# isunLt/U2MKD

Hardware: AMD Instinct MI355X
Metric: LiDAR points/sec/node fwd+bwd (teacher+student+KD), 1/2/4/8 MI355X (higher is better)
Workload: dtype f32 (fp32 products emulated on the 16-bit matrix pipe: f16x2 forward / input gradient, bf16x3 weight gradient; fp32 accumulate)

## Files before the change

### include/u2mkd_hip.h

```cpp
#ifndef U2MKD_HIP_H
#define U2MKD_HIP_H

#include <stddef.h>
#include <stdint.h>

#ifdef __cplusplus
extern "C" {
#endif

typedef void *u2mkd_stream_t;

int u2mkd_version(void);
const char *u2mkd_last_error(void);
int u2mkd_stream_wait_stream(u2mkd_stream_t waiter, u2mkd_stream_t signaler);
void *u2mkd_mailbox_alloc(size_t bytes);
int u2mkd_mailbox_free(void *p);
int u2mkd_mailbox_post(const void *const *srcs, uint32_t is64, int32_t n, int64_t *slot, int64_t seq, u2mkd_stream_t s);

int u2mkd_hash(const int32_t *coords , int64_t n, int64_t *out , u2mkd_stream_t s);
int u2mkd_kernel_hash(const int32_t *coords , const int32_t *offsets , int64_t n,
                      int32_t k, int64_t *out , u2mkd_stream_t s);

size_t u2mkd_hash_table_bytes(int64_t n_refs);
int u2mkd_hash_table_build(const int64_t *refs, int64_t n_refs, void *table, u2mkd_stream_t s);
// ... 7 lines not shown
                           int32_t *nbr , u2mkd_stream_t s);
int u2mkd_kmap_invert(const int32_t *nbr , int64_t n_out, int32_t k, int64_t n_in,
                      int32_t *nbr_inv , u2mkd_stream_t s);
int u2mkd_kmap_sizes(const int32_t *nbr, int64_t n_out, int32_t k, int32_t *nbsizes ,
                     int32_t *block_counts , u2mkd_stream_t s);
int u2mkd_kmap_compact(const int32_t *nbr, int64_t n_out, int32_t k, const int32_t *nbsizes ,
                       int32_t *block_counts ,
                       int32_t *nbmaps , u2mkd_stream_t s);

int64_t u2mkd_pairs_capacity(int64_t n_in, int64_t n_out, int32_t k);
int u2mkd_pairs_build(const int32_t *nbr , int64_t n_out, int64_t n_in, int32_t k,
                      const int32_t *nbsizes, int32_t *block_counts, int32_t *pair_in, int32_t *pair_out,
                      int32_t *pos_out, int32_t *pos_in, int32_t *tile_k, int32_t *meta, u2mkd_stream_t s);
int u2mkd_downsample_keys(const int32_t *coords , int64_t n, int32_t sx, int32_t sy, int32_t sz,
                          int64_t *keys , u2mkd_stream_t s);
int u2mkd_downsample_keys_checked(const int32_t *coords , int64_t n, int32_t sx, int32_t sy, int32_t sz,
                                  int64_t *keys , int32_t *range_flag, u2mkd_stream_t s);
int u2mkd_unpack_keys(const int64_t *keys, int64_t n, int32_t *coords , u2mkd_stream_t s);
int u2mkd_downsample_keys_general(const int32_t *coords , int64_t n, int32_t tsx, int32_t tsy, int32_t tsz, int32_t kx,
                                  int32_t ky, int32_t kz, int32_t sx, int32_t sy, int32_t sz, const int32_t *cmin ,
                                  int32_t m, int64_t *keys , int32_t *range_flag, u2mkd_stream_t s);
int u2mkd_floor_coords(const float *pc , int64_t n, int32_t stride, int32_t *out , u2mkd_stream_t s);

int u2mkd_transpose_weights(const float *w , int32_t k, int32_t cin, int32_t cout,
                            float *wt , u2mkd_stream_t s);
int u2mkd_conv_forward(const float *in , int64_t n_in, int32_t cin, const float *wt ,
                       int32_t cout, const int32_t *nbr , int64_t n_out, int32_t k, int32_t kflip,
                       float *out , u2mkd_stream_t s);
int u2mkd_conv_forward_sorted(const float *in, int64_t n_in, int32_t cin, const float *wt, int32_t cout,
                              const int32_t *nbr_sorted , const int32_t *order ,
                              const int32_t *tile_order , int64_t n_out, int32_t k,
                              int32_t kflip, float *out , u2mkd_stream_t s);
int32_t u2mkd_conv_tiles_supported(int32_t cin, int32_t cout, int32_t k);
int32_t u2mkd_conv_tiles_arith(int32_t cin, int32_t cout, int32_t k);
size_t u2mkd_weight_fragments_bytes(int32_t k, int32_t rows, int32_t cols, int32_t arith);
int u2mkd_weight_fragments(const float *w, int32_t k, int32_t rows, int32_t cols, int32_t transpose, int32_t arith,
                           void *wf, u2mkd_stream_t s);
int u2mkd_weight_fragments_batch(const int64_t *jobs, int32_t n_jobs, int64_t total_units, u2mkd_stream_t s);
int u2mkd_conv_forward_tiles(const float *in, int64_t n_in, int32_t cin, const void *wf, int32_t cout,
                             const int32_t *nbr_sorted , const int32_t *order ,
                             const int32_t *items ,
                             const int32_t *n_items , int64_t n_out, int32_t k,
                             int32_t kflip, int32_t arith, float *out , u2mkd_stream_t s);
int u2mkd_conv_forward_tiles_ep(const float *in, int64_t n_in, int32_t cin, const void *wf, int32_t cout,
                                const int32_t *nbr_sorted, const int32_t *order, const int32_t *items,
                                const int32_t *n_items, int64_t n_out, int32_t k, int32_t kflip, int32_t arith,
                                const float *scale , const float *shift , const float *res ,
                                int32_t relu, float *out, u2mkd_stream_t s);
int32_t u2mkd_pairs_gather_sum_stats_slab_rows(void);
int32_t u2mkd_pairs_gather_sum_stats_supported(int32_t cout);
int u2mkd_pairs_gather_sum_stats(const float *y, const int32_t *pos, int64_t n_rows, int32_t k, int32_t cout, float *out,
                                 float *partial, u2mkd_stream_t s);
int u2mkd_pairs_gather_sum_ep(const float *y, const int32_t *pos, int64_t n_rows, int32_t k, int32_t cout, const float *scale,
                              const float *shift, const float *res, int32_t relu, float *out, u2mkd_stream_t s);
int u2mkd_debug_conv_forward_sorted(const float *in, int64_t n_in, int32_t cin, const float *wt, int32_t cout,
                                    const int32_t *nbr_sorted, const int32_t *order, const int32_t *tile_order,
                                    int64_t n_out, int32_t k, int32_t kflip, int32_t variant, float *out,
                                    u2mkd_stream_t s);
int u2mkd_debug_conv_tile_pairs_stamps(const float *in, int64_t n_in, const void *wf ,
                                       const int32_t *nbr_sorted, const int32_t *order, const int32_t *items,
                                       const int32_t *n_items, int64_t n_out, int32_t k, int32_t arith, float *out,
                                       uint64_t *stamps, u2mkd_stream_t s);
int u2mkd_debug_wgrad_stamps(const float *a, const float *b, const int32_t *pairs, const int32_t *plan, int64_t n_rows,
                             int32_t k, void *workspace, uint64_t *stamps, u2mkd_stream_t s);
int u2mkd_conv_forward_pairs(const float *in, int64_t n_in, int32_t cin, const float *wt, int32_t cout,
                             const int32_t *pair_idx, const int32_t *tile_k, const int32_t *meta, int64_t capacity,
                             int32_t k, int32_t kc, float *y , u2mkd_stream_t s);
int32_t u2mkd_conv_pairs_x3_supported(int32_t cin, int32_t cout);
int u2mkd_conv_forward_pairs_x3(const float *in, int64_t n_in, int32_t cin, const void *wf, int32_t cout,
                                const int32_t *pair_idx, const int32_t *tile_k, const int32_t *meta, int64_t capacity,
                                int32_t k, float *y , u2mkd_stream_t s);
int u2mkd_linear_forward(const float *x , int64_t n, int32_t cin, const float *w , int32_t cout,
                         const float *bias , int32_t kc, float *y, u2mkd_stream_t s);
int u2mkd_linear_forward_x3(const float *x , int64_t n, int32_t cin, const void *wf, int32_t cout,
                            const float *bias , float *y , u2mkd_stream_t s);
int32_t u2mkd_conv_pairs_f16x2_supported(int32_t cin, int32_t cout);
int u2mkd_conv_forward_pairs_f16x2(const float *in, int64_t n_in, int32_t cin, const void *wf, int32_t cout,
                                    const int32_t *pair_idx, const int32_t *tile_k, const int32_t *meta, int64_t capacity,
                                    int32_t k, float *y, u2mkd_stream_t s);
int u2mkd_linear_forward_f16x2(const float *x, int64_t n, int32_t cin, const void *wf, int32_t cout, const float *bias,
                               float *y, u2mkd_stream_t s);
int u2mkd_pairs_gather_sum(const float *y, const int32_t *pos , int64_t n_rows, int32_t k, int32_t cout,
                           float *out , u2mkd_stream_t s);
int u2mkd_kmap_rowmask(const int32_t *nbr , int64_t n_out, int32_t k, int32_t *mask ,
                       u2mkd_stream_t s);
int u2mkd_conv_forward_tiles_bf16(const void *in , int64_t n_in, int32_t cin, const void *wf, int32_t cout,
                                  const int32_t *nbr_sorted, const int32_t *order, const int32_t *items,
                                  const int32_t *n_items, int64_t n_out, int32_t k, int32_t kflip,
                                  void *out , u2mkd_stream_t s);
int u2mkd_conv_wgrad_pairs_bf16(const void *a , int32_t ca, const void *b , int32_t cb,
                                const int32_t *pairs, const int32_t *plan, int64_t n_rows, int32_t k, int32_t swap,
                                void *workspace, size_t workspace_bytes, float *dw , u2mkd_stream_t s);
int u2mkd_conv_forward_tiles_f16(const void *in , int64_t n_in, int32_t cin, const void *wf, int32_t cout,
                                 const int32_t *nbr_sorted, const int32_t *order, const int32_t *items,
                                 const int32_t *n_items, int64_t n_out, int32_t k, int32_t kflip,
                                 void *out , u2mkd_stream_t s);
int u2mkd_conv_wgrad_pairs_f16(const void *a , int32_t ca, const void *b , int32_t cb,
                               const int32_t *pairs, const int32_t *plan, int64_t n_rows, int32_t k, int32_t swap,
                               void *workspace, size_t workspace_bytes, float *dw , u2mkd_stream_t s);
int u2mkd_conv_forward_pairs_f16(const void *in , int64_t n_in, int32_t cin, const void *wf, int32_t cout,
                                  const int32_t *pair_idx, const int32_t *tile_k, const int32_t *meta, int64_t capacity,
                                  int32_t k, void *y , u2mkd_stream_t s);
int u2mkd_linear_forward_f16(const void *x , int64_t n, int32_t cin, const void *wf, int32_t cout,
                             const float *bias , void *y , u2mkd_stream_t s);
int u2mkd_pairs_gather_sum_f16(const void *y , const int32_t *pos , int64_t n_rows, int32_t k,
                               int32_t cout, void *out , u2mkd_stream_t s);
int u2mkd_conv_forward_pairs_bf16(const void *in , int64_t n_in, int32_t cin, const void *wf, int32_t cout,
                                   const int32_t *pair_idx, const int32_t *tile_k, const int32_t *meta, int64_t capacity,
                                   int32_t k, void *y , u2mkd_stream_t s);
int u2mkd_linear_forward_bf16(const void *x , int64_t n, int32_t cin, const void *wf, int32_t cout,
                              const float *bias , void *y , u2mkd_stream_t s);
int u2mkd_pairs_gather_sum_bf16(const void *y , const int32_t *pos , int64_t n_rows, int32_t k,
                                int32_t cout, void *out , u2mkd_stream_t s);
size_t u2mkd_tile_schedule_workspace_bytes(int64_t n_rows);
int u2mkd_tile_schedule(const int32_t *mask , const int32_t *order , int64_t n_rows,
                        int32_t k, int32_t split0, int32_t split1, void *workspace, int32_t *tile_order,
                        int32_t *items, int32_t *n_items, u2mkd_stream_t s);
int32_t u2mkd_wgrad_plan_ints(int32_t k);
int u2mkd_wgrad_plan(const int32_t *nbsizes , int32_t k, int64_t n_rows, int32_t *plan, u2mkd_stream_t s);
size_t u2mkd_conv_wgrad_pairs_workspace_bytes(int64_t n_rows, int32_t ca, int32_t cb, int32_t k);
int u2mkd_conv_wgrad_pairs(const float *a, int32_t ca, const float *b, int32_t cb, const int32_t *pairs ,
                           const int32_t *plan, int64_t n_rows, int32_t k, int32_t swap, void *workspace,
                           size_t workspace_bytes, float *dw , u2mkd_stream_t s);

size_t u2mkd_convolution_workspace_bytes(int64_t n_in_rows, int64_t n_out_rows, int32_t cin, int32_t cout,
                                         const int32_t *nbsizes_host , int32_t k);
int u2mkd_convolution_forward(const float *in_feat , int64_t n_in_rows, int32_t cin,
                              float *out_feat , int64_t n_out_rows, int32_t cout,
                              const float *kernel , const int32_t *nbmaps ,
                              const int32_t *nbsizes_host , int32_t k, int32_t transpose, void *workspace,
                              size_t workspace_bytes, u2mkd_stream_t s);
int u2mkd_convolution_backward(const float *in_feat , int64_t n_in_rows, int32_t cin,
                               float *grad_in_feat , const float *grad_out_feat ,
                               int64_t n_out_rows, int32_t cout, const float *kernel ,
                               float *grad_kernel , const int32_t *nbmaps, const int32_t *nbsizes_host,
                               int32_t k, int32_t transpose, void *workspace, size_t workspace_bytes, u2mkd_stream_t s);

int u2mkd_count(const int32_t *idx , int64_t n, int32_t *counts , int64_t num,
                u2mkd_stream_t s);
int u2mkd_voxelize_forward(const float *feats , const int32_t *idx , const int32_t *counts ,
                           int64_t n, int64_t nv, int32_t c, float *out , u2mkd_stream_t s);
int u2mkd_voxelize_backward(const float *grad_out , const int32_t *idx, const int32_t *counts, int64_t n,
                            int64_t nv, int32_t c, float *grad_feats , u2mkd_stream_t s);
int u2mkd_devoxelize_forward(const float *feats , const int32_t *idx , const float *w ,
                             int64_t n, int32_t c, float *out , u2mkd_stream_t s);
int u2mkd_devoxelize_backward(const float *grad_out , const int32_t *idx , const float *w ,
                              int64_t n, int64_t nv, int32_t c, float *grad_feats ,
                              u2mkd_stream_t s);
int u2mkd_segment_sum(const float *src , int32_t c, const int32_t *entry_row ,
                      const float *entry_w , const int32_t *seg_offsets , int64_t nv,
                      int32_t mean, float *out , u2mkd_stream_t s);
int u2mkd_voxelize_backward_bf16(const void *grad_out , const int32_t *idx, const int32_t *counts, int64_t n,
                                 int64_t nv, int32_t c, void *grad_feats , u2mkd_stream_t s);
int u2mkd_devoxelize_forward_bf16(const void *feats , const int32_t *idx , const float *w ,
                                  int64_t n, int32_t c, void *out , u2mkd_stream_t s);
int u2mkd_segment_sum_bf16(const void *src , int32_t c, const int32_t *entry_row ,
                           const float *entry_w , const int32_t *seg_offsets , int64_t nv,
                           int32_t mean, void *out , u2mkd_stream_t s);
int u2mkd_voxelize_backward_f16(const void *grad_out , const int32_t *idx, const int32_t *counts, int64_t n,
                                int64_t nv, int32_t c, void *grad_feats , u2mkd_stream_t s);
int u2mkd_devoxelize_forward_f16(const void *feats , const int32_t *idx , const float *w ,
                                 int64_t n, int32_t c, void *out , u2mkd_stream_t s);
int u2mkd_segment_sum_f16(const void *src , int32_t c, const int32_t *entry_row ,
                          const float *entry_w , const int32_t *seg_offsets , int64_t nv,
                          int32_t mean, void *out , u2mkd_stream_t s);
size_t u2mkd_csr_workspace_bytes(int64_t n_entries, int64_t nv);
// ... 254 lines not shown
```

### u2mkd_amd/_lib.py

```python
from __future__ import annotations

import ctypes as C
import os

import torch

_HERE = os.path.dirname(os.path.abspath(__file__))
LIB_PATH = os.path.join(_HERE, 'lib', 'libu2mkd_hip%s.so' % os.environ.get('U2MKD_LIB_SUFFIX', ''))

_i32, _i64, _sz, _f32, _p = C.c_int32, C.c_int64, C.c_size_t, C.c_float, C.c_void_p

SIGNATURES = {
    'u2mkd_version': (C.c_int, []),
    'u2mkd_last_error': (C.c_char_p, []),
    'u2mkd_hash': (C.c_int, [_p, _i64, _p, _p]),
    'u2mkd_kernel_hash': (C.c_int, [_p, _p, _i64, _i32, _p, _p]),
    'u2mkd_hash_table_bytes': (_sz, [_i64]),
    'u2mkd_hash_table_build': (C.c_int, [_p, _i64, _p, _p]),
    'u2mkd_hash_table_query': (C.c_int, [_p, _i64, _p, _i64, _p, _p]),
    'u2mkd_hash_table_query2': (C.c_int, [_p, _i64, _p, _i64, _p, _p, _p]),
    'u2mkd_kmap_build_table': (C.c_int, [_p, _i64, _p, _i64, _p, _i32, _p, _p]),
    'u2mkd_kmap_invert': (C.c_int, [_p, _i64, _i32, _i64, _p, _p]),
    'u2mkd_kmap_sizes': (C.c_int, [_p, _i64, _i32, _p, _p, _p]),
    'u2mkd_kmap_compact': (C.c_int, [_p, _i64, _i32, _p, _p, _p, _p]),
    'u2mkd_downsample_keys': (C.c_int, [_p, _i64, _i32, _i32, _i32, _p, _p]),
    'u2mkd_downsample_keys_checked': (C.c_int, [_p, _i64, _i32, _i32, _i32, _p, _p, _p]),
    'u2mkd_downsample_keys_general': (C.c_int, [_p, _i64] + [_i32] * 9 + [_p, _i32, _p, _p, _p]),
    'u2mkd_floor_coords': (C.c_int, [_p, _i64, _i32, _p, _p]),
    'u2mkd_unpack_keys': (C.c_int, [_p, _i64, _p, _p]),
    'u2mkd_transpose_weights': (C.c_int, [_p, _i32, _i32, _i32, _p, _p]),
    'u2mkd_conv_forward': (C.c_int, [_p, _i64, _i32, _p, _i32, _p, _i64, _i32, _i32, _p, _p]),
    'u2mkd_conv_forward_sorted': (C.c_int, [_p, _i64, _i32, _p, _i32, _p, _p, _p, _i64, _i32, _i32, _p, _p]),
    'u2mkd_debug_conv_forward_sorted': (C.c_int, [_p, _i64, _i32, _p, _i32, _p, _p, _p, _i64, _i32, _i32, _i32, _p, _p]),
    'u2mkd_stream_wait_stream': (C.c_int, [_p, _p]),
    'u2mkd_sgd_chunk_elements': (_i32, []),
    'u2mkd_sgd_batch': (C.c_int, [_p, _i32, _i64, _f32, _f32, _f32, _i32, _i32, _p]),
    'u2mkd_grads_unscale_check': (C.c_int, [_p, _i32, _i64, _p, _p, _p]),
    'u2mkd_sgd_batch_amp': (C.c_int, [_p, _i32, _i64, _f32, _f32, _f32, _i32, _i32, _p, _p, _p]),
    'u2mkd_adam_batch': (C.c_int, [_p, _i32, _i64, _p, _f32, _f32, _i32, _f32, _f32, _f32, _f32, _i32, _p]),
    'u2mkd_adam_batch_amp': (C.c_int, [_p, _i32, _i64, _p, _i32, _f32, _f32, _i32, _f32, _f32, _f32, _f32, _i32, _p, _p, _i32, _p, _p, _p]),
    'u2mkd_debug_adam_stage': (C.c_int, [_i32, _i32, _p, _p, _p, _f32, _p, _i64, _p]),
    'u2mkd_mailbox_alloc': (_p, [_sz]),
    'u2mkd_mailbox_free': (C.c_int, [_p]),
    'u2mkd_mailbox_post': (C.c_int, [_p, C.c_uint32, _i32, _p, _i64, _p]),
    'u2mkd_conv_tiles_supported': (_i32, [_i32, _i32, _i32]),
    'u2mkd_conv_tiles_arith': (_i32, [_i32, _i32, _i32]),
    'u2mkd_weight_fragments_bytes': (_sz, [_i32, _i32, _i32, _i32]),
    'u2mkd_weight_fragments': (C.c_int, [_p, _i32, _i32, _i32, _i32, _i32, _p, _p]),
    'u2mkd_weight_fragments_batch': (C.c_int, [_p, _i32, _i64, _p]),
    'u2mkd_conv_forward_tiles': (C.c_int, [_p, _i64, _i32, _p, _i32, _p, _p, _p, _p, _i64, _i32, _i32, _i32, _p, _p]),
    'u2mkd_conv_forward_tiles_ep': (C.c_int, [_p, _i64, _i32, _p, _i32, _p, _p, _p, _p, _i64, _i32, _i32, _i32, _p, _p, _p, _i32, _p, _p]),
    'u2mkd_pairs_gather_sum_ep': (C.c_int, [_p, _p, _i64, _i32, _i32, _p, _p, _p, _i32, _p, _p]),
    'u2mkd_pairs_gather_sum_stats_slab_rows': (_i32, []),
    'u2mkd_pairs_gather_sum_stats_supported': (_i32, [_i32]),
    'u2mkd_pairs_gather_sum_stats': (C.c_int, [_p, _p, _i64, _i32, _i32, _p, _p, _p]),
    'u2mkd_debug_conv_tile_pairs_stamps': (C.c_int, [_p, _i64, _p, _p, _p, _p, _p, _i64, _i32, _i32, _p, _p, _p]),
    'u2mkd_debug_wgrad_stamps': (C.c_int, [_p, _p, _p, _p, _i64, _i32, _p, _p, _p]),
    'u2mkd_conv_forward_pairs': (C.c_int, [_p, _i64, _i32, _p, _i32, _p, _p, _p, _i64, _i32, _i32, _p, _p]),
    'u2mkd_conv_pairs_x3_supported': (_i32, [_i32, _i32]),
    'u2mkd_conv_forward_pairs_x3': (C.c_int, [_p, _i64, _i32, _p, _i32, _p, _p, _p, _i64, _i32, _p, _p]),
    'u2mkd_linear_forward': (C.c_int, [_p, _i64, _i32, _p, _i32, _p, _i32, _p, _p]),
    'u2mkd_bn2d_workspace_bytes': (C.c_size_t, [_i64, _i32, _i64]),
    'u2mkd_bn2d_train_forward': (C.c_int, [_p, _p, _i64, _i32, _i64, _p, _p, C.c_float, C.c_float, _i32, _p, _p, _p, _p, _p, _p, _p, _p]),
    'u2mkd_bn2d_eval_forward': (C.c_int, [_p, _p, _i64, _i32, _i64, _p, _p, C.c_float, _i32, _p, _p, _p, _p]),
    'u2mkd_bn2d_backward': (C.c_int, [_p, _p, _p, _i64, _i32, _i64, _p, _p, _p, _p, _i32, _i32, _p, _p, _p, _p, _p, _p]),
    'u2mkd_bn2d_local_stats': (C.c_int, [_p, _i64, _i32, _i64, _p, _p, _p]),
    'u2mkd_bn2d_apply': (C.c_int, [_p, _p, _i64, _i32, _i64, _p, _p, _p, _p, _i32, _p, _p]),
    'u2mkd_bn2d_backward_local': (C.c_int, [_p, _p, _p, _i64, _i32, _i64, _p, _p, _p, _p, _i32, _p, _p, _p, _p]),
    'u2mkd_bn2d_backward_apply': (C.c_int, [_p, _p, _p, _i64, _i32, _i64, _p, _p, _p, _p, _p, _i32, _p, _p, _p, _p]),
    'u2mkd_linear_forward_x3': (C.c_int, [_p, _i64, _i32, _p, _i32, _p, _p, _p]),
    'u2mkd_conv_pairs_f16x2_supported': (_i32, [_i32, _i32]),
    'u2mkd_conv_forward_pairs_f16x2': (C.c_int, [_p, _i64, _i32, _p, _i32, _p, _p, _p, _i64, _i32, _p, _p]),
    'u2mkd_linear_forward_f16x2': (C.c_int, [_p, _i64, _i32, _p, _i32, _p, _p, _p]),
    'u2mkd_pairs_capacity': (_i64, [_i64, _i64, _i32]),
    'u2mkd_pairs_build': (C.c_int, [_p, _i64, _i64, _i32, _p, _p, _p, _p, _p, _p, _p, _p, _p]),
    'u2mkd_pairs_gather_sum': (C.c_int, [_p, _p, _i64, _i32, _i32, _p, _p]),
    'u2mkd_kmap_rowmask': (C.c_int, [_p, _i64, _i32, _p, _p]),
    'u2mkd_tile_schedule_workspace_bytes': (_sz, [_i64]),
    'u2mkd_tile_schedule': (C.c_int, [_p, _p, _i64, _i32, _i32, _i32, _p, _p, _p, _p, _p]),
    'u2mkd_wgrad_plan_ints': (_i32, [_i32]),
    'u2mkd_wgrad_plan': (C.c_int, [_p, _i32, _i64, _p, _p]),
    'u2mkd_conv_wgrad_pairs_workspace_bytes': (_sz, [_i64, _i32, _i32, _i32]),
    'u2mkd_conv_wgrad_pairs': (C.c_int, [_p, _i32, _p, _i32, _p, _p, _i64, _i32, _i32, _p, _sz, _p, _p]),
    'u2mkd_conv_forward_tiles_bf16': (C.c_int, [_p, _i64, _i32, _p, _i32, _p, _p, _p, _p, _i64, _i32, _i32, _p, _p]),
    'u2mkd_conv_forward_tiles_f16': (C.c_int, [_p, _i64, _i32, _p, _i32, _p, _p, _p, _p, _i64, _i32, _i32, _p, _p]),
    'u2mkd_conv_wgrad_pairs_bf16': (C.c_int, [_p, _i32, _p, _i32, _p, _p, _i64, _i32, _i32, _p, _sz, _p, _p]),
    'u2mkd_conv_wgrad_pairs_f16': (C.c_int, [_p, _i32, _p, _i32, _p, _p, _i64, _i32, _i32, _p, _sz, _p, _p]),
    'u2mkd_conv_forward_pairs_bf16': (C.c_int, [_p, _i64, _i32, _p, _i32, _p, _p, _p, _i64, _i32, _p, _p]),
    'u2mkd_conv_forward_pairs_f16': (C.c_int, [_p, _i64, _i32, _p, _i32, _p, _p, _p, _i64, _i32, _p, _p]),
    'u2mkd_linear_forward_bf16': (C.c_int, [_p, _i64, _i32, _p, _i32, _p, _p, _p]),
    'u2mkd_linear_forward_f16': (C.c_int, [_p, _i64, _i32, _p, _i32, _p, _p, _p]),
    'u2mkd_pairs_gather_sum_bf16': (C.c_int, [_p, _p, _i64, _i32, _i32, _p, _p]),
    'u2mkd_pairs_gather_sum_f16': (C.c_int, [_p, _p, _i64, _i32, _i32, _p, _p]),
    'u2mkd_convolution_workspace_bytes': (_sz, [_i64, _i64, _i32, _i32, _p, _i32]),
    'u2mkd_convolution_forward': (C.c_int, [_p, _i64, _i32, _p, _i64, _i32, _p, _p, _p, _i32, _i32, _p, _sz, _p]),
    'u2mkd_convolution_backward': (C.c_int, [_p, _i64, _i32, _p, _p, _i64, _i32, _p, _p, _p, _p, _i32, _i32, _p, _sz, _p]),
    'u2mkd_bn_num_slabs': (_i64, [_i64]),
    'u2mkd_bn_train_forward': (C.c_int, [_p, _p, _i32, _i64, _i32, _p, _p, _f32, _f32, _p, _p, _p, _i32, _p, _p, _p, _p, _p]),
    'u2mkd_bn_train_forward_from_partial': (C.c_int, [_p, _p, _i64, _i32, _p, _p, _f32, _f32, _p, _p, _p, _i32, _p, _i32, _p, _p, _p, _p]),
    'u2mkd_bn_eval_forward': (C.c_int, [_p, _p, _i32, _i64, _i32, _p, _p, _f32, _p, _p, _i32, _p, _p, _p]),
    'u2mkd_bn_backward': (C.c_int, [_p, _p, _p, _i32, _i64, _i32, _p, _p, _p, _p, _i32, _i32, _p, _p, _p, _p, _p, _p]),
    'u2mkd_bn_local_stats': (C.c_int, [_p, _i32, _i64, _i32, _p, _p, _p]),
    'u2mkd_bn_merge_stats': (C.c_int, [_p, _i32, _i32, _f32, _f32, _p, _p, _p, _p, _p, _p, _p]),
    'u2mkd_bn_apply': (C.c_int, [_p, _p, _i32, _i64, _i32, _p, _p, _p, _p, _i32, _p, _p]),
    'u2mkd_bn_backward_local': (C.c_int, [_p, _p, _p, _i32, _i64, _i32, _p, _p, _p, _p, _i32, _p, _p, _p, _p]),
    'u2mkd_bn_backward_apply': (C.c_int, [_p, _p, _p, _i32, _i64, _i32, _p, _p, _p, _p, _p, _i32, _p, _p, _p, _p]),
    'u2mkd_ln_num_slabs': (_i64, [_i64, _i32]),
    'u2mkd_ln_forward': (C.c_int, [_p, _i32, _i64, _i32, _p, _p, _f32, _p, _p, _p, _p]),
    'u2mkd_ln_add_forward': (C.c_int, [_p, _p, _p, _i32, _i64, _i32, _p, _p, _f32, _p, _p, _p, _p, _p]),
    'u2mkd_ln_backward': (C.c_int, [_p, _p, _p, _p, _i32, _i64, _i32, _p, _p, _p, _p, _p, _p, _p, _p, _p]),
    'u2mkd_sptr_window_keys': (C.c_int, [_p, _p, _i64, _p, _p, _f32, _f32, _f32, _p, _p]),
    'u2mkd_select_mse_partials': (_i32, []),
    'u2mkd_select_mse_forward': (C.c_int, [_p, _p, _p, _i64, _i32, _p, _p, _p, _p]),
    'u2mkd_select_mse_backward': (C.c_int, [_p, _p, _p, _p, _p, _p, _i64, _i32, _p, _p, _p]),
    'u2mkd_sptr_plan_prepare_workspace_bytes': (_sz, []),
    'u2mkd_sptr_plan_prepare': (C.c_int, [_p, _p, _i64, _f32, _f32, _f32, _f32, _f32, _f32, _p, _p, _p, _p, _p, _p]),
    'u2mkd_sptr_window_ranges': (C.c_int, [_p, _i64, _p, _p, _p]),
    'u2mkd_sptr_quant_coords': (C.c_int, [_p, _p, _i64, _p, _f32, _f32, _f32, _f32, _f32, _f32, _p, _p, _p]),
    'u2mkd_sptr_attention_forward': (C.c_int, [_p, _p, _p, _p, _p, _p, _p, _p, _p, _p, _p, _i32, _i32, _f32, _i64, _i32, _i32, _p, _p, _p]),
    'u2mkd_sptr_backward_workspace_bytes': (_sz, [_i64, _i32, _i32]),
    'u2mkd_sptr_attention_backward': (C.c_int, [_p] * 14 + [_i32, _i32, _f32, _i32, _i64, _i32, _i32] + [_p, _p, _sz] + [_p] * 7),
    'u2mkd_sptr_tiles_workspace_bytes': (_sz, [_i64, _i32]),
    'u2mkd_sptr_attention_forward_tiles': (C.c_int, [_p, _p, _p, _i64, _f32] + [_p] * 8 + [_i32, _i32, _f32, _i64, _i32, _i32, _p, _i64, _p, _p, _sz, _p]),
    'u2mkd_sptr_attention_forward_strided': (C.c_int, [_p, _p, _p, _i64, _f32] + [_p] * 8 + [_i32, _i32, _f32, _i64, _i32, _i32, _p, _i64, _p, _p]),
    'u2mkd_sptr_attention_backward_strided': (C.c_int, [_p, _p, _p, _i64, _f32, _p, _p, _i64] + [_p] * 9 + [_i32, _i32, _f32, _i32, _i64, _i32, _i32]
                                              + [_p, _p, _sz] + [_p, _p, _p, _i64, _p, _p, _p, _p]),
    'u2mkd_sptr_table_reduce': (C.c_int, [_p, _i64, _i32, _i32, _f32, _p, _p, _p, _p]),
    'u2mkd_sptr_precompute_all': (C.c_int, [_i32, _i32, C.c_uint32] + [_p] * 8),
    'u2mkd_sptr_attention_step1_forward': (C.c_int, [_i32, _i32, _i32, _i32, _i32, C.c_uint32] + [_p] * 6),
    'u2mkd_sptr_attention_step1_backward': (C.c_int, [_i32, _i32, _i32, _i32, C.c_uint32] + [_p] * 10),
    'u2mkd_sptr_attention_step2_forward': (C.c_int, [_i32] * 5 + [_p] * 6),
    'u2mkd_sptr_attention_step2_backward': (C.c_int, [_i32] * 5 + [_p] * 10),
    'u2mkd_sptr_dot_prod_with_idx_forward': (C.c_int, [_i32] * 6 + [_p] * 10),
    'u2mkd_sptr_dot_prod_with_idx_all_forward': (C.c_int, [_i32] * 6 + [_p] * 10),
    'u2mkd_sptr_dot_prod_with_idx_backward': (C.c_int, [_i32] * 6 + [_p] * 14),
    'u2mkd_sptr_attention_step2_with_rel_pos_value_forward': (C.c_int, [_i32] * 5 + [_p] * 8),
    'u2mkd_sptr_attention_step2_with_rel_pos_value_backward': (C.c_int, [_i32] * 6 + [_p] * 13),
    'u2mkd_count': (C.c_int, [_p, _i64, _p, _i64, _p]),
    'u2mkd_voxelize_forward': (C.c_int, [_p, _p, _p, _i64, _i64, _i32, _p, _p]),
    'u2mkd_voxelize_backward': (C.c_int, [_p, _p, _p, _i64, _i64, _i32, _p, _p]),
    'u2mkd_devoxelize_forward': (C.c_int, [_p, _p, _p, _i64, _i32, _p, _p]),
    'u2mkd_devoxelize_backward': (C.c_int, [_p, _p, _p, _i64, _i64, _i32, _p, _p]),
    'u2mkd_segment_sum': (C.c_int, [_p, _i32, _p, _p, _p, _i64, _i32, _p, _p]),
    'u2mkd_voxelize_backward_bf16': (C.c_int, [_p, _p, _p, _i64, _i64, _i32, _p, _p]),
    'u2mkd_voxelize_backward_f16': (C.c_int, [_p, _p, _p, _i64, _i64, _i32, _p, _p]),
    'u2mkd_devoxelize_forward_bf16': (C.c_int, [_p, _p, _p, _i64, _i32, _p, _p]),
    'u2mkd_devoxelize_forward_f16': (C.c_int, [_p, _p, _p, _i64, _i32, _p, _p]),
    'u2mkd_segment_sum_bf16': (C.c_int, [_p, _i32, _p, _p, _p, _i64, _i32, _p, _p]),
    'u2mkd_segment_sum_f16': (C.c_int, [_p, _i32, _p, _p, _p, _i64, _i32, _p, _p]),
    'u2mkd_c2l_plan': (C.c_int, [_p, _p, _i32, _i64, _i32, _i32, _i32, _p, _p, _p]),
    'u2mkd_l2c_keys': (C.c_int, [_p, _p, _i32, _i64, _i32, _i64, _i64, _i32, _i32, _p, _p, _p, _p, _p]),
    'u2mkd_l2c_finish': (C.c_int, [_p, _p, _p, _p, _p, _i64, _p, _p, _p, _p, _p]),
    'u2mkd_up_bilinear_forward': (C.c_int, [_p, _p, _i64, _i32, _i32, _i32, _i32, _f32, _f32, _p, _p]),
    'u2mkd_up_bilinear_backward': (C.c_int, [_p, _i64, _i32, _i32, _i32, _i32, _p, _p, _p, _p, _i32, _p, _p]),
    'u2mkd_maxpool3s2_forward': (C.c_int, [_p, _i64, _i32, _i32, _p, _p, _p]),
    'u2mkd_maxpool3s2_backward': (C.c_int, [_p, _p, _i64, _i32, _i32, _p, _p]),
    'u2mkd_transpose_batched': (C.c_int, [_p, _p, _i32, _i32, _i32, _p]),
    'u2mkd_transpose_batched_scaled': (C.c_int, [_p, _p, _i32, _i32, _i32, C.c_float, _p]),
    'u2mkd_l2c_combine_forward': (C.c_int, [_p, _p, _p, _p] + [_i32] * 11 + [_p, _p]),
# ... 76 lines not shown
```

### u2mkd_amd/csrc/conv.hip

```cpp
#include <stdlib.h>

#include "conv_internal.h"

namespace u2mkd {

__global__ void transpose_weights_kernel(const float *__restrict__ w, int cin, int cout, float *__restrict__ wt,
                                         int64_t total) {
    int64_t t = (int64_t)blockIdx.x * blockDim.x + threadIdx.x;
    if (t >= total) return;
    int ci = (int)(t % cin);
    int64_t r = t / cin;
    int co = (int)(r % cout);
    int64_t k = r / cout;
    wt[t] = w[(k * cin + ci) * cout + co];
}

template <int WAVES, int NB, int KC>
__global__ void __launch_bounds__(64 * WAVES)
conv_os2_kernel(const float *__restrict__ in, int cin, const float *__restrict__ wt, int cout,
                const int32_t *__restrict__ nbr, const int32_t *__restrict__ order, RowRange rr_, int K, int kflip,
                float *__restrict__ out) {
    constexpr int NT = 64 * WAVES;
    constexpr int TM = 16 * WAVES, TN = 16 * NB;
    constexpr int BS = KC + 8;
// ... 654 lines not shown
    __syncthreads();
    int buf = 0, c = 0;
    while (true) {
        const bool last_chunk = c + 1 == nchunk;
        const bool have_next = !last_chunk || tile_n < tile_end;
        const bool new_b = have_next && (nchunk > 1 || k_n != k);
        if (have_next) {
            if (!last_chunk) load_stage(k, c + 1, idx, a_nxt, new_b);
            else load_stage(k_n, 0, idx_n, a_nxt, new_b);
        }
        if (__ballot(idx >= 0) != 0ULL) {
            const float *bb = Bs + (size_t)buf * TN * BS + r * BS + 4 * q;
#pragma unroll
            for (int j = 0; j < NJ; ++j) {
                float4 b[NB];
#pragma unroll
                for (int n = 0; n < NB; ++n) b[n] = *reinterpret_cast<const float4 *>(bb + 16 * n * BS + 16 * j);
#pragma unroll
                for (int n = 0; n < NB; ++n) acc[n] = __builtin_amdgcn_mfma_f32_16x16x4f32(a_cur[j].x, b[n].x, acc[n], 0, 0, 0);
#pragma unroll
                for (int n = 0; n < NB; ++n) acc[n] = __builtin_amdgcn_mfma_f32_16x16x4f32(a_cur[j].y, b[n].y, acc[n], 0, 0, 0);
#pragma unroll
                for (int n = 0; n < NB; ++n) acc[n] = __builtin_amdgcn_mfma_f32_16x16x4f32(a_cur[j].z, b[n].z, acc[n], 0, 0, 0);
#pragma unroll
                for (int n = 0; n < NB; ++n) acc[n] = __builtin_amdgcn_mfma_f32_16x16x4f32(a_cur[j].w, b[n].w, acc[n], 0, 0, 0);
            }
        }
        if (last_chunk) {
            float *yr = y + ((size_t)tile * 64 + 16 * wave + 4 * q) * cout + col0 + r;
#pragma unroll
            for (int reg = 0; reg < 4; ++reg)
#pragma unroll
                for (int n = 0; n < NB; ++n) {
                    if (col0 + 16 * n + r < cout) yr[(size_t)reg * cout + 16 * n] = acc[n][reg];
                    acc[n][reg] = bv[n];
                }
        }
        if (!have_next) break;
        if (new_b) {
            store_B(buf ^ 1);
            __syncthreads();
            buf ^= 1;
        }
        if (last_chunk) {
            tile = tile_n;
            idx = idx_n;
            k = k_n;
            c = 0;
            ++tile_n;
            idx_n = -1;
            if (tile_n < tile_end) {
                idx_n = entry(tile_n);
                k_n = tile_k ? tile_k[tile_n] : 0;
            }
        } else {
            ++c;
        }
#pragma unroll
        for (int j = 0; j < NJ; ++j) a_cur[j] = a_nxt[j];
    }
}

template <int KC>
static int launch_conv_pairs(int nb, dim3 grid, hipStream_t st, const float *in, int cin, const float *wt, int cout,
                             const int32_t *pair_idx, const int32_t *tile_k, const int32_t *n_tiles, int64_t n_dense,
                             const float *bias, float *y) {
    size_t lds = (size_t)2 * 16 * nb * (KC + 8) * 4;
#define U2_CASE(N)                                                                                                 \
    case N:                                                                                                        \
        if (lds > 65536)                                                                                           \
            (void)hipFuncSetAttribute(reinterpret_cast<const void *>(&conv_pairs_kernel<N, KC>),                   \
                                      hipFuncAttributeMaxDynamicSharedMemorySize, (int)lds);                       \
        hipLaunchKernelGGL((conv_pairs_kernel<N, KC>), grid, dim3(256), lds, st, in, cin, wt, cout, pair_idx,      \
                           tile_k, n_tiles, n_dense, bias, y);                                                     \
        break;
    switch (nb) {
        U2_CASE(1) U2_CASE(2) U2_CASE(3) U2_CASE(4) U2_CASE(5) U2_CASE(6) U2_CASE(7) U2_CASE(8)
        default: set_error("conv pairs: unsupported column block count %d", nb); return 2;
    }
#undef U2_CASE
    return 0;
}

__global__ void __launch_bounds__(256)
pairs_gather_sum_kernel(const float *__restrict__ y, const int32_t *__restrict__ pos, int64_t n_rows, int K, int c4,
                        float *__restrict__ out, const float *__restrict__ ep_scale = nullptr,
                        const float *__restrict__ ep_shift = nullptr, const float *__restrict__ ep_res = nullptr, int ep_relu = 0) {
    int64_t t = (int64_t)blockIdx.x * 256 + threadIdx.x;
    if (t >= n_rows * c4) return;
    int64_t r = t / c4;
    int c = (int)(t - r * c4);
    const int32_t *pr = pos + r * K;
    float4 acc = make_float4(0.f, 0.f, 0.f, 0.f);
    for (int k0 = 0; k0 < K; k0 += 8) {
        int p[8];
        float4 v[8];
#pragma unroll
        for (int i = 0; i < 8; ++i) p[i] = k0 + i < K ? pr[k0 + i] : -1;
#pragma unroll
        for (int i = 0; i < 8; ++i)
            v[i] = p[i] >= 0 ? reinterpret_cast<const float4 *>(y)[(int64_t)p[i] * c4 + c] : make_float4(0.f, 0.f, 0.f, 0.f);
#pragma unroll
        for (int i = 0; i < 8; ++i) { acc.x += v[i].x; acc.y += v[i].y; acc.z += v[i].z; acc.w += v[i].w; }
    }
    if (ep_scale) {
        const float4 sc = reinterpret_cast<const float4 *>(ep_scale)[c], sh = reinterpret_cast<const float4 *>(ep_shift)[c];
        acc.x = fmaf(acc.x, sc.x, sh.x); acc.y = fmaf(acc.y, sc.y, sh.y); acc.z = fmaf(acc.z, sc.z, sh.z); acc.w = fmaf(acc.w, sc.w, sh.w);
        if (ep_res) {
            const float4 rs = reinterpret_cast<const float4 *>(ep_res)[r * c4 + c];
            acc.x += rs.x; acc.y += rs.y; acc.z += rs.z; acc.w += rs.w;
        }
        if (ep_relu) { acc.x = fmaxf(acc.x, 0.f); acc.y = fmaxf(acc.y, 0.f); acc.z = fmaxf(acc.z, 0.f); acc.w = fmaxf(acc.w, 0.f); }
    }
    reinterpret_cast<float4 *>(out)[r * c4 + c] = acc;
}

constexpr int kGsSlabRows = 32, kGsMaxIt = 16;

__global__ void __launch_bounds__(256)
pairs_gather_sum_stats_kernel(const float *__restrict__ y, const int32_t *__restrict__ pos, int64_t n_rows, int K, int c4,
                              float *__restrict__ out, float *__restrict__ partial) {
    __shared__ float4 red[256];
    const int rl = 256 / c4;
    const int ry = threadIdx.x / c4, j = threadIdx.x - ry * c4;
    const bool lane_on = ry < rl;
    const int64_t r0 = (int64_t)blockIdx.x * kGsSlabRows;
    const int rows = (int)min((int64_t)kGsSlabRows, n_rows - r0);
    float4 vals[kGsMaxIt];
    float4 sum = make_float4(0.f, 0.f, 0.f, 0.f);
#pragma unroll
    for (int it = 0; it < kGsMaxIt; ++it) {
        const int rr = it * rl + ry;
        vals[it] = make_float4(0.f, 0.f, 0.f, 0.f);
        if (lane_on && rr < rows) {
            const int64_t r = r0 + rr;
            const int32_t *pr = pos + r * K;
            float4 acc = make_float4(0.f, 0.f, 0.f, 0.f);
            for (int k0 = 0; k0 < K; k0 += 8) {
                int p[8];
                float4 v[8];
#pragma unroll
                for (int i = 0; i < 8; ++i) p[i] = k0 + i < K ? pr[k0 + i] : -1;
#pragma unroll
                for (int i = 0; i < 8; ++i)
                    v[i] = p[i] >= 0 ? reinterpret_cast<const float4 *>(y)[(int64_t)p[i] * c4 + j] : make_float4(0.f, 0.f, 0.f, 0.f);
#pragma unroll
                for (int i = 0; i < 8; ++i) { acc.x += v[i].x; acc.y += v[i].y; acc.z += v[i].z; acc.w += v[i].w; }
            }
            reinterpret_cast<float4 *>(out)[r * c4 + j] = acc;
            vals[it] = acc;
            sum.x += acc.x; sum.y += acc.y; sum.z += acc.z; sum.w += acc.w;
        }
    }
    if (lane_on) red[ry * c4 + j] = sum;
    __syncthreads();
    float4 mean = make_float4(0.f, 0.f, 0.f, 0.f);
    if (lane_on) {
        for (int g = 0; g < rl; ++g) {
            const float4 v = red[g * c4 + j];
            mean.x += v.x; mean.y += v.y; mean.z += v.z; mean.w += v.w;
        }
        const float inv = 1.f / (float)rows;
        mean.x *= inv; mean.y *= inv; mean.z *= inv; mean.w *= inv;
    }
    __syncthreads();
    float4 m2 = make_float4(0.f, 0.f, 0.f, 0.f);
#pragma unroll
    for (int it = 0; it < kGsMaxIt; ++it) {
        if (lane_on && it * rl + ry < rows) {
            const float dx = vals[it].x - mean.x, dy = vals[it].y - mean.y, dz = vals[it].z - mean.z, dw = vals[it].w - mean.w;
            m2.x += dx * dx; m2.y += dy * dy; m2.z += dz * dz; m2.w += dw * dw;
        }
    }
    if (lane_on) red[ry * c4 + j] = m2;
    __syncthreads();
    if (lane_on && ry == 0) {
        float4 t = make_float4(0.f, 0.f, 0.f, 0.f);
        for (int g = 0; g < rl; ++g) {
            const float4 v = red[g * c4 + j];
            t.x += v.x; t.y += v.y; t.z += v.z; t.w += v.w;
        }
        float *p = partial + (size_t)blockIdx.x * 2 * (4 * c4);
        *reinterpret_cast<float4 *>(p + 4 * j) = mean;
        *reinterpret_cast<float4 *>(p + 4 * c4 + 4 * j) = t;
    }
}

template <bool H16>
__global__ void __launch_bounds__(256)
pairs_gather_sum_rows16_kernel(const uint4 *__restrict__ y, const int32_t *__restrict__ pos, int64_t n_rows, int K, int c8,
                               uint4 *__restrict__ out) {
    int64_t t = (int64_t)blockIdx.x * 256 + threadIdx.x;
    if (t >= n_rows * c8) return;
    int64_t r = t / c8;
    int c = (int)(t - r * c8);
// ... 263 lines not shown
}

int u2mkd_conv_forward_pairs_x3(const float *in, int64_t n_in, int32_t cin, const void *wf, int32_t cout,
                                 const int32_t *pair_idx, const int32_t *tile_k, const int32_t *meta, int64_t capacity,
                                 int32_t k, float *y, u2mkd_stream_t s) {
    if (capacity == 0) return 0;
    U2_REQUIRE(in && wf && pair_idx && tile_k && meta && y, "u2mkd_conv_forward_pairs_x3: null pointer");
    U2_REQUIRE(k > 0 && n_in > 0 && capacity % 64 == 0, "u2mkd_conv_forward_pairs_x3: the capacity must be a multiple of 64");
    int rc = launch_conv_px3("u2mkd_conv_forward_pairs_x3", in, cin, reinterpret_cast<const float *>(wf), cout, pair_idx,
                             tile_k, meta + 1, capacity, y, as_stream(s));
    U2_REQUIRE(rc >= 0, "u2mkd_conv_forward_pairs_x3: cin=%d and cout=%d must be multiples of 32 "
               "(ask u2mkd_conv_pairs_x3_supported first)", cin, cout);
    return rc;
}

int32_t u2mkd_conv_pairs_f16x2_supported(int32_t cin, int32_t cout) {
    static const int pref = [] {
        const char *e = getenv("U2MKD_CONV_ARITH");
        return (e && (e[0] == 'b' || (e[0] == 'f' && e[1] == '3'))) ? 0 : 1;
    }();
    return (pref && conv_px3_supported(cin, cout)) ? 1 : 0;
}

int u2mkd_conv_forward_pairs_f16x2(const float *in, int64_t n_in, int32_t cin, const void *wf, int32_t cout,
                                    const int32_t *pair_idx, const int32_t *tile_k, const int32_t *meta, int64_t capacity,
                                    int32_t k, float *y, u2mkd_stream_t s) {
    if (capacity == 0) return 0;
    U2_REQUIRE(in && wf && pair_idx && tile_k && meta && y, "u2mkd_conv_forward_pairs_f16x2: null pointer");
    U2_REQUIRE(k > 0 && n_in > 0 && capacity % 64 == 0, "u2mkd_conv_forward_pairs_f16x2: the capacity must be a multiple of 64");
    int rc = launch_conv_px3("u2mkd_conv_forward_pairs_f16x2", in, cin, reinterpret_cast<const float *>(wf), cout, pair_idx,
                             tile_k, meta + 1, capacity, y, as_stream(s), false, k);
    U2_REQUIRE(rc >= 0, "u2mkd_conv_forward_pairs_f16x2: cin=%d and cout=%d must be multiples of 32", cin, cout);
    return rc;
}

int u2mkd_linear_forward_f16x2(const float *x, int64_t n, int32_t cin, const void *wf, int32_t cout, const float *bias,
                               float *y, u2mkd_stream_t s) {
    if (n == 0) return 0;
    U2_REQUIRE(x && wf && y, "u2mkd_linear_forward_f16x2: null pointer");
    U2_REQUIRE(n > 0 && n < ((int64_t)1 << 31) - 64, "u2mkd_linear_forward_f16x2: %lld rows out of range", (long long)n);
    int rc = launch_linear_px3("u2mkd_linear_forward_f16x2", x, n, cin, reinterpret_cast<const float *>(wf), cout, bias, y,
                               as_stream(s), false, true);
    U2_REQUIRE(rc >= 0, "u2mkd_linear_forward_f16x2: cin=%d and cout=%d must be multiples of 32", cin, cout);
    return rc;
}

int u2mkd_linear_forward(const float *x, int64_t n, int32_t cin, const float *w, int32_t cout, const float *bias,
                         int32_t variant, float *y, u2mkd_stream_t s) {
    if (n == 0) return 0;
    U2_REQUIRE(x && w && y, "u2mkd_linear_forward: null pointer");
    U2_REQUIRE(cin > 0 && cin % 4 == 0 && cout > 0, "u2mkd_linear_forward: cin=%d must be a positive multiple of 4", cin);
    if (variant == 0) variant = ((int64_t)cin * cout >= 16384 && cin % 64 == 0) ? 64 : 32;
    U2_REQUIRE(variant == 32 || variant == 64, "u2mkd_linear_forward: bad variant %d", variant);
    const int c16 = (cout + 15) / 16;
    const int nb = pick_nb(c16);
    int64_t gx = ceil_div(n, 64);
    if (gx > 2048) gx = 2048;
    dim3 grid((unsigned)gx, (unsigned)ceil_div(c16, nb));
    int rc = variant == 32 ? launch_conv_pairs<32>(nb, grid, as_stream(s), x, cin, w, cout, nullptr, nullptr, nullptr, n, bias, y)
                           : launch_conv_pairs<64>(nb, grid, as_stream(s), x, cin, w, cout, nullptr, nullptr, nullptr, n, bias, y);
    if (rc) return rc;
    return check_launch("u2mkd_linear_forward");
}

int u2mkd_linear_forward_x3(const float *x, int64_t n, int32_t cin, const void *wf, int32_t cout, const float *bias,
                            float *y, u2mkd_stream_t s) {
    if (n == 0) return 0;
    U2_REQUIRE(x && wf && y, "u2mkd_linear_forward_x3: null pointer");
    U2_REQUIRE(n > 0 && n < ((int64_t)1 << 31) - 64, "u2mkd_linear_forward_x3: %lld rows out of range", (long long)n);
    int rc = launch_linear_px3("u2mkd_linear_forward_x3", x, n, cin, reinterpret_cast<const float *>(wf), cout, bias, y,
                               as_stream(s));
    U2_REQUIRE(rc >= 0, "u2mkd_linear_forward_x3: cin=%d and cout=%d must be multiples of 32 "
               "(ask u2mkd_conv_pairs_x3_supported first)", cin, cout);
    return rc;
}

int u2mkd_pairs_gather_sum(const float *y, const int32_t *pos, int64_t n_rows, int32_t k, int32_t cout, float *out,
                            u2mkd_stream_t s) {
    if (n_rows == 0) return 0;
    U2_REQUIRE(y && pos && out, "u2mkd_pairs_gather_sum: null pointer");
    U2_REQUIRE(cout > 0 && cout % 4 == 0 && k > 0, "u2mkd_pairs_gather_sum: cout=%d must be a positive multiple of 4", cout);
    const int c4 = cout / 4;
    const int64_t total = n_rows * c4;
    hipLaunchKernelGGL(pairs_gather_sum_kernel, dim3((unsigned)ceil_div(total, 256)), dim3(256), 0, as_stream(s), y, pos,
                       n_rows, k, c4, out, (const float *)nullptr, (const float *)nullptr, (const float *)nullptr, 0);
    return check_launch("u2mkd_pairs_gather_sum");
}

int32_t u2mkd_pairs_gather_sum_stats_slab_rows(void) { return kGsSlabRows; }

int32_t u2mkd_pairs_gather_sum_stats_supported(int32_t cout) { return cout >= 8 && cout % 4 == 0 && cout <= 512; }

int u2mkd_pairs_gather_sum_stats(const float *y, const int32_t *pos, int64_t n_rows, int32_t k, int32_t cout, float *out,
                                 float *partial, u2mkd_stream_t s) {
    if (n_rows == 0) return 0;
    U2_REQUIRE(y && pos && out && partial, "u2mkd_pairs_gather_sum_stats: null pointer");
    U2_REQUIRE(k > 0 && u2mkd_pairs_gather_sum_stats_supported(cout), "u2mkd_pairs_gather_sum_stats: cout=%d must be a multiple of 4 in 8..512", cout);
    const int64_t slabs = ceil_div(n_rows, (int64_t)kGsSlabRows);
    U2_REQUIRE(slabs < ((int64_t)1 << 31), "u2mkd_pairs_gather_sum_stats: too many rows");
    hipLaunchKernelGGL(pairs_gather_sum_stats_kernel, dim3((unsigned)slabs), dim3(256), 0, as_stream(s), y, pos, n_rows, k, cout / 4,
                       out, partial);
    return check_launch("u2mkd_pairs_gather_sum_stats");
}

int u2mkd_pairs_gather_sum_ep(const float *y, const int32_t *pos, int64_t n_rows, int32_t k, int32_t cout, const float *scale,
                              const float *shift, const float *res, int32_t relu, float *out, u2mkd_stream_t s) {
    if (n_rows == 0) return 0;
    U2_REQUIRE(y && pos && out && scale && shift, "u2mkd_pairs_gather_sum_ep: null pointer");
    U2_REQUIRE(cout > 0 && cout % 4 == 0 && k > 0, "u2mkd_pairs_gather_sum_ep: cout=%d must be a positive multiple of 4", cout);
    const int c4 = cout / 4;
    const int64_t total = n_rows * c4;
    hipLaunchKernelGGL(pairs_gather_sum_kernel, dim3((unsigned)ceil_div(total, 256)), dim3(256), 0, as_stream(s), y, pos,
                       n_rows, k, c4, out, scale, shift, res, (int)relu);
    return check_launch("u2mkd_pairs_gather_sum_ep");
}

static int conv_forward_pairs_rows16(const char *who, int rows16, const void *in, int64_t n_in, int32_t cin, const void *wf,
                                     int32_t cout, const int32_t *pair_idx, const int32_t *tile_k, const int32_t *meta,
                                     int64_t capacity, int32_t k, void *y, u2mkd_stream_t s) {
    if (capacity == 0) return 0;
    U2_REQUIRE(in && wf && pair_idx && tile_k && meta && y, "%s: null pointer", who);
    U2_REQUIRE(k > 0 && n_in > 0 && capacity % 64 == 0, "%s: the capacity must be a multiple of 64", who);
    int rc = launch_conv_px3(who, reinterpret_cast<const float *>(in), cin, reinterpret_cast<const float *>(wf), cout, pair_idx,
                             tile_k, meta + 1, capacity, reinterpret_cast<float *>(y), as_stream(s), rows16);
    U2_REQUIRE(rc >= 0, "%s: cin=%d and cout=%d must be multiples of 32", who, cin, cout);
    return rc;
}

static int linear_forward_rows16(const char *who, int rows16, const void *x, int64_t n, int32_t cin, const void *wf,
                                 int32_t cout, const float *bias, void *y, u2mkd_stream_t s) {
    if (n == 0) return 0;
    U2_REQUIRE(x && wf && y, "%s: null pointer", who);
    U2_REQUIRE(n > 0 && n < ((int64_t)1 << 31) - 64, "%s: %lld rows out of range", who, (long long)n);
    int rc = launch_linear_px3(who, reinterpret_cast<const float *>(x), n, cin, reinterpret_cast<const float *>(wf), cout, bias,
                               reinterpret_cast<float *>(y), as_stream(s), rows16);
    U2_REQUIRE(rc >= 0, "%s: cin=%d and cout=%d must be multiples of 32", who, cin, cout);
    return rc;
}

static int pairs_gather_sum_rows16(const char *who, int rows16, const void *y, const int32_t *pos, int64_t n_rows, int32_t k,
                                   int32_t cout, void *out, u2mkd_stream_t s) {
    if (n_rows == 0) return 0;
    U2_REQUIRE(y && pos && out, "%s: null pointer", who);
    U2_REQUIRE(cout > 0 && cout % 8 == 0 && k > 0, "%s: cout=%d must be a positive multiple of 8", who, cout);
    const int c8 = cout / 8;
    const int64_t total = n_rows * c8;
    if (rows16 == kRowsF16)
        hipLaunchKernelGGL(pairs_gather_sum_rows16_kernel<true>, dim3((unsigned)ceil_div(total, 256)), dim3(256), 0, as_stream(s),
                           reinterpret_cast<const uint4 *>(y), pos, n_rows, k, c8, reinterpret_cast<uint4 *>(out));
    else
        hipLaunchKernelGGL(pairs_gather_sum_rows16_kernel<false>, dim3((unsigned)ceil_div(total, 256)), dim3(256), 0, as_stream(s),
                           reinterpret_cast<const uint4 *>(y), pos, n_rows, k, c8, reinterpret_cast<uint4 *>(out));
    return check_launch(who);
}

int u2mkd_conv_forward_pairs_bf16(const void *in, int64_t n_in, int32_t cin, const void *wf, int32_t cout,
                                   const int32_t *pair_idx, const int32_t *tile_k, const int32_t *meta, int64_t capacity,
                                   int32_t k, void *y, u2mkd_stream_t s) {
    return conv_forward_pairs_rows16("u2mkd_conv_forward_pairs_bf16", kRowsBf16, in, n_in, cin, wf, cout, pair_idx, tile_k, meta,
                                     capacity, k, y, s);
}

int u2mkd_conv_forward_pairs_f16(const void *in, int64_t n_in, int32_t cin, const void *wf, int32_t cout,
                                  const int32_t *pair_idx, const int32_t *tile_k, const int32_t *meta, int64_t capacity,
                                  int32_t k, void *y, u2mkd_stream_t s) {
    return conv_forward_pairs_rows16("u2mkd_conv_forward_pairs_f16", kRowsF16, in, n_in, cin, wf, cout, pair_idx, tile_k, meta,
                                     capacity, k, y, s);
}

int u2mkd_linear_forward_bf16(const void *x, int64_t n, int32_t cin, const void *wf, int32_t cout, const float *bias,
                              void *y, u2mkd_stream_t s) {
    return linear_forward_rows16("u2mkd_linear_forward_bf16", kRowsBf16, x, n, cin, wf, cout, bias, y, s);
}

int u2mkd_linear_forward_f16(const void *x, int64_t n, int32_t cin, const void *wf, int32_t cout, const float *bias,
                             void *y, u2mkd_stream_t s) {
    return linear_forward_rows16("u2mkd_linear_forward_f16", kRowsF16, x, n, cin, wf, cout, bias, y, s);
}

int u2mkd_pairs_gather_sum_bf16(const void *y, const int32_t *pos, int64_t n_rows, int32_t k, int32_t cout, void *out,
                                u2mkd_stream_t s) {
    return pairs_gather_sum_rows16("u2mkd_pairs_gather_sum_bf16", kRowsBf16, y, pos, n_rows, k, cout, out, s);
}

int u2mkd_pairs_gather_sum_f16(const void *y, const int32_t *pos, int64_t n_rows, int32_t k, int32_t cout, void *out,
                               u2mkd_stream_t s) {
    return pairs_gather_sum_rows16("u2mkd_pairs_gather_sum_f16", kRowsF16, y, pos, n_rows, k, cout, out, s);
}

int u2mkd_debug_wgrad_stamps(const float *a, const float *b, const int32_t *pairs, const int32_t *plan, int64_t n_rows,
                             int32_t k, void *workspace, uint64_t *stamps, u2mkd_stream_t s) {
    constexpr int SA_ = 80;
    size_t lds = (size_t)2 * 32 * (SA_ + SA_) * 4;
    dim3 grid(wgrad_g_target(n_rows, k) + k, 1);
    hipLaunchKernelGGL((conv_wgrad_pairs_kernel<2, 2, 32, true>), grid, dim3(256), lds, as_stream(s), a, 64, b, 64, pairs, plan,
// ... 156 lines not shown
```

### u2mkd_amd/csrc/conv_internal.h

```cpp
#pragma once
#include "common.h"

namespace u2mkd {

typedef float f32x4 __attribute__((ext_vector_type(4)));

#ifndef U2MKD_MFMA_GFX950_K32
#define U2MKD_MFMA_GFX950_K32 0
#endif
typedef short u2_s16x8 __attribute__((ext_vector_type(8)));
typedef short u2_s16x4 __attribute__((ext_vector_type(4)));
template <int H, class V8>
__device__ __forceinline__ f32x4 mfma_bf16_k32_half(const V8 &a, const V8 &b, f32x4 c) {
    static_assert(sizeof(V8) == 16, "mfma_bf16_k32_half: 8 bf16 per lane");
    const u2_s16x8 a8 = __builtin_bit_cast(u2_s16x8, a), b8 = __builtin_bit_cast(u2_s16x8, b);
    return H == 0 ? __builtin_amdgcn_mfma_f32_16x16x16bf16_1k(a8.lo, b8.lo, c, 0, 0, 0)
                  : __builtin_amdgcn_mfma_f32_16x16x16bf16_1k(a8.hi, b8.hi, c, 0, 0, 0);
}

template <class V8>
__device__ __forceinline__ f32x4 mfma_bf16_k32(const V8 &a, const V8 &b, f32x4 c, int = 0, int = 0, int = 0) {
    static_assert(sizeof(V8) == 16, "mfma_bf16_k32: 8 bf16 per lane");
#if U2MKD_MFMA_GFX950_K32
    typedef __bf16 bf8_t __attribute__((ext_vector_type(8)));
// ... 6 lines not shown
}

typedef _Float16 u2_h16x8 __attribute__((ext_vector_type(8)));
typedef _Float16 u2_h16x4 __attribute__((ext_vector_type(4)));
typedef _Float16 u2_h16x2 __attribute__((ext_vector_type(2)));
template <int H, class V8>
__device__ __forceinline__ f32x4 mfma_f16_k32_half(const V8 &a, const V8 &b, f32x4 c) {
    static_assert(sizeof(V8) == 16, "mfma_f16_k32_half: 8 fp16 per lane");
    const u2_h16x8 a8 = __builtin_bit_cast(u2_h16x8, a), b8 = __builtin_bit_cast(u2_h16x8, b);
    return H == 0 ? __builtin_amdgcn_mfma_f32_16x16x16f16(a8.lo, b8.lo, c, 0, 0, 0)
                  : __builtin_amdgcn_mfma_f32_16x16x16f16(a8.hi, b8.hi, c, 0, 0, 0);
}
enum Row16 : int { kRowsF32 = 0, kRowsBf16 = 1, kRowsF16 = 2 };
template <class V8>
__device__ __forceinline__ f32x4 mfma_f16_k32(const V8 &a, const V8 &b, f32x4 c) {
    static_assert(sizeof(V8) == 16, "mfma_f16_k32: 8 fp16 per lane");
    const u2_h16x8 a8 = __builtin_bit_cast(u2_h16x8, a), b8 = __builtin_bit_cast(u2_h16x8, b);
    c = __builtin_amdgcn_mfma_f32_16x16x16f16(a8.lo, b8.lo, c, 0, 0, 0);
    return __builtin_amdgcn_mfma_f32_16x16x16f16(a8.hi, b8.hi, c, 0, 0, 0);
}
template <bool H16, class V8>
__device__ __forceinline__ f32x4 mfma_rows16_k32(const V8 &a, const V8 &b, f32x4 c) {
    if constexpr (H16) return mfma_f16_k32(a, b, c);
    else return mfma_bf16_k32(a, b, c);
}
template <bool H16>
__device__ __forceinline__ uint32_t pack_rows16(float lo, float hi) {
    if constexpr (H16) {
        const u2_h16x2 h = {(_Float16)lo, (_Float16)hi};
        return __builtin_bit_cast(uint32_t, h);
    } else {
        const __bf16 a = (__bf16)lo, b = (__bf16)hi;
        return (uint32_t)__builtin_bit_cast(unsigned short, a) | ((uint32_t)__builtin_bit_cast(unsigned short, b) << 16);
    }
}
template <bool H16>
__device__ __forceinline__ void unpack_rows16(uint32_t w, float &lo, float &hi) {
    if constexpr (H16) {
        const u2_h16x2 h = __builtin_bit_cast(u2_h16x2, w);
        lo = (float)h[0];
        hi = (float)h[1];
    } else {
        lo = __uint_as_float(w << 16);
        hi = __uint_as_float(w & 0xffff0000u);
    }
}

__device__ __forceinline__ void f16x2_scale(float m, float &s, float &inv) {
    unsigned e = __float_as_uint(m) >> 23;
    e = e < 15u ? 15u : (e > 253u ? 253u : e);
    s = __uint_as_float((268u - e) << 23);
    inv = __uint_as_float((e - 14u) << 23);
}
__device__ __forceinline__ void f16x2_split2(float a, float b, uint32_t &h, uint32_t &l) {
    const u2_h16x2 hv = {(_Float16)a, (_Float16)b};
    const u2_h16x2 lv = {(_Float16)(a - (float)hv[0]), (_Float16)(b - (float)hv[1])};
    h = __builtin_bit_cast(uint32_t, hv);
    l = __builtin_bit_cast(uint32_t, lv);
}

struct RowRange {
    int64_t ld, begin, end;
    const int32_t *tile_order;
    const float *ep_scale = nullptr, *ep_shift = nullptr, *ep_res = nullptr;
    int ep_relu = 0;
};

int launch_conv_tp(const char *who, const float *in, int cin, const float *wf, int cout, const int32_t *nbr,
                   const int32_t *order, RowRange rr, const int32_t *items, const int32_t *n_items, int k, int kflip,
                   int arith, float *out, hipStream_t st, unsigned long long *stamps = nullptr);
bool conv_tp_supported(int cin, int cout, int k);
bool conv_tp_f16x2_supported(int cin);
int conv_tp_arith(int arith);
size_t weight_fragments_bytes(int k, int rows, int cols, int arith);
int launch_weight_fragments(const float *w, int k, int rows, int cols, int transpose, int arith, float *wf, hipStream_t st);
int launch_weight_fragments_batch(const int64_t *jobs, int n_jobs, int64_t total_units, hipStream_t st);

bool conv_px3_supported(int cin, int cout);
int launch_conv_px3(const char *who, const float *in, int cin, const float *wf, int cout, const int32_t *pair_idx,
                    const int32_t *tile_k, const int32_t *n_tiles, int64_t capacity, float *y, hipStream_t st,
                    int rows16 = kRowsF32 ,
                    int f16x2_k = 0 );
int launch_linear_px3(const char *who, const float *in, int64_t n_rows, int cin, const float *wf, int cout,
                      const float *bias, float *y, hipStream_t st, int rows16 = kRowsF32, bool f16x2 = false);

bool conv_wgrad_x3_supported(int ca, int cb, int k);
int launch_conv_wgrad_x3(const float *a, int ca, const float *b, int cb, const int32_t *pairs, const int32_t *plan,
                         int k, int swap, int g, int merge, float *slabs, hipStream_t st, int rows16);
int conv_wgrad_x3_merge(int ca, int cb);

}
```

### u2mkd_amd/csrc/conv_px3.hip

```cpp
#include <stdlib.h>

#include <type_traits>

#include "conv_internal.h"

namespace u2mkd {

typedef __bf16 px_bf16x8 __attribute__((ext_vector_type(8)));
typedef __bf16 px_bf16x4 __attribute__((ext_vector_type(4)));

__device__ __forceinline__ void px_split3(float x, __bf16 &h, __bf16 &m, __bf16 &l) {
    h = (__bf16)x;
    float r1 = x - (float)h;
    m = (__bf16)r1;
    float r2 = r1 - (float)m;
    l = (__bf16)r2;
}

__device__ __forceinline__ px_bf16x8 px_bf8(const float4 &x) {
    f32x4 v = (f32x4){x.x, x.y, x.z, x.w};
    return __builtin_bit_cast(px_bf16x8, v);
}

template <int CTRL>
__device__ __forceinline__ float px_dpp(float v) {
    return __int_as_float(__builtin_amdgcn_update_dpp(0, __float_as_int(v), CTRL, 0xf, 0xf, true));
}

template <int NW, int NBW, bool DENSE = false, bool B16 = false, int SC = 32, int TL = 1, bool F2 = false, bool H16 = false>
__global__ void __launch_bounds__(64 * NW)
conv_px3_kernel(const float *__restrict__ in, int cin, const float *__restrict__ wf, int cout,
                const int32_t *__restrict__ pair_idx, const int32_t *__restrict__ tile_k,
                const int32_t *__restrict__ n_tiles, float *__restrict__ y, const float *__restrict__ bias = nullptr,
                int n_rows = 0, int k_total = 1) {
    static_assert(B16 ? (SC == 32 || SC == 64) : SC == 32, "step width");
    static_assert(!(F2 && B16), "f16x2 is an arithmetic of fp32 rows");
    static_assert(!H16 || B16, "fp16 storage is a form of the 2-byte-row pipeline");
    constexpr int NT = 64 * NW, TN = 16 * NW * NBW;
    constexpr int RS = 192;
    constexpr int CH = B16 ? SC / 8 : 8;
    constexpr int RU = 64 * TL, RB = 4 * TL;
    constexpr int NCH = RU * CH;
    constexpr int LPT = (NCH + NT - 1) / NT;
    constexpr int NWF = B16 ? SC / 32 : F2 ? 2 : 3;
    const float wsc = F2 ? reinterpret_cast<const float *>(reinterpret_cast<const char *>(wf) + (size_t)k_total * cin * cout * 4)[1] : 1.f;
    const int esz = B16 ? 2 : 4;
    extern __shared__ __attribute__((aligned(16))) char smem[];
    const int tid = threadIdx.x, lane = tid & 63, wave = tid >> 6;
    const int r = lane & 15, q = lane >> 4;
    const int ntile64 = DENSE ? (n_rows + 63) / 64 : *n_tiles;
    const int ntile = (ntile64 + TL - 1) / TL;
    const int gy = (cout + TN - 1) / TN;
    const int lin = (int)blockIdx.x, wpx = (int)gridDim.x >> 3;
    int upb = wpx;
    while ((upb & 1) == 0 && ((ntile + upb - 1) / upb) * gy < 24 * (wpx / upb)) upb >>= 1;
    const int teams = 8 * (wpx / upb);
    const int team = (lin & 7) + 8 * ((lin >> 3) / upb), slot = (lin >> 3) % upb;
    if (slot >= ntile) return;
    const int gmax = (ntile - 1 - slot) / upb;
    const int bmax = gmax * gy + gy - 1;
    if (bmax < team) return;
    const int t0 = 0, t1 = (bmax - team) / teams + 1;
    const int ns = cin / SC;
    const int nsteps = (t1 - t0) * ns;
    const int ncb = cout / 16;
    auto block_of = [&](int t) __attribute__((always_inline)) { return team + teams * min(t, t1 - 1); };
    auto unit_of = [&](int t) __attribute__((always_inline)) { return (block_of(t) / gy) * upb + slot; };
    auto cbw_of = [&](int t) __attribute__((always_inline)) { return (block_of(t) % gy) * (TN / 16) + NBW * wave; };

    int crow[LPT], cch[LPT];
#pragma unroll
    for (int l = 0; l < LPT; ++l) {
        const int e = min(tid + l * NT, NCH - 1);
        crow[l] = e / CH;
        cch[l] = e % CH;
    }

    f32x4 acc[RB][NBW];
#pragma unroll
    for (int b = 0; b < RB; ++b)
#pragma unroll
        for (int n = 0; n < NBW; ++n) acc[b][n] = (f32x4){0.f, 0.f, 0.f, 0.f};
    float4 bw[2][NWF * NBW];
    f32x4 g[2][LPT];
    int gix[LPT];
    int kw, cw;

    auto load_idx = [&](int t, int (&ix)[LPT]) __attribute__((always_inline)) {
        const int tt = unit_of(t);
#pragma unroll
        for (int l = 0; l < LPT; ++l) {
            if (DENSE) {
                const int row = tt * RU + crow[l];
                ix[l] = row < n_rows ? row : 0;
            } else {
                ix[l] = pair_idx[(size_t)tt * RU + crow[l]];
            }
        }
    };
    auto issue_G = [&](const int (&ix)[LPT], int s, f32x4 (&gg)[LPT]) __attribute__((always_inline)) {
#pragma unroll
        for (int l = 0; l < LPT; ++l) {
            const int row = ix[l] >= 0 ? ix[l] : 0;
            gg[l] = *reinterpret_cast<const f32x4 *>(reinterpret_cast<const char *>(in) +
                                                     ((size_t)row * cin + SC * s) * esz + 16 * cch[l]);
        }
    };
    auto issue_B = [&](int k, int cbw, int s, float4 (&bb)[NWF * NBW]) __attribute__((always_inline)) {
#pragma unroll
        for (int n = 0; n < NBW; ++n) {
            const int cb = min(cbw + n, ncb - 1);
            const float *pb = wf + ((((size_t)k * ncb + cb) * ns + s) * NWF * 64 + lane) * 4;
#pragma unroll
            for (int p = 0; p < NWF; ++p) bb[NWF * n + p] = *reinterpret_cast<const float4 *>(pb + p * 256);
        }
    };
    auto store_G = [&](const f32x4 (&gg)[LPT], int slot) __attribute__((always_inline)) {
#pragma unroll
        for (int l = 0; l < LPT; ++l) {
            if (B16) {
// ... 60 lines not shown
        load_idx(tg, gix);
        kw = tile_offset(tw);
        cw = cbw_of(tw);
        store_G(g[0], 0);
        lds_barrier();
    }

    auto step = [&](auto U, int i) __attribute__((always_inline)) {
        constexpr int u = decltype(U)::value;
        const int kcur = __builtin_amdgcn_readfirstlane(kw);
        issue_B(kcur, __builtin_amdgcn_readfirstlane(cw), sw, bw[u ^ 1]);
        issue_G(gix, sg, g[u]);
        adv(tw, sw);
        adv(tg, sg);
        kw = tile_offset(tw);
        cw = cbw_of(tw);
        load_idx(tg, gix);
        float4 a[2][NWF];
        read_frag(u, 0, a[0]);
#pragma unroll
        for (int rb = 0; rb < RB; ++rb) {
            if (rb < RB - 1) read_frag(u, rb + 1, a[(rb + 1) & 1]);
            if (B16) {
#pragma unroll
                for (int n = 0; n < NBW; ++n) {
                    f32x4 c = acc[rb][n];
#pragma unroll
                    for (int p = 0; p < NWF; ++p)
                        c = mfma_rows16_k32<H16>(px_bf8(bw[u][NWF * n + p]), px_bf8(a[rb & 1][p]), c);
                    acc[rb][n] = c;
                }
                continue;
            }
            if (F2) {
                const float osc = *reinterpret_cast<const float *>(smem + (u * RU + 16 * rb + r) * RS + 128);
                const float4 xh = a[rb & 1][0], xl = a[rb & 1][NWF - 1];
                f32x4 c[NBW];
#pragma unroll
                for (int n = 0; n < NBW; ++n) c[n] = mfma_f16_k32_half<0>(bw[u][NWF * n + NWF - 1], xh, (f32x4){0.f, 0.f, 0.f, 0.f});
#pragma unroll
                for (int n = 0; n < NBW; ++n) c[n] = mfma_f16_k32_half<1>(bw[u][NWF * n + NWF - 1], xh, c[n]);
#pragma unroll
                for (int n = 0; n < NBW; ++n) c[n] = mfma_f16_k32_half<0>(bw[u][NWF * n], xl, c[n]);
#pragma unroll
                for (int n = 0; n < NBW; ++n) c[n] = mfma_f16_k32_half<1>(bw[u][NWF * n], xl, c[n]);
#pragma unroll
                for (int n = 0; n < NBW; ++n) c[n] = mfma_f16_k32_half<0>(bw[u][NWF * n], xh, c[n]);
#pragma unroll
                for (int n = 0; n < NBW; ++n) c[n] = mfma_f16_k32_half<1>(bw[u][NWF * n], xh, c[n]);
#pragma unroll
                for (int n = 0; n < NBW; ++n) {
                    acc[rb][n][0] = fmaf(c[n][0], osc, acc[rb][n][0]);
                    acc[rb][n][1] = fmaf(c[n][1], osc, acc[rb][n][1]);
                    acc[rb][n][2] = fmaf(c[n][2], osc, acc[rb][n][2]);
                    acc[rb][n][3] = fmaf(c[n][3], osc, acc[rb][n][3]);
                }
                continue;
            }
            const px_bf16x8 xh = px_bf8(a[rb & 1][0]), xm = px_bf8(a[rb & 1][NWF / 2]), xl = px_bf8(a[rb & 1][NWF - 1]);
#pragma unroll
            for (int n = 0; n < NBW; ++n) {
                const px_bf16x8 wh = px_bf8(bw[u][NWF * n]), wm = px_bf8(bw[u][NWF * n + NWF / 2]), wl = px_bf8(bw[u][NWF * n + NWF - 1]);
                f32x4 c = acc[rb][n];
                c = mfma_bf16_k32(wl, xh, c, 0, 0, 0);
                c = mfma_bf16_k32(wh, xl, c, 0, 0, 0);
                c = mfma_bf16_k32(wm, xm, c, 0, 0, 0);
                c = mfma_bf16_k32(wm, xh, c, 0, 0, 0);
                c = mfma_bf16_k32(wh, xm, c, 0, 0, 0);
                c = mfma_bf16_k32(wh, xh, c, 0, 0, 0);
                acc[rb][n] = c;
            }
        }
        if (sc + 1 == ns) {
            const int cbw = cbw_of(tc);
#pragma unroll
            for (int rb = 0; rb < RB; ++rb)
#pragma unroll
                for (int n = 0; n < NBW; ++n) {
                    const int col = 16 * (cbw + n) + 4 * q;
                    const int row = unit_of(tc) * RU + 16 * rb + r;
                    if (cbw + n < ncb && (!DENSE || row < n_rows)) {
                        f32x4 o = acc[rb][n];
                        if (DENSE && bias) o += *reinterpret_cast<const f32x4 *>(bias + col);
                        if (H16) {
                            *reinterpret_cast<uint2 *>(reinterpret_cast<char *>(y) + ((size_t)row * cout + col) * 2) =
                                make_uint2(pack_rows16<true>(o[0], o[1]), pack_rows16<true>(o[2], o[3]));
                        } else if (B16) {
                            px_bf16x4 ob;
                            ob[0] = (__bf16)o[0]; ob[1] = (__bf16)o[1]; ob[2] = (__bf16)o[2]; ob[3] = (__bf16)o[3];
                            *reinterpret_cast<px_bf16x4 *>(reinterpret_cast<char *>(y) + ((size_t)row * cout + col) * 2) = ob;
                        } else {
                            *reinterpret_cast<f32x4 *>(y + (size_t)row * cout + col) = o;
                        }
                    }
                    acc[rb][n] = (f32x4){0.f, 0.f, 0.f, 0.f};
                }
        }
        adv(tc, sc);
        store_G(g[u ^ 1], u ^ 1);
        (void)i;
        lds_barrier();
    };
    for (int i = 0; i < nsteps; i += 2) {
        step(std::integral_constant<int, 0>{}, i);
        if (i + 1 >= nsteps) break;
        step(std::integral_constant<int, 1>{}, i + 1);
    }
}

bool conv_px3_supported(int cin, int cout) { return cin >= 32 && cin % 32 == 0 && cout >= 32 && cout % 32 == 0; }

static bool px3_wide(int cout) { return cout % 256 == 0; }

static bool px3_wide3(int cout) { return cout % 192 == 0; }

struct Px3Shape { bool w3; int nbw, tl, tn; };
static Px3Shape px3_shape(int cin, int cout) {
    Px3Shape p;
    p.w3 = cout % 96 == 0 && cout % 128 != 0;
    p.tl = (cin >= 512 || cout >= 384) ? 2 : 1;
    if (p.tl == 2) p.nbw = 2;
    else p.nbw = (!p.w3 && px3_wide(cout)) || (p.w3 && px3_wide3(cout)) ? 4 : 2;
    p.tn = 16 * (p.w3 ? 3 : 4) * p.nbw;
    return p;
}

template <bool DENSE, bool B16, int SC, bool F2 = false, bool H16 = false>
static void px3_launch(const Px3Shape &p, dim3 grid, hipStream_t st, const float *in, int cin, const float *wf, int cout,
                       const int32_t *pair_idx, const int32_t *tile_k, const int32_t *n_tiles, float *y, const float *bias,
                       int n_rows, int k_total = 1) {
    const size_t lds = (size_t)2 * 64 * p.tl * 192;
#define U2_PX3(NW_, NBW_, TL_)                                                                                                  \
    hipLaunchKernelGGL((conv_px3_kernel<NW_, NBW_, DENSE, B16, SC, TL_, F2, H16>), grid, dim3(64 * NW_), lds, st, in, cin, wf, cout, pair_idx, \
                       tile_k, n_tiles, y, bias, n_rows, k_total)
    if (p.tl == 2) {
        if (p.w3) U2_PX3(3, 2, 2); else U2_PX3(4, 2, 2);
    } else if (p.nbw == 4) {
        if (p.w3) U2_PX3(3, 4, 1); else U2_PX3(4, 4, 1);
    } else {
        if (p.w3) U2_PX3(3, 2, 1); else U2_PX3(4, 2, 1);
    }
#undef U2_PX3
}

int launch_conv_px3(const char *who, const float *in, int cin, const float *wf, int cout, const int32_t *pair_idx,
                    const int32_t *tile_k, const int32_t *n_tiles, int64_t capacity, float *y, hipStream_t st, int rows16,
                    int f16x2_k) {
    if (!conv_px3_supported(cin, cout)) return -1;
    const Px3Shape p = px3_shape(cin, cout);
    const int64_t cap_x = (p.tl == 1 && p.nbw == 2 ? 3 : 2) * 256;
    const int gy = (int)ceil_div(cout, p.tn);
    int64_t gx = std::min<int64_t>(cap_x, ceil_div(capacity / (64 * p.tl) * gy, 8) * 8);
    if (gx < 8) gx = 8;
    dim3 grid((unsigned)gx);
    if (f16x2_k > 0) px3_launch<false, false, 32, true>(p, grid, st, in, cin, wf, cout, pair_idx, tile_k, n_tiles, y, nullptr, 0, f16x2_k);
    else if (rows16 == kRowsF32) px3_launch<false, false, 32>(p, grid, st, in, cin, wf, cout, pair_idx, tile_k, n_tiles, y, nullptr, 0);
    else if (rows16 == kRowsF16 && cin % 64 == 0) px3_launch<false, true, 64, false, true>(p, grid, st, in, cin, wf, cout, pair_idx, tile_k, n_tiles, y, nullptr, 0);
    else if (rows16 == kRowsF16) px3_launch<false, true, 32, false, true>(p, grid, st, in, cin, wf, cout, pair_idx, tile_k, n_tiles, y, nullptr, 0);
    else if (cin % 64 == 0) px3_launch<false, true, 64>(p, grid, st, in, cin, wf, cout, pair_idx, tile_k, n_tiles, y, nullptr, 0);
    else px3_launch<false, true, 32>(p, grid, st, in, cin, wf, cout, pair_idx, tile_k, n_tiles, y, nullptr, 0);
    return check_launch(who);
}

int launch_linear_px3(const char *who, const float *in, int64_t n_rows, int cin, const float *wf, int cout,
                      const float *bias, float *y, hipStream_t st, int rows16, bool f16x2) {
    if (!conv_px3_supported(cin, cout)) return -1;
    const Px3Shape p = px3_shape(cin, cout);
    const int gy = (int)ceil_div(cout, p.tn);
    const int64_t cap_x = (p.tl == 1 && p.nbw == 2 ? 3 : 2) * 256;
    int64_t gx = std::min<int64_t>(cap_x, ceil_div(ceil_div(n_rows, 64 * p.tl) * gy, 8) * 8);
    if (gx < 8) gx = 8;
    dim3 grid((unsigned)gx);
    if (f16x2) px3_launch<true, false, 32, true>(p, grid, st, in, cin, wf, cout, nullptr, nullptr, nullptr, y, bias, (int)n_rows, 1);
    else if (rows16 == kRowsF32) px3_launch<true, false, 32>(p, grid, st, in, cin, wf, cout, nullptr, nullptr, nullptr, y, bias, (int)n_rows);
    else if (rows16 == kRowsF16 && cin % 64 == 0) px3_launch<true, true, 64, false, true>(p, grid, st, in, cin, wf, cout, nullptr, nullptr, nullptr, y, bias, (int)n_rows);
    else if (rows16 == kRowsF16) px3_launch<true, true, 32, false, true>(p, grid, st, in, cin, wf, cout, nullptr, nullptr, nullptr, y, bias, (int)n_rows);
    else if (cin % 64 == 0) px3_launch<true, true, 64>(p, grid, st, in, cin, wf, cout, nullptr, nullptr, nullptr, y, bias, (int)n_rows);
    else px3_launch<true, true, 32>(p, grid, st, in, cin, wf, cout, nullptr, nullptr, nullptr, y, bias, (int)n_rows);
    return check_launch(who);
}

}
```

### u2mkd_amd/csrc/conv_tp.hip

```cpp
#include <stdlib.h>

#include <type_traits>

#include "conv_internal.h"

namespace u2mkd {

#ifndef U2MKD_TP_EXTRA_LDS
#define U2MKD_TP_EXTRA_LDS 0
#endif
constexpr int kTpPad = 8;
constexpr int kTpRowShift = 25;

__global__ void weight_fragments_kernel(const float *__restrict__ w, int rows, int cols, int transpose,
                                        float *__restrict__ wf, int64_t total) {
    int64_t t = (int64_t)blockIdx.x * blockDim.x + threadIdx.x;
    if (t >= total) return;
    if (transpose == 2) {
        transpose = 1 - (int)blockIdx.y;
        wf += (size_t)blockIdx.y * total;
    }
    const int ncol = transpose ? cols : rows, nred = transpose ? rows : cols;
    const int c = (int)(t & 3);
    const int lane = (int)((t >> 2) & 63);
// ... 503 lines not shown
                        const float4 wh = bw[SB ? 0 : (u & 1)][2 * sk][n], wl = bw[SB ? 0 : (u & 1)][2 * sk + 1][n];
                        const float4 xh = a[2 * sk], xl = a[2 * sk + 1];
                        acc0 = mfma_f16_k32_half<0>(wl, xh, acc0);
                        acc1 = mfma_f16_k32_half<0>(wh, xl, acc1);
                        acc0 = mfma_f16_k32_half<1>(wl, xh, acc0);
                        acc1 = mfma_f16_k32_half<1>(wh, xl, acc1);
                        acc0 = mfma_f16_k32_half<0>(wh, xh, acc0);
                        acc1 = mfma_f16_k32_half<1>(wh, xh, acc1);
                    }
                } else if (B16) {
#pragma unroll
                    for (int sk = 0; sk < CIN / 32; ++sk) {
                        if (sk & 1) acc1 = mfma_rows16_k32<H16>(as_bf8(bw[SB ? 0 : (u & 1)][sk][n]), as_bf8(a[sk]), acc1);
                        else acc0 = mfma_rows16_k32<H16>(as_bf8(bw[SB ? 0 : (u & 1)][sk][n]), as_bf8(a[sk]), acc0);
                    }
                } else {
#pragma unroll
                    for (int j = 0; j < NJ; ++j) {
                        acc0 = __builtin_amdgcn_mfma_f32_16x16x4f32(bw[SB ? 0 : (u & 1)][j][n].x, a[j].x, acc0, 0, 0, 0);
                        acc1 = __builtin_amdgcn_mfma_f32_16x16x4f32(bw[SB ? 0 : (u & 1)][j][n].y, a[j].y, acc1, 0, 0, 0);
                        acc0 = __builtin_amdgcn_mfma_f32_16x16x4f32(bw[SB ? 0 : (u & 1)][j][n].z, a[j].z, acc0, 0, 0, 0);
                        acc1 = __builtin_amdgcn_mfma_f32_16x16x4f32(bw[SB ? 0 : (u & 1)][j][n].w, a[j].w, acc1, 0, 0, 0);
                    }
                }
                asm volatile("" : "+v"(o[n].x), "+v"(o[n].y), "+v"(o[n].z), "+v"(o[n].w));
                if (live) {
                    if (F2) {
                        o[n].x = fmaf(acc0[0] + acc1[0], osc, o[n].x);
                        o[n].y = fmaf(acc0[1] + acc1[1], osc, o[n].y);
                        o[n].z = fmaf(acc0[2] + acc1[2], osc, o[n].z);
                        o[n].w = fmaf(acc0[3] + acc1[3], osc, o[n].w);
                    } else {
                        o[n].x += acc0[0] + acc1[0];
                        o[n].y += acc0[1] + acc1[1];
                        o[n].z += acc0[2] + acc1[2];
                        o[n].w += acc0[3] + acc1[3];
                    }
                    *po[n] = o[n];
                }
            }
            if (SB && (d1 >> 8) != kcur) {
                issue_B(d1, bw[0]);
                kcur = d1 >> 8;
            }
            store_G(g[(u + 1) % 3], (u + 1) & 1);
            d1 = d2;
            d2 = desc(t + 3);
            d4 = d5;
            if (STAMP) ++n_blocks;
            asm volatile("s_waitcnt lgkmcnt(0)\n\ts_barrier" ::: "memory");
        };
        for (int t0 = 0; t0 < total; t0 += 6) {
            step(std::integral_constant<int, 0>{}, t0);
            if (t0 + 1 >= total) break;
            step(std::integral_constant<int, 1>{}, t0 + 1);
            if (t0 + 2 >= total) break;
            step(std::integral_constant<int, 2>{}, t0 + 2);
            if (t0 + 3 >= total) break;
            step(std::integral_constant<int, 3>{}, t0 + 3);
            if (t0 + 4 >= total) break;
            step(std::integral_constant<int, 4>{}, t0 + 4);
            if (t0 + 5 >= total) break;
            step(std::integral_constant<int, 5>{}, t0 + 5);
        }
    }
    if (STAMP) t_c2 = __builtin_amdgcn_s_memtime();
    __syncthreads();

    constexpr int F4 = TN / 4;
    for (int e = tid; e < T * F4; e += NT) {
        const int row = e / F4, c4 = e - row * F4;
        const int rid = s_rid[row];
        const int col = col0 + 4 * c4;
        if (rid >= 0 && col < cout) {
            float4 v = *reinterpret_cast<const float4 *>(s_out + row * OS + 4 * c4);
            if (!B16 && rr_.ep_scale) {
                const float4 sc = *reinterpret_cast<const float4 *>(rr_.ep_scale + col), sh = *reinterpret_cast<const float4 *>(rr_.ep_shift + col);
                v.x = fmaf(v.x, sc.x, sh.x); v.y = fmaf(v.y, sc.y, sh.y); v.z = fmaf(v.z, sc.z, sh.z); v.w = fmaf(v.w, sc.w, sh.w);
                if (rr_.ep_res) {
                    const float4 r = *reinterpret_cast<const float4 *>(rr_.ep_res + (size_t)rid * cout + col);
                    v.x += r.x; v.y += r.y; v.z += r.z; v.w += r.w;
                }
                if (rr_.ep_relu) { v.x = fmaxf(v.x, 0.f); v.y = fmaxf(v.y, 0.f); v.z = fmaxf(v.z, 0.f); v.w = fmaxf(v.w, 0.f); }
            }
            if (H16) {
                *reinterpret_cast<uint2 *>(reinterpret_cast<char *>(out) + ((size_t)rid * cout + col) * 2) =
                    make_uint2(pack_rows16<true>(v.x, v.y), pack_rows16<true>(v.z, v.w));
            } else if (B16) {
                bf16x4 b;
                b[0] = (__bf16)v.x; b[1] = (__bf16)v.y; b[2] = (__bf16)v.z; b[3] = (__bf16)v.w;
                *reinterpret_cast<bf16x4 *>(reinterpret_cast<char *>(out) + ((size_t)rid * cout + col) * 2) = b;
            } else {
                *reinterpret_cast<float4 *>(out + (size_t)rid * cout + col) = v;
            }
        }
    }
    if (STAMP && tid == 0) {
        unsigned long long *o = stamps + (size_t)it * 8;
        o[0] = t_rt0; o[1] = t_c0; o[2] = t_c1; o[3] = t_c2; o[4] = __builtin_amdgcn_s_memtime();
        o[5] = __builtin_amdgcn_s_memrealtime(); o[6] = (unsigned long long)n_blocks; o[7] = (unsigned long long)code;
    }
    __syncthreads();
    if (it_n < 0) break;
    rq = rq_n; it = it_n; code = code_n;
    if (PF) {
#pragma unroll
        for (int i = 0; i < KPW; ++i) v[i] = vn[PF ? i : 0];
    }
    }
}

static int device_cus() {
    static const int cus = [] {
        int dev = 0, n = 0;
        if (hipGetDevice(&dev) != hipSuccess || hipDeviceGetAttribute(&n, hipDeviceAttributeMultiprocessorCount, dev) != hipSuccess || n <= 0)
            n = 256;
        return n;
    }();
    return cus;
}

template <int NW, int NBW, int CIN, bool STAMP = false, int AR = 1, bool SB = true>
static void launch_tp(dim3 grid, int K, hipStream_t st, const float *in, const float *wt, int cout, const int32_t *nbr,
                      const int32_t *order, RowRange rr, const int32_t *items, const int32_t *n_items, int kflip,
                      float *out, unsigned long long *stamps = nullptr) {
    constexpr int TN = 16 * NW * NBW;
    const size_t lds = (size_t)64 * (TN + 4) * 4 + (size_t)2 * 16 * ((AR == 2 ? 6 * CIN : (AR == 3 || AR == 5) ? 2 * CIN : 4 * CIN) + 4 * kTpPad) + (size_t)(K + 1) * 64 * 4 + 32 * 4 + 64 * 4 +
                       (size_t)(4 * K + 8) * 4 + (AR == 4 ? 2 * 16 * 4 : 0) + U2MKD_TP_EXTRA_LDS;
    const int n_tiles = (int)ceil_div(rr.end - rr.begin, 64);
    static int occ_by_k[33];
    if (occ_by_k[K] == 0) {
        int n = 0;
        if (hipOccupancyMaxActiveBlocksPerMultiprocessor(&n, conv_tp_kernel<NW, NBW, CIN, STAMP, AR, SB>, 64 * NW, lds) != hipSuccess || n <= 0) n = 1;
        occ_by_k[K] = n;
    }
    const int per_cu = occ_by_k[K];
    const unsigned slots = (unsigned)(per_cu * device_cus());
    if (grid.x > slots) grid.x = slots;
    hipLaunchKernelGGL((conv_tp_kernel<NW, NBW, CIN, STAMP, AR, SB>), grid, dim3(64 * NW), lds, st, in, wt, cout, nbr, order, rr,
                       items, n_items, n_tiles, K, kflip, out, stamps);
}

static bool tp_split(int cout, int &nw, int &nbw) {
    if (cout % 16 != 0) return false;
    switch (cout) {
        case 32: nw = 2; nbw = 1; return true;
        case 64: nw = 4; nbw = 1; return true;
        case 96: nw = 3; nbw = 2; return true;
        case 128: nw = 4; nbw = 2; return true;
        default: return false;
    }
}

bool conv_tp_supported(int cin, int cout, int k) {
    int nw, nbw;
    if (k < 1 || k > 32 || !tp_split(cout, nw, nbw)) return false;
    if (!(cin == 32 || cin == 64 || cin == 96 || cin == 128)) return false;
    return cin * nbw <= 128;
}

bool conv_tp_f16x2_supported(int cin) { return cin == 32 || cin == 64 || cin == 128; }

int conv_tp_arith(int arith) {
    if (arith >= 1 && arith <= 5) return arith;
    static const int dflt = [] {
        const char *e = getenv("U2MKD_CONV_ARITH");
// ... 88 lines not shown
```

### u2mkd_amd/fusion.py

```python
import os

import torch
import torch.nn.functional as F
from torch import nn

from .camera import BatchNorm2d, bn_act

__all__ = ['IA_Layer', 'Atten_Fusion_Conv', 'L2CAILayer', 'L2CFusion', 'feature_gather', 'c2l_gather',
           'l2c_scatter', 'feature_fetch', 'l2c_scatter_torch', 'c2l_gather_torch']


def _rows_linear(x, weight, bias, before=None):
    w = weight.squeeze(-1) if weight.dim() == 3 else weight
    if x.is_cuda and w.shape[1] % 4 == 0:
        from .torchsparse.nn import functional as spf
        return spf.linear(x, w, bias, bias_feeds_batchnorm=before is not None and before.training)
    return F.linear(x, w, bias)


def _rows_bn(bn, x, relu=False):
    if x.is_cuda and x.shape[1] % 4 == 0:
        from .torchsparse.nn import functional as spf
        return spf.batch_norm(x, bn, relu)
    y = bn(x)
    return F.relu(y) if relu else y


class IA_Layer(nn.Module):

    def __init__(self, channels):
        super().__init__()
        self.ic, self.pc = channels
        rc = self.pc // 4
        self.conv1 = nn.Sequential(nn.Conv1d(self.ic, self.pc, 1), nn.BatchNorm1d(self.pc), nn.ReLU(True))
        self.fc1 = nn.Sequential(nn.BatchNorm1d(self.ic), nn.ReLU(True), nn.Linear(self.ic, rc))
        self.fc2 = nn.Linear(self.pc, rc)
        self.fc3 = nn.Linear(rc, 1)

    def forward(self, img_feats, point_feats):
        img_feats = img_feats.contiguous()
        ri = _rows_linear(_rows_bn(self.fc1[0], img_feats, relu=True), self.fc1[2].weight, self.fc1[2].bias)
        rp = _rows_linear(point_feats.contiguous(), self.fc2.weight, self.fc2.bias)
        att = torch.sigmoid(_rows_linear(torch.tanh(ri + rp), self.fc3.weight, self.fc3.bias))
        img = _rows_bn(self.conv1[1], _rows_linear(img_feats, self.conv1[0].weight, self.conv1[0].bias, before=self.conv1[1]), relu=True)
        return img * att


class Atten_Fusion_Conv(nn.Module):
    def __init__(self, inplanes_I, inplanes_P, outplanes):
        super().__init__()
        self.ai_layer = IA_Layer(channels=[inplanes_I, inplanes_P])
        self.conv1 = nn.Conv1d(inplanes_P + inplanes_P, outplanes, 1)
        self.bn1 = nn.BatchNorm1d(outplanes)

    def forward(self, point_features, img_features):
        img = self.ai_layer(img_features, point_features)
        fused = torch.cat([point_features, img], dim=1)
        return _rows_bn(self.bn1, _rows_linear(fused, self.conv1.weight, self.conv1.bias, before=self.bn1), relu=True)


class L2CAILayer(nn.Module):
    def __init__(self, channels):
        super().__init__()
        self.ic, self.pc = channels
        rc = self.ic // 4
        self.conv1 = nn.Sequential(nn.Conv2d(self.pc, self.ic, 1), BatchNorm2d(self.ic), nn.ReLU(True))
        self.fc1 = nn.Conv2d(self.ic, rc, kernel_size=1)
        self.fc2 = nn.Conv2d(self.pc, rc, kernel_size=1)
        self.fc3 = nn.Conv2d(rc, 1, kernel_size=1)

    def forward(self, img_feats, point_feats):
        att = torch.sigmoid(self.fc3(torch.tanh(self.fc1(img_feats.contiguous()) + self.fc2(point_feats.contiguous()))))
        return bn_act(self.conv1[1], self.conv1[0](point_feats), relu=True) * att


class L2CFusion(nn.Module):
    def __init__(self, inplanes_I, inplanes_P, outplanes):
        super().__init__()
        self.conv1 = nn.Conv2d(inplanes_I + inplanes_I, outplanes, kernel_size=1)
        self.bn1 = BatchNorm2d(outplanes)
        self.l2c_ai_layer = L2CAILayer(channels=[inplanes_I, inplanes_P])

    def forward(self, point_features, img_features):
        l2c = self.l2c_ai_layer(img_features, point_features)
        fused = self.bn1(self.conv1(torch.cat([img_features, l2c], dim=1)))
        return F.relu(fused), fused


def feature_gather(feature_map, xy, mode='bilinear'):
    return F.grid_sample(feature_map, xy.unsqueeze(1), padding_mode='zeros', align_corners=True, mode=mode).squeeze(2)


def _last_camera(mask):
    ncam = mask.shape[0]
    rank = torch.arange(1, ncam + 1, device=mask.device).view(-1, 1) * mask.to(torch.int64)
    best = rank.max(0)[0]
    return (best - 1).clamp(min=0), best > 0


class _NchwToRows(torch.autograd.Function):

    @staticmethod
    def forward(ctx, fm):
        ctx.shape = fm.shape
        B, ncam, C, h, w = fm.shape
        if fm.is_cuda and fm.dtype == torch.float32 and fm.is_contiguous() and B * ncam <= 65535 and fm.numel():
            from . import _lib as L
            out = torch.empty(B * ncam * h * w, C, dtype=torch.float32, device=fm.device)
            L.call('u2mkd_transpose_batched', L.ptr(fm), L.ptr(out), B * ncam, C, h * w, L.stream())
            return out
        return fm.permute(0, 1, 3, 4, 2).contiguous().view(B * ncam * h * w, C)

    @staticmethod
    def backward(ctx, g):
        B, ncam, C, h, w = ctx.shape
        if g.is_cuda and g.dtype == torch.float32 and B * ncam <= 65535 and g.numel():
            from . import _lib as L
            g = g.contiguous()
            out = torch.empty(B, ncam, C, h, w, dtype=torch.float32, device=g.device)
            L.call('u2mkd_transpose_batched', L.ptr(g), L.ptr(out), B * ncam, h * w, C, L.stream())
            return out
        return g.view(B, ncam, h, w, C).permute(0, 1, 4, 2, 3).contiguous()


def _c2l_plan_torch(pixel_coordinates, masks, h, w):
    ncam = masks[0].shape[0]
    idx, wts = [], []
    for b, (coord, mask) in enumerate(zip(pixel_coordinates, masks)):
        cam, seen = _last_camera(mask)
        xy = coord.gather(0, cam.view(1, -1, 1).expand(1, -1, 2)).squeeze(0).float()
        x = (xy[:, 0] + 1.0) * 0.5 * (w - 1)
        y = (xy[:, 1] + 1.0) * 0.5 * (h - 1)
        x0, y0 = torch.floor(x), torch.floor(y)
        fx, fy = x - x0, y - y0
        base = (b * ncam + cam) * (h * w)
        ii, ww = [], []
        for dy, wy in ((0, 1.0 - fy), (1, fy)):
            for dx, wx in ((0, 1.0 - fx), (1, fx)):
                xi, yi = x0.long() + dx, y0.long() + dy
# ... 271 lines not shown
```

### u2mkd_amd/kd.py

```python
from copy import deepcopy

import os

import torch
import torch.nn.functional as F
from torch import nn

from . import torchsparse
from .camera import BNReluConv, SwiftNetRes18
from .graphs import PieceCache, StaticPiece
from .fusion import Atten_Fusion_Conv, L2CFusion, c2l_gather, feature_fetch, l2c_scatter
from .pixel_head import sampled_head_applies, sampled_pixel_logits
from .lidar.blocks import (BasicConvolutionBlock, BasicDeconvolutionBlock, FusedSequential, PointBatchNorm1d, PointLinear,
                           ResidualBlock)
from .lidar.point_voxel import (initial_voxelize, point_to_voxel, prepare_geometry, prepare_geometry_many, prepare_geometry_staged,
                                voxel_to_point)
from .torchsparse.nn import functional as spf
from .lidar.sphereformer import SphereFormer
from .lidar.spvcnn_spformer import SPVCNN_SPFORMER
from .losses import MixLovaszCrossEntropy, kl_div_logits
from .torchsparse import PointTensor
from .torchsparse import nn as spnn

__all__ = ['StudentMSP2IFM', 'TSDFull', 'teacher_to_student', 'kd_losses', 'KDCriterion']
# ... 88 lines not shown
            elif name.startswith('l2c'):
                blk = self.l2c_fusion_blocks[int(name[3:])]
                fn, mods = (lambda fmap, skip: blk(fmap, skip)), [blk]
            elif name == 'decoder_low':
                fn, mods = (lambda *feats: pb.forward_up(list(feats), im_size=None)), [pb.upsample]
            else:
                assert name.startswith('decoder_'), name
                im_size = tuple(int(v) for v in name[8:].split('x'))
                fn = lambda *feats: self.classifier_pix(pb.forward_up(list(feats), im_size=im_size))
                mods = [pb.upsample, self.classifier_pix]
            pieces[name] = StaticPiece(name, fn, mods)
        return pieces[name]

    def _camera_stage(self, x_in, idx):
        return self._piece('head')(x_in) if idx == 0 else self._piece('stage%d' % idx)(x_in)

    def camera_head(self, in_mod):
        im = in_mod['images']
        im = im.reshape(-1, *im.shape[2:])
        return _Fork(im, 'camera', _CAMERA_STREAM and _overlap_ok()).on_side(
            lambda: self._camera_stage(im, 0), im)

    @staticmethod
    def _tokens(coords, stride, zz):
        from .lidar.point_voxel import p2v_maps
        idx_query, counts = p2v_maps(coords, stride, zz)
        return spf.spvoxelize(zz.F, idx_query, counts)[:, :3].contiguous(), coords[:, 3]

    @torch.no_grad()
    def prefetch_plans(self, in_mod):
        from .fusion import prefetch_plans as fusion_plans
        from .lidar.point_voxel import p2v_maps, v2p_maps
        z, x0 = in_mod['_geometry']
        if x0.C.shape[0] == 0:
            return
        zz = PointTensor(x0.F, x0.C.float())
        n_stage = len(self.vox_downs)
        strides = [x0.s] + [tuple(v * 2 ** (i + 1) for v in x0.s) for i in range(n_stage)]
        if any(x0.cmaps.get(s3) is None for s3 in strides):
            return
        tokens = []
        parts = spf._PREFETCH_PARTS
        for i, s3 in enumerate(strides):
            coords = x0.cmaps[s3]
            if 'A' in parts:
                v2p_maps(coords, s3, z, plans=True)
                p2v_maps(coords, s3, z, plans=True)
            if i > 0 and 'C' in parts:
                p2v_maps(coords, s3, zz, plans=True)
                tok = self._tokens(coords, s3, zz)
                self.transformer_blocks[i - 1].attn.plans(tok[0].float(), tok[1], quantised=True)
                tokens.append(tok)
        if 'C' in parts:
            x0.__dict__['_u2mkd_kd_plans'] = {'zz': zz, 'tokens': tokens}
        im = in_mod['images']
        shapes = self._fusion_shapes.get((int(im.shape[-2]), int(im.shape[-1])))
        if shapes is not None and len(shapes) == n_stage and 'D' in parts:
            fusion_plans(in_mod['pixel_coordinates'], in_mod['masks'], [shapes[i] for i in range(n_stage)])

    def forward(self, in_mod):
        x = in_mod['lidar']
        im = in_mod['images']
        ib, ncam, ic, ih, iw = im.shape
        im = im.reshape(-1, ic, ih, iw)
        pixel_coordinates, masks, fov_mask = in_mod['pixel_coordinates'], in_mod['masks'], in_mod['fov_mask']
        fork = _Fork(im, 'camera', _CAMERA_STREAM and _overlap_ok())
        on_side, join = fork.on_side, fork.join
        n_stage = len(self.vox_downs)
        cam_stage = self._camera_stage
        cam = in_mod.get('_camera_head')
        if cam is None:
            cam = self.camera_head(in_mod)
        z, x0 = in_mod.get('_geometry') or prepare_geometry(x, self.pres, self.vres)
        ahead = x0.__dict__.get('_u2mkd_kd_plans')
        zz = ahead['zz'] if ahead is not None else PointTensor(x0.F, x0.C.float())
        x0 = self.stem(x0)
        z0 = voxel_to_point(x0, z, nearest=False)
        vox_feats = [point_to_voxel(x0, z0)]
        img_feats, mse_loss, pts_feats = [], [], []
        x_im_ready = None
        for idx in range(n_stage):
            if idx > 0:
                cam = on_side(lambda: cam_stage(x_im, idx), x_im, after=x_im_ready if _CAMERA_FORK_EARLY else None)
            vox_out = self.vox_downs[idx](vox_feats[idx])
            if ahead is not None:
                coord_xyz, batch = ahead['tokens'][idx]
            else:
                coord_xyz, batch = self._tokens(vox_out.C, vox_out.s, zz)
            vox_out.F = self.transformer_blocks[idx](vox_out.F, coord_xyz, batch)
            pts_feat = voxel_to_point(vox_out, z0)
            if idx == n_stage - 1:
                pts_feats.append(self.adapt_layer(pts_feat.F))

            x_im, skip = cam
            join(x_im, skip)
            _, ifc, ifh, ifw = skip.shape
            self._fusion_shapes.setdefault((ih, iw), {})[idx] = (ifh, ifw, n_stage - idx)

            l2c_feat_map = l2c_scatter(pts_feat.F, pixel_coordinates, masks, ifh, ifw, n_stage - idx)
            x_im, skip = self._piece('l2c%d' % idx)(l2c_feat_map, skip)
            x_im_ready = fork.mark()
            img_feats.append(skip)

            img_feat_tensor = c2l_gather(skip.view(ib, ncam, ifc, ifh, ifw), pixel_coordinates, masks)
            pseudo = self.learner[idx](pts_feat.F)
            img_feat_tensor, mse = _select_and_mse(img_feat_tensor, pseudo, fov_mask)
            mse_loss.append(mse)
            pts_feat.F = self.c2l_fusion_blocks[idx](pts_feat.F, img_feat_tensor)
            vox_feats.append(point_to_voxel(vox_out, pts_feat))

        fused = fork.mark()
        _, x1, x2, x3, x4 = vox_feats
        z1 = pts_feat
        z1.F = z1.F + self.point_transforms[0](z0.F)
        y1 = point_to_voxel(x4, z1)
        y1.F = self.dropout(y1.F)
        y1 = self.vox_ups[0][0](y1)
        y1 = self.vox_ups[0][1](torchsparse.cat([y1, x3]))
        y2 = self.vox_ups[1][0](y1)
        y2 = self.vox_ups[1][1](torchsparse.cat([y2, x2]))
        z2 = voxel_to_point(y2, z1)
        z2.F = z2.F + self.point_transforms[1](z1.F)
        y3 = point_to_voxel(y2, z2)
        y3.F = self.dropout(y3.F)
        y3 = self.vox_ups[2][0](y3)
        y3 = self.vox_ups[2][1](torchsparse.cat([y3, x1]))
        y4 = self.vox_ups[3][0](y3)
        y4 = self.vox_ups[3][1](torchsparse.cat([y4, x0]))
        z3 = voxel_to_point(y4, z2)
        z3.F = z3.F + self.point_transforms[2](z2.F)

        ret = {'x_vox': self.classifier_vox(z3.F), 'num_pts': [c.shape[1] for c in pixel_coordinates],
               'mse_loss': mse_loss, 'pts_feats': pts_feats}
        if self.run_pix_decoder:
            sampled = sampled_head_applies(img_feats[0], self.classifier_pix)

            def pix_decoder():
                if sampled:
                    fmap = self._piece('decoder_low')(*img_feats)
                    return sampled_pixel_logits(fmap, self.classifier_pix, pixel_coordinates, masks, (ih, iw), ib, ncam)
                if ib * ncam * self.pix_branch.num_features * ih * iw * 4 >= 2 ** 32:
                    raise RuntimeError('the dense pixel head would form a %.1f GB tensor, beyond what MIOpen computes '
                                       'correctly: use the sampled head (U2MKD_SAMPLED_PIXEL_HEAD=1, the default)'
                                       % (ib * ncam * self.pix_branch.num_features * ih * iw * 4 / 1e9))
                fmap = self._piece('decoder_%dx%d' % (ih, iw))(*img_feats)
                fmap = fmap.view(ib, ncam, fmap.shape[1], fmap.shape[2], fmap.shape[3])
                return feature_fetch(masks, pixel_coordinates, fmap)
            x_pix = on_side(pix_decoder, *img_feats, after=fused)
            join(x_pix)
            ret['x_pix'] = x_pix
        return ret


class _SelectMSE(torch.autograd.Function):

    @staticmethod
    def forward(ctx, gathered, pseudo, fov):
        from . import _lib as L
        n, c = pseudo.shape
        gathered, pseudo = gathered.contiguous(), pseudo.contiguous()
        fov8 = fov.contiguous().view(torch.uint8)
        out = torch.empty_like(pseudo)
        partial = torch.empty(2 * L.load().u2mkd_select_mse_partials(), dtype=torch.float32, device=pseudo.device)
        stats = torch.empty(2, dtype=torch.float32, device=pseudo.device)
        L.call('u2mkd_select_mse_forward', L.ptr(gathered), L.ptr(pseudo), L.ptr(fov8), n, c, L.ptr(out), L.ptr(partial),
               L.ptr(stats), L.stream())
        ctx.save_for_backward(gathered, pseudo, fov8, stats)
        return out, stats[0]

    @staticmethod
    def backward(ctx, g_out, g_loss):
        from . import _lib as L
        gathered, pseudo, fov8, stats = ctx.saved_tensors
        n, c = pseudo.shape
        g_out = g_out.contiguous() if g_out is not None else None
        g_loss = g_loss.contiguous().float() if g_loss is not None else None
        d_g = torch.empty_like(gathered) if ctx.needs_input_grad[0] else None
        d_p = torch.empty_like(pseudo)
        L.call('u2mkd_select_mse_backward', L.ptr(g_out), L.ptr(g_loss), L.ptr(stats), L.ptr(gathered), L.ptr(pseudo),
               L.ptr(fov8), n, c, L.ptr(d_g), L.ptr(d_p), L.stream())
        return d_g, d_p, None


def _select_and_mse(gathered, pseudo, fov):
    if (pseudo.is_cuda and pseudo.dtype == torch.float32 and gathered.dtype == torch.float32 and pseudo.shape[1] % 4 == 0
            and fov.dtype == torch.bool and not torch.is_autocast_enabled()):
        return _SelectMSE.apply(gathered, pseudo, fov)
    out = torch.where(fov.unsqueeze(1), gathered, pseudo)
    return out, _masked_mse(pseudo, out.detach(), fov)


# ... 207 lines not shown
```

### u2mkd_amd/lidar/blocks.py

```python
import torch
from torch import nn

from ..torchsparse import SparseTensor
from ..torchsparse import nn as spnn
from ..torchsparse.nn import functional as spf
from ..torchsparse.nn.utils import fapply

__all__ = ['BasicConvolutionBlock', 'BasicDeconvolutionBlock', 'ResidualBlock', 'FusedSequential',
           'PointBatchNorm1d', 'PointLinear', 'RowLayerNorm']


class PointLinear(nn.Linear):

    def forward(self, input):
        return spf.linear(input, self.weight, self.bias)


class RowLayerNorm(nn.LayerNorm):

    def forward(self, input, branch=None, row_scale=None):
        if branch is not None:
            return spf.add_layer_norm(input, branch, row_scale, self.normalized_shape, self.weight, self.bias, self.eps)
        return spf.layer_norm(input, self.normalized_shape, self.weight, self.bias, self.eps)

    def add_norm(self, shortcut, branch, row_scale=None):
        return self(shortcut, branch, row_scale)


class PointBatchNorm1d(nn.BatchNorm1d):

    def forward(self, input):
        return spf.batch_norm(input, self)


import os as _os
_FOLD_EVAL_BN = _os.environ.get('U2MKD_FOLD_EVAL_BN', '1') != '0'
_FOLDABLE_BN = ('BatchNorm', 'SparseSyncBatchNorm')

_FUSABLE_BN = ('BatchNorm', 'PointBatchNorm1d', 'SparseSyncBatchNorm', 'PointSyncBatchNorm1d')
_STATS_BN = ('BatchNorm',)


class FusedSequential(nn.Sequential):

    def forward(self, x, residual=None):
        mods = list(self)
        i = 0
        fold = _FOLD_EVAL_BN and isinstance(x, SparseTensor) and not torch.is_grad_enabled()
        stats = None
        while i < len(mods):
            m = mods[i]
            nxt = mods[i + 1] if i + 1 < len(mods) else None
            if fold and isinstance(m, spnn.Conv3d) and type(nxt).__name__ in _FOLDABLE_BN and not nxt.training \
                    and nxt.track_running_stats and nxt.running_mean is not None:
                after = mods[i + 2] if i + 2 < len(mods) else None
                last_bn = residual is not None and i + 1 == len(mods) - 1
                relu = last_bn or type(after) in (spnn.ReLU, nn.ReLU)
                scale, shift = spf.eval_bn_affine(nxt)
                y = spf.conv_eval_affine(x, m, scale, shift, relu, residual if last_bn else None)
                if y is not None:
                    x = y
                    i += 2 if last_bn or not relu else 3
                    continue
            if (isinstance(m, spnn.Conv3d) and m.bias is None and type(nxt).__name__ in _STATS_BN and nxt.training
                    and isinstance(x, SparseTensor) and torch.is_grad_enabled() and spf.conv_bn_stats_enabled()):
                stats = spf.BnStats()
                spf.BN_STATS_SINK[0] = stats
                try:
                    x = m(x)
                finally:
                    spf.BN_STATS_SINK[0] = None
                i += 1
                continue
            st, stats = (stats if stats is not None and stats.partial is not None else None), None
            fusable = (type(m).__name__ in _FUSABLE_BN and type(nxt) in (spnn.ReLU, nn.ReLU))
            if residual is not None and i == len(mods) - 1:
                assert type(m).__name__ in _FUSABLE_BN, type(m).__name__
                r = residual.F if isinstance(residual, SparseTensor) else residual
                kw = {'stats': st} if st is not None else {}
                if isinstance(x, SparseTensor):
                    x = fapply(x, spf.batch_norm, m, True, r, **kw)
                else:
                    x = spf.batch_norm(x, m, True, r, **kw)
                i += 1
            elif fusable:
                kw = {'stats': st} if st is not None else {}
                if isinstance(x, SparseTensor):
                    x = fapply(x, spf.batch_norm, m, True, **kw)
                else:
                    x = spf.batch_norm(x, m, True, **kw)
                i += 2
            elif st is not None and st.partial is not None and type(m).__name__ in _STATS_BN:
                x = fapply(x, spf.batch_norm, m, False, None, stats=st)
                i += 1
            elif isinstance(m, PointLinear) and type(nxt).__name__ in _FUSABLE_BN and nxt.training and not isinstance(x, SparseTensor):
                x = spf.linear(x, m.weight, m.bias, bias_feeds_batchnorm=True)
                i += 1
            else:
                x = m(x)
                i += 1
        return x


def _conv_bn(inc, outc, ks, stride=1, dilation=1, transposed=False, relu=True):
    layers = [spnn.Conv3d(inc, outc, kernel_size=ks, dilation=dilation, stride=stride, transposed=transposed),
              spnn.BatchNorm(outc)]
    if relu:
        layers.append(spnn.ReLU(True))
    return layers


class BasicConvolutionBlock(nn.Module):
    def __init__(self, inc, outc, ks=3, stride=1, dilation=1):
        super().__init__()
        self.net = FusedSequential(*_conv_bn(inc, outc, ks, stride, dilation))

    def forward(self, x):
        return self.net(x)


class BasicDeconvolutionBlock(nn.Module):
    def __init__(self, inc, outc, ks=3, stride=1):
        super().__init__()
        self.net = FusedSequential(*_conv_bn(inc, outc, ks, stride, transposed=True))

    def forward(self, x):
        return self.net(x)


class ResidualBlock(nn.Module):
    def __init__(self, inc, outc, ks=3, stride=1, dilation=1):
        super().__init__()
        self.net = FusedSequential(*_conv_bn(inc, outc, ks, stride, dilation),
                                   *_conv_bn(outc, outc, ks, 1, dilation, relu=False))
        if inc == outc and stride == 1:
            self.downsample = nn.Sequential()
        else:
            self.downsample = FusedSequential(*_conv_bn(inc, outc, 1, stride, 1, relu=False))
        self.relu = spnn.ReLU(True)

    def forward(self, x):
        return self.net(x, residual=self.downsample(x))
```

### u2mkd_amd/torchsparse/nn/functional.py

```python
from __future__ import annotations

import os
import threading

import weakref

import torch
from torch.autograd import Function

from ... import _host
from ... import _lib as L
from ..tensor import SparseTensor
from ..utils import make_ntuple
from .utils import get_kernel_offsets

_HOST = False


def host_ops():
    global _HOST
    if _HOST is False:
        _HOST = _host.ops()
    return _HOST

# ... 470 lines not shown

class deferred_range_check:

    def __enter__(self):
        st = _deferred()
        self._outer = st[0]
        st[0] = True
        self._start = len(st)
        return self

    def __exit__(self, exc_type, exc, tb):
        st = _deferred()
        flags = st[self._start:]
        del st[self._start:]
        st[0] = self._outer
        if exc_type is None and not self._outer:
            seen = set()
            for f in flags:
                if id(f) not in seen:
                    seen.add(id(f))
                    _check_range_flag(f)
        elif self._outer:
            st.extend(flags)
        return False


def _range_flag(device):
    key = (device.index, torch.cuda.current_stream(device).cuda_stream)
    f = _RANGE_FLAGS.get(key)
    if f is None:
        f = _RANGE_FLAGS[key] = torch.zeros(1, dtype=torch.int32, device=device)
    return f


def _pairs_mode(cin, cout, n_rows=0):
    env = os.environ.get('U2MKD_CONV_SCHEDULE')
    if env in ('tiles', 'pairs'):
        return env == 'pairs'
    if cout % 4:
        return False
    return cin * cout > 8192 or (cin * cout == 8192 and n_rows < 24000)


_PAIRS_X3 = os.environ.get('U2MKD_PAIRS_X3', '1') != '0'

_SCRATCH = {}


def _scratch(nbytes, device):
    key = (device.type, device.index, torch.cuda.current_stream(device).cuda_stream)
    buf = _SCRATCH.get(key)
    if buf is None or buf.numel() < nbytes:
        buf = torch.empty(int(nbytes * 1.25) + 4096, dtype=torch.uint8, device=device)
        _SCRATCH[key] = buf
    return buf


_TILE_SPLIT = tuple(int(v) for v in os.environ.get('U2MKD_TILE_SPLIT', '30,60').split(','))


class TileSchedule:

    def __init__(self, tbl):
        self.k, self.n = tbl.shape
        k, n = tbl.shape
        dev = tbl.device
        mask = torch.empty(n, dtype=torch.int32, device=dev)
        if n:
            L.call('u2mkd_kmap_rowmask', L.ptr(tbl), n, k, L.ptr(mask), L.stream())
        order = torch.argsort(mask, stable=True)
        self.nbr_s = tbl.index_select(1, order).contiguous()
        self.order = order.int()
        t = (n + 63) // 64
        self.tile_order = torch.empty(t, dtype=torch.int32, device=dev)
        self.items = torch.empty(7 * t, dtype=torch.int32, device=dev)
        self.n_items = torch.empty(1, dtype=torch.int32, device=dev)
        ws = torch.empty(max(t, 1) * 8, dtype=torch.int32, device=dev)
        L.call('u2mkd_tile_schedule', L.ptr(mask), L.ptr(self.order), n, k, _TILE_SPLIT[0], _TILE_SPLIT[1], L.ptr(ws),
               L.ptr(self.tile_order), L.ptr(self.items), L.ptr(self.n_items), L.stream())

    def tiles(self):
        return self.nbr_s, self.order

    def run(self, feats, weight, transpose, cout, kflip, out, epilogue=None):
        n_in, cin = feats.shape
        ar = 4 if feats.dtype == torch.float32 and _tiles_arith(cin, cout, self.k) == 4 else 0
        if epilogue is not None:
            sc, sh, res, relu = epilogue
            wf = _weight_layout(weight, transpose, True, arith=ar)
            L.call('u2mkd_conv_forward_tiles_ep', L.ptr(feats), n_in, cin, L.ptr(wf), cout, L.ptr(self.nbr_s),
                   L.ptr(self.order), L.ptr(self.items), L.ptr(self.n_items), self.n, self.k, int(kflip), ar, L.ptr(sc), L.ptr(sh),
                   L.ptr(res), int(relu), L.ptr(out), L.stream())
            return out
        if feats.dtype != torch.float32:
            wf = _weight_layout(weight, transpose, True, arith=_arith16(feats.dtype))
            L.call(_entry('u2mkd_conv_forward_tiles', feats.dtype), L.ptr(feats), n_in, cin, L.ptr(wf), cout, L.ptr(self.nbr_s),
                   L.ptr(self.order), L.ptr(self.items), L.ptr(self.n_items), self.n, self.k, int(kflip), L.ptr(out),
                   L.stream())
        elif L.load().u2mkd_conv_tiles_supported(cin, cout, self.k):
            wf = _weight_layout(weight, transpose, True, arith=ar)
            L.call('u2mkd_conv_forward_tiles', L.ptr(feats), n_in, cin, L.ptr(wf), cout, L.ptr(self.nbr_s),
                   L.ptr(self.order), L.ptr(self.items), L.ptr(self.n_items), self.n, self.k, int(kflip), ar, L.ptr(out),
                   L.stream())
        else:
            wt = _weight_layout(weight, transpose, False)
            L.call('u2mkd_conv_forward_sorted', L.ptr(feats), n_in, cin, L.ptr(wt), cout, L.ptr(self.nbr_s),
                   L.ptr(self.order), L.ptr(self.tile_order), self.n, self.k, int(kflip), L.ptr(out), L.stream())
        return out


class BnStats:
    __slots__ = ('partial', 'slab_rows', 'of')

    def __init__(self):
        self.partial = self.slab_rows = self.of = None

    def describes(self, x):
        return self.partial is not None and self.of == (x.data_ptr(), x.shape[0], x.shape[1]) and x.dtype == torch.float32


BN_STATS_SINK = [None]
_CONV_BN_STATS = os.environ.get('U2MKD_CONV_BN_STATS', '0') != '0'


def conv_bn_stats_enabled():
    return _CONV_BN_STATS


_STATS_MAX_ROWS, _STATS_MIN_COUT = (int(v) for v in os.environ.get('U2MKD_CONV_BN_STATS_SHAPES', '100000000,8').split(','))


def _stats_in_store(n_rows, cout):
    return n_rows <= _STATS_MAX_ROWS and cout >= _STATS_MIN_COUT and bool(L.load().u2mkd_pairs_gather_sum_stats_supported(cout))


class PairSchedule:

    def __init__(self, nbr, n_in):
        k, n_out = nbr.shape
        dev = nbr.device
        lib = L.load()
        self.k, self.n_in, self.n_out = k, n_in, n_out
        self.cap = int(lib.u2mkd_pairs_capacity(n_in, n_out, k))
        nblocks = max((n_out + 1023) // 1024, 1)
        zeros = torch.zeros(k + 2, dtype=torch.int32, device=dev)
        nbsizes = zeros[:k]
        block_counts = torch.empty(k, nblocks, dtype=torch.int32, device=dev)
        self.pair_in = torch.empty(self.cap, dtype=torch.int32, device=dev)
        self.pair_out = torch.empty(self.cap, dtype=torch.int32, device=dev)
        self.pos_out = torch.empty(n_out, k, dtype=torch.int32, device=dev)
        self.pos_in = torch.full((n_in, k), -1, dtype=torch.int32, device=dev)
        self.tile_k = torch.empty(self.cap // 64, dtype=torch.int32, device=dev)
        self.meta = zeros[k:]
        if n_out and n_in:
            st = L.stream()
            L.call('u2mkd_kmap_sizes', L.ptr(nbr), n_out, k, L.ptr(nbsizes), L.ptr(block_counts), st)
            L.call('u2mkd_pairs_build', L.ptr(nbr), n_out, n_in, k, L.ptr(nbsizes), L.ptr(block_counts),
                   L.ptr(self.pair_in), L.ptr(self.pair_out), L.ptr(self.pos_out), L.ptr(self.pos_in),
                   L.ptr(self.tile_k), L.ptr(self.meta), st)
        self.nbsizes = nbsizes

    def run(self, feats, wt, cout, swap, out, variant=0, fragments=False, epilogue=None):
        n, cin = feats.shape
        st = L.stream()
        idx, pos, n_rows = (self.pair_out, self.pos_in, self.n_in) if swap else (self.pair_in, self.pos_out, self.n_out)
        if n_rows == 0:
            return out
        y = _scratch(self.cap * cout * 4, feats.device)
        if feats.dtype != torch.float32:
            L.call(_entry('u2mkd_conv_forward_pairs', feats.dtype), L.ptr(feats), n, cin, L.ptr(wt), cout, L.ptr(idx), L.ptr(self.tile_k),
                   L.ptr(self.meta), self.cap, self.k, L.ptr(y), st)
            L.call(_entry('u2mkd_pairs_gather_sum', feats.dtype), L.ptr(y), L.ptr(pos), n_rows, self.k, cout, L.ptr(out), st)
            return out
        if fragments:
            L.call('u2mkd_conv_forward_pairs_f16x2' if fragments == 2 else 'u2mkd_conv_forward_pairs_x3', L.ptr(feats), n, cin, L.ptr(wt), cout, L.ptr(idx), L.ptr(self.tile_k),
                   L.ptr(self.meta), self.cap, self.k, L.ptr(y), st)
        else:
            L.call('u2mkd_conv_forward_pairs', L.ptr(feats), n, cin, L.ptr(wt), cout, L.ptr(idx), L.ptr(self.tile_k),
                   L.ptr(self.meta), self.cap, self.k, variant, L.ptr(y), st)
        if epilogue is not None:
            sc, sh, res, relu = epilogue
            L.call('u2mkd_pairs_gather_sum_ep', L.ptr(y), L.ptr(pos), n_rows, self.k, cout, L.ptr(sc), L.ptr(sh), L.ptr(res), int(relu),
                   L.ptr(out), st)
            return out
        sink = BN_STATS_SINK[0]
        if sink is not None and sink.partial is None and out.dtype == torch.float32 and _stats_in_store(n_rows, cout):
            rows = int(L.load().u2mkd_pairs_gather_sum_stats_slab_rows())
            partial = torch.empty((n_rows + rows - 1) // rows * 2 * cout, dtype=torch.float32, device=out.device)
            L.call('u2mkd_pairs_gather_sum_stats', L.ptr(y), L.ptr(pos), n_rows, self.k, cout, L.ptr(out), L.ptr(partial), st)
            sink.partial, sink.slab_rows, sink.of = partial, rows, (out.data_ptr(), n_rows, cout)
            return out
        L.call('u2mkd_pairs_gather_sum', L.ptr(y), L.ptr(pos), n_rows, self.k, cout, L.ptr(out), st)
        return out


KMAP_USES = {}


class KernelMap:

    def __init__(self, nbr, nbr_inv, n_in, n_out, symmetric, out_coords):
        self.nbr = nbr
        self.nbr_inv = nbr_inv
        self.n_in = int(n_in)
        self.n_out = int(n_out)
        self.k = int(nbr.shape[0])
        self.symmetric = bool(symmetric)
        self.out_coords = out_coords
        self._rulebook = None
        self._pairs = None
        self._sorted = {}
        self._pair_schedule = None
        self.tag = None

    def _note(self, use):
        if self.tag is not None:
            uses = KMAP_USES.get(self.tag)
            if uses is None:
                uses = KMAP_USES[self.tag] = set()
            uses.add(use)

    def prebuild(self, uses):
        for use in sorted(uses, key=repr):
            if use == 'pair_schedule':
                self.pair_schedule()
            elif use == 'pairs_plan':
                self.pairs_plan()
            elif use[0] == 'schedule' and (not use[1] or self.nbr_inv is not None):
                self.schedule(use[1])

    def sorted_table(self, inverse=False):
        return self.schedule(inverse).tiles()

    def schedule(self, inverse=False):
        hit = self._sorted.get(inverse)
        if hit is None:
            self._note(('schedule', bool(inverse)))
            hit = TileSchedule(self.nbr_inv if inverse else self.nbr)
            self._sorted[inverse] = hit
        return hit

    def pair_schedule(self):
        if self._pair_schedule is None:
            self._note('pair_schedule')
            self._pair_schedule = PairSchedule(self.nbr, self.n_in)
        return self._pair_schedule

    def pairs_plan(self):
        if self._pairs is None:
            self._note('pairs_plan')
            k, n_out = self.k, self.n_out
            dev = self.nbr.device
            nblocks = max((n_out + 1023) // 1024, 1)
            nbsizes = torch.zeros(k, dtype=torch.int32, device=dev)
            block_counts = torch.empty(k, nblocks, dtype=torch.int32, device=dev)
            cap = max(min(k * n_out, self.n_in * k), 1)
            pairs = torch.empty(cap, 2, dtype=torch.int32, device=dev)
            plan = torch.empty(L.load().u2mkd_wgrad_plan_ints(k), dtype=torch.int32, device=dev)
            if n_out:
                L.call('u2mkd_kmap_sizes', L.ptr(self.nbr), n_out, k, L.ptr(nbsizes), L.ptr(block_counts), L.stream())
                L.call('u2mkd_kmap_compact', L.ptr(self.nbr), n_out, k, L.ptr(nbsizes), L.ptr(block_counts),
                       L.ptr(pairs), L.stream())
            L.call('u2mkd_wgrad_plan', L.ptr(nbsizes), k, n_out, L.ptr(plan), L.stream())
            self._pairs = (pairs, nbsizes, plan)
        return self._pairs

    def rulebook(self):
        if self._rulebook is None:
            pairs, nbsizes, plan = self.pairs_plan()
            total = int(plan[0].item())
            self._rulebook = (pairs[:total], nbsizes)
        return self._rulebook

    def __len__(self):
        return 3

    def __getitem__(self, i):
        if i == 0:
            return self.rulebook()[0]
        if i == 1:
            return self.rulebook()[1]
        if i == 2:
            return (self.n_in, self.n_out)
        raise IndexError(i)

    def __iter__(self):
        return iter((self[0], self[1], self[2]))


def build_kmap(coords: torch.Tensor, tensor_stride, kernel_size, stride, out_coords=None) -> KernelMap:
    coords = _i32(coords).contiguous()
    L.require_cuda(coords)
    dev = coords.device
    n_in = coords.shape[0]
    offsets = get_kernel_offsets(kernel_size, stride=tensor_stride, device=dev)
    k = offsets.shape[0]
    table = coords_table(coords)
    strided = any(s > 1 for s in stride)
    if not strided:
        out_coords = coords
    elif out_coords is None:
        out_coords = spdownsample(coords, stride, kernel_size, tensor_stride)
    n_out = out_coords.shape[0]
    nbr = torch.empty(k, n_out, dtype=torch.int32, device=dev)
    L.call('u2mkd_kmap_build_table', L.ptr(table.buf), n_in, L.ptr(out_coords), n_out, L.ptr(offsets), k,
           L.ptr(nbr), L.stream())
    symmetric = (not strided) and (k % 2 == 1)
    nbr_inv = None
    if not symmetric:
        nbr_inv = torch.full((k, n_in), -1, dtype=torch.int32, device=dev)
        L.call('u2mkd_kmap_invert', L.ptr(nbr), n_out, k, n_in, L.ptr(nbr_inv), L.stream())
    return KernelMap(nbr, nbr_inv, n_in, n_out, symmetric, out_coords)


def prefetch_kmaps(x: SparseTensor, specs, level_coords=None, tag=None) -> None:
    coords, ts = x.coords, x.stride
    x.cmaps.setdefault(ts, coords)
    one = (1, 1, 1)
    for kernel_size, stride in specs:
        kernel_size, stride = make_ntuple(kernel_size, ndim=3), make_ntuple(stride, ndim=3)
        key = (ts, kernel_size, stride, one)
        kmap = x.kmaps.get(key)
        if kmap is None:
            nxt = None
            if level_coords is not None and stride != one:
                nxt = level_coords.get(tuple(ts[k] * stride[k] for k in range(3)))
            kmap = x.kmaps[key] = build_kmap(coords, ts, kernel_size, stride, out_coords=nxt)
            if tag is not None and _PREFETCH_PLANS and 'B' in _PREFETCH_PARTS:
                kmap.tag = (tag, key)
                kmap.prebuild(KMAP_USES.get(kmap.tag, ()))
        if stride != one:
            coords, ts = kmap.out_coords, tuple(ts[k] * stride[k] for k in range(3))
            x.cmaps.setdefault(ts, coords)


def _conv_os(feats, weight, transpose, cout, kmap, inverse, n_rows, kflip, epilogue=None):
    out = torch.empty(n_rows, cout, dtype=feats.dtype, device=feats.device)
    rows16 = feats.dtype != torch.float32
    if rows16 and not L.load().u2mkd_conv_tiles_supported(feats.shape[1], cout, kmap.k):
        wt = _weight_layout(weight, transpose, True, arith=_arith16(feats.dtype))
        return kmap.pair_schedule().run(feats, wt, cout, bool(inverse) or bool(kflip), out)
    if not rows16 and _pairs_mode(feats.shape[1], cout, n_rows):
        x3 = _PAIRS_X3 and bool(L.load().u2mkd_conv_pairs_x3_supported(feats.shape[1], cout))
        f2 = x3 and _pairs_f16x2(feats.shape[1], cout)
        wt = _weight_layout(weight, transpose, x3, arith=4 if f2 else 0)
        return kmap.pair_schedule().run(feats, wt, cout, bool(inverse) or bool(kflip), out, fragments=2 if f2 else x3, epilogue=epilogue)
    if inverse and kmap.nbr_inv is None:
        inverse, kflip = False, 1 - int(kflip)
    sch = kmap.schedule(inverse)
    assert sch.n == n_rows
    return sch.run(feats, weight, transpose, cout, kflip, out, epilogue=epilogue)


def conv_epilogue_supported(feats, cin, cout, k, n_rows):
    if feats.dtype != torch.float32 or row_dtype() is not None or cin % 4 or cout % 4:
        return False
    if _pairs_mode(cin, cout, n_rows):
        return True
    return bool(L.load().u2mkd_conv_tiles_supported(cin, cout, k)) and conv_arith_is_default()


_TILES_ARITH = {}
_PAIRS_F16X2 = {}


def _pairs_f16x2(cin, cout):
    key = (cin, cout)
    hit = _PAIRS_F16X2.get(key)
    if hit is None:
        hit = _PAIRS_F16X2[key] = bool(L.load().u2mkd_conv_pairs_f16x2_supported(cin, cout))
    return hit



def _tiles_arith(cin, cout, k):
    key = (cin, cout, k)
    hit = _TILES_ARITH.get(key)
    if hit is None:
        hit = _TILES_ARITH[key] = int(L.load().u2mkd_conv_tiles_arith(cin, cout, k))
    return hit


def conv_arith_is_default():
    return os.environ.get('U2MKD_CONV_SCHEDULE') in (None, 'tiles', 'pairs')


def conv_eval_affine(input: SparseTensor, conv, scale, shift, relu, residual=None):
    kernel_size, stride, dilation = make_ntuple(conv.kernel_size, ndim=3), make_ntuple(conv.stride, ndim=3), make_ntuple(conv.dilation, ndim=3)
    weight = conv.kernel
    if conv.bias is not None or weight.dim() != 3 or kernel_size == (1, 1, 1):
        return None
    feats = input.feats
    k, cin, cout = weight.shape
    if not conv.transposed:
        key = (input.stride, kernel_size, stride, dilation)
        kmap = input.kmaps.get(key)
        if kmap is None:
            kmap = build_kmap(input.coords, input.stride, kernel_size, stride)
            input.kmaps[key] = kmap
        inverse, n_rows = False, kmap.n_out
        out_coords, out_stride = kmap.out_coords, tuple(input.stride[i] * stride[i] for i in range(3))
    else:
        out_stride = tuple(input.stride[i] // stride[i] for i in range(3))
        kmap = input.kmaps[(out_stride, kernel_size, stride, dilation)]
        inverse, n_rows = True, kmap.n_in
        out_coords = input.cmaps[out_stride]
    if not conv_epilogue_supported(feats, cin, cout, k, n_rows) or feats.shape[1] != cin:
        return None
    res = None
    if residual is not None:
        res = (residual.F if isinstance(residual, SparseTensor) else residual).contiguous().float()
    with torch.no_grad():
        out = _conv_os(feats.contiguous(), weight.contiguous().float(), True, cout, kmap, inverse, n_rows, 0,
                       epilogue=(scale, shift, res, bool(relu)))
    output = SparseTensor(coords=out_coords, feats=out, stride=out_stride)
    output.cmaps = input.cmaps
    output.cmaps.setdefault(output.stride, output.coords)
    output.kmaps = input.kmaps
    return output


def eval_bn_affine(bn):
    key = (bn.running_mean._version, bn.running_var._version, None if bn.weight is None else bn.weight._version,
           None if bn.bias is None else bn.bias._version, bn.eps, bn.running_mean.data_ptr(), _WEIGHT_EPOCH[1])
    hit = bn.__dict__.get('_u2mkd_affine')
    if hit is not None and hit[0] == key:
        return hit[1], hit[2]
    with torch.no_grad():
        inv = torch.rsqrt(bn.running_var.float() + bn.eps)
        scale = inv * bn.weight.float() if bn.weight is not None else inv
        shift = (bn.bias.float() if bn.bias is not None else 0.0) - bn.running_mean.float() * scale
        scale, shift = scale.contiguous(), shift.contiguous()
    bn.__dict__['_u2mkd_affine'] = (key, scale, shift)
    return scale, shift
# ... 48 lines not shown
    L.call('u2mkd_weight_fragments_batch', L.ptr(_FRAG_TABLE[0]), len(live), _FRAG_TABLE[1], L.stream())
    epoch = tuple(_WEIGHT_EPOCH)
    for w, job in live:
        w.__dict__[job[1]] = ((w._version, job[7]) + epoch, job[2])


try:
    from torch.optim.optimizer import register_optimizer_step_post_hook as _reg_post
    _reg_post(refresh_weight_fragments)
except ImportError:
    pass


def _conv_rows16_ok(cin, cout):
    return cin >= 32 and cin % 32 == 0 and cout >= 32 and cout % 32 == 0


def _weight_layout(weight, transpose, fragments, arith=0):
    if not transpose and not fragments:
        return weight
    k, r, c = weight.shape if weight.dim() == 3 else (1,) + tuple(weight.shape)
    frozen = not weight.requires_grad
    stamp = (weight._version, weight.data_ptr(), _WEIGHT_EPOCH[0] if not frozen else -1, _WEIGHT_EPOCH[1])
    holder, tag = weight, ''
    base = weight._base
    if base is not None and base.numel() == weight.numel() and base.data_ptr() == weight.data_ptr() and base.is_contiguous() \
            and weight.is_contiguous() and base.requires_grad == weight.requires_grad:
        holder, tag = base, ':%dx%dx%d' % (k, r, c)
    if fragments:
        slot = {3: '_u2mkd_wfrag3', 4: '_u2mkd_wfrag4', 5: '_u2mkd_wfrag5'}.get(arith, '_u2mkd_wfrag') + tag
        hit = holder.__dict__.get(slot)
        if hit is None or hit[0] != stamp:
            nbytes = L.load().u2mkd_weight_fragments_bytes(k, r, c, arith)
            fresh = hit is None or hit[1].shape[1] != nbytes or hit[1].device != weight.device
            both = torch.empty(2, nbytes, dtype=torch.uint8, device=weight.device) if fresh else hit[1]
            L.call('u2mkd_weight_fragments', L.ptr(weight), k, r, c, 2, arith, L.ptr(both), L.stream())
            hit = (stamp, both)
            holder.__dict__[slot] = hit
            job = _FRAG_JOBS.get((id(holder), slot))
            if not frozen and holder.is_leaf and (fresh or job is None or job[0]() is not holder or job[7] != stamp[1] or job[2] is not both):
                _register_fragments(holder, slot, both, k, r, c, arith)
        return hit[1][0 if transpose else 1]
    key = '_u2mkd_wt' + tag
    if frozen:
        hit = holder.__dict__.get(key)
        if hit is not None and hit[0] == stamp:
            return hit[1]
    out = torch.empty(k, c, r, dtype=torch.float32, device=weight.device)
    L.call('u2mkd_transpose_weights', L.ptr(weight), k, r, c, L.ptr(out), L.stream())
    if frozen:
        holder.__dict__[key] = (stamp, out)
    return out


def _transpose_weights(weight):
    return _weight_layout(weight, True, False)


_IDENTITY_PAIRS = {}


def _identity_pairs(n, device):
    key = (n, device.index)
    hit = _IDENTITY_PAIRS.get(key)
    if hit is None:
        if len(_IDENTITY_PAIRS) > 64:
            _IDENTITY_PAIRS.clear()
        i = torch.arange(n, dtype=torch.int32, device=device)
        pairs = torch.stack([i, i], 1).contiguous()
        nbsizes = torch.full((1,), n, dtype=torch.int32, device=device)
        plan = torch.empty(L.load().u2mkd_wgrad_plan_ints(1), dtype=torch.int32, device=device)
        L.call('u2mkd_wgrad_plan', L.ptr(nbsizes), 1, n, L.ptr(plan), L.stream())
        hit = _IDENTITY_PAIRS[key] = (pairs, plan)
    return hit


_LINEAR_X3 = os.environ.get('U2MKD_LINEAR_X3', '1') != '0'


def _dense_x3_ok(cin, cout):
    return _PAIRS_X3 and _LINEAR_X3 and bool(L.load().u2mkd_conv_pairs_x3_supported(cin, cout))


def _dense_x3(x, weight, forward, bias=None, kernel_layout=False):
    n = x.shape[0]
    if kernel_layout:
        cout = weight.shape[-1] if forward else weight.shape[-2]
    else:
        cout = weight.shape[0] if forward else weight.shape[1]
    rows16 = x.dtype != torch.float32
    f2 = not rows16 and _pairs_f16x2(x.shape[1], cout)
    wf = _weight_layout(weight, forward if kernel_layout else not forward, True, arith=_arith16(x.dtype) if rows16 else (4 if f2 else 0))
    y = torch.empty(n, cout, dtype=x.dtype, device=x.device)
    L.call(_entry('u2mkd_linear_forward', x.dtype) if rows16 else ('u2mkd_linear_forward_f16x2' if f2 else 'u2mkd_linear_forward_x3'), L.ptr(x), n,
           x.shape[1], L.ptr(wf), cout, L.ptr(bias), L.ptr(y), L.stream())
    return y


def _dense(x, w_oc_ic, bias=None):
    n, cin = x.shape
    cout = w_oc_ic.shape[0]
    y = torch.empty((n + 63) // 64 * 64, cout, dtype=torch.float32, device=x.device)
    L.call('u2mkd_linear_forward', L.ptr(x), n, cin, L.ptr(w_oc_ic), cout, L.ptr(bias), 0, L.ptr(y), L.stream())
    return y[:n]


_VIEW_NODES = ('SqueezeBackward0', 'SqueezeBackward1', 'UnsqueezeBackward0', 'ViewBackward0', 'UnsafeViewBackward0', 'AliasBackward0')
_LEAF_VIEWS = os.environ.get('U2MKD_DEFER_VIEW_WGRAD', '1') != '0'


def _leaf_behind_view(w):
    base = w._base
    fn = w.grad_fn
    if (not _LEAF_VIEWS or base is None or fn is None or not base.is_leaf or not base.requires_grad or base.numel() != w.numel()
            or base.data_ptr() != w.data_ptr() or base.dtype != w.dtype or not base.is_contiguous() or not w.is_contiguous()
            or type(fn).__name__ not in _VIEW_NODES or len(fn.next_functions) != 1):
        return None
    acc = fn.next_functions[0][0]
    if acc is None or type(acc).__name__ != 'AccumulateGrad' or getattr(acc, 'variable', None) is not base:
        return None
    return base


class LinearFunction(Function):

    @staticmethod
    def forward(ctx, x, weight, bias, bias_grad_is_zero=False):
        L.require_cuda(x, weight)
        param = weight
        weight = weight.contiguous().float()
        owner = param if param.is_leaf else _leaf_behind_view(param)
        ctx.weight_owner = owner if (owner is not None and weight.data_ptr() == param.data_ptr() and weight.dtype == param.dtype) else None
        ctx.weight_is_param = ctx.weight_owner is not None
        ctx.bias_param = bias if (bias is not None and bias.is_leaf and bias.requires_grad and bias.dtype == torch.float32) else None
        ctx.overlap_ok = _deferred_overlap_ok()
        want16 = row_dtype()
        rows16 = want16 if _conv_rows16_ok(weight.shape[1], weight.shape[0]) else None
        ctx.in_dtype = x.dtype
        x = _rows(x, rows16)
        if x.dim() != 2 or x.shape[1] != weight.shape[1]:
            raise RuntimeError(f'linear: input {tuple(x.shape)} does not match weight {tuple(weight.shape)}')
        if weight.shape[1] % 4 != 0 or weight.shape[0] % 4 != 0:
            raise RuntimeError('linear: in/out features must be multiples of 4 on the HIP path')
        ctx.save_for_backward(x, weight)
        ctx.has_bias = bias is not None
        ctx.bias_grad_is_zero = bool(bias_grad_is_zero)
        if x.shape[0] == 0:
            return x.new_zeros(0, weight.shape[0])
        b = bias.contiguous().float() if bias is not None else None
        ctx.x3 = rows16 is not None or _dense_x3_ok(weight.shape[1], weight.shape[0])
        y = _dense_x3(x, weight, True, b) if ctx.x3 else _dense(x, weight, b)
        return y.to(want16) if (want16 is not None and rows16 is None) else y

    @staticmethod
    def backward(ctx, g):
        x, weight = ctx.saved_tensors
        g = _rows(g, x.dtype)
        n = x.shape[0]
        cout, cin = weight.shape
        gx = gw = gb = None
        if n == 0:
            return x.new_zeros(x.shape), torch.zeros_like(weight), (weight.new_zeros(cout) if ctx.has_bias else None), None
        side, deferred_join = None, False
        if ctx.needs_input_grad[1]:
            pairs, plan = _identity_pairs(n, g.device)
            lib = L.load()
            nbytes = lib.u2mkd_conv_wgrad_pairs_workspace_bytes(n, cout, cin, 1)
            ws = torch.empty(max(nbytes, 16), dtype=torch.uint8, device=g.device)
            gw = torch.empty_like(weight)
            side, deferred_join = _wgrad_side(ctx.weight_owner if ctx.weight_is_param else weight, ctx.weight_is_param, g.device,
                                               ctx.needs_input_grad[0], x, g, ws, gw, pairs, plan, allow=getattr(ctx, 'overlap_ok', True))
            L.call(_entry('u2mkd_conv_wgrad_pairs', x.dtype), L.ptr(g), cout, L.ptr(x), cin,
                   L.ptr(pairs), L.ptr(plan), n, 1, 0, L.ptr(ws), nbytes, L.ptr(gw), side.cuda_stream if side is not None else L.stream())
        if ctx.needs_input_grad[0] and ctx.x3:
            gx = _dense_x3(g, weight, False)
        elif ctx.needs_input_grad[0]:
            w_t = torch.empty(1, cin, cout, dtype=torch.float32, device=g.device)
            L.call('u2mkd_transpose_weights', L.ptr(weight), 1, cout, cin, L.ptr(w_t), L.stream())
            gx = _dense(g, w_t[0])
        if side is not None and not deferred_join:
            torch.cuda.current_stream(g.device).wait_stream(side)
        if ctx.has_bias and ctx.needs_input_grad[2]:
            if _DEFER_BIAS_GRAD and deferred_join and side is not None and ctx.bias_param is not None and ctx.bias_param.grad is None:
                gb = torch.empty(cout, dtype=torch.float32, device=g.device)
                gb.record_stream(side)
                with torch.cuda.stream(side):
                    if ctx.bias_grad_is_zero:
                        gb.zero_()
                    else:
                        torch.sum(g, 0, dtype=torch.float32, out=gb)
            else:
                gb = weight.new_zeros(cout) if ctx.bias_grad_is_zero else g.sum(0, dtype=torch.float32)
        if gx is not None and gx.dtype != ctx.in_dtype:
            gx = gx.to(ctx.in_dtype)
        return gx, gw, gb, None


class PointwiseConvFunction(Function):

    @staticmethod
    def forward(ctx, x, kernel, bias):
        L.require_cuda(x, kernel)
        ctx.weight_is_param = kernel.is_leaf
        ctx.overlap_ok = _deferred_overlap_ok()
        cin, cout = kernel.shape[-2], kernel.shape[-1]
        want16 = row_dtype()
        rows16 = want16 if _conv_rows16_ok(cin, cout) else None
        ctx.in_dtype = x.dtype
        x = _rows(x, rows16)
        if x.dim() != 2 or x.shape[1] != cin:
            raise RuntimeError(f'conv3d (1x1x1): input {tuple(x.shape)} does not match kernel {tuple(kernel.shape)}')
        ctx.save_for_backward(x, kernel)
        ctx.has_bias = bias is not None
        if x.shape[0] == 0:
            return x.new_zeros(0, cout)
        b = bias.contiguous().float() if bias is not None else None
        y = _dense_x3(x, kernel, True, b, kernel_layout=True)
        return y.to(want16) if (want16 is not None and rows16 is None) else y

    @staticmethod
    def backward(ctx, g):
        x, kernel = ctx.saved_tensors
        g = _rows(g, x.dtype)
        n = x.shape[0]
        cin, cout = kernel.shape[-2], kernel.shape[-1]
        gx = gw = gb = None
        if n == 0:
            return x.new_zeros(x.shape), torch.zeros_like(kernel), (kernel.new_zeros(cout) if ctx.has_bias else None)
        side, deferred_join = None, False
        if ctx.needs_input_grad[1]:
            pairs, plan = _identity_pairs(n, g.device)
            nbytes = L.load().u2mkd_conv_wgrad_pairs_workspace_bytes(n, cin, cout, 1)
            ws = torch.empty(max(nbytes, 16), dtype=torch.uint8, device=g.device)
            gw = torch.empty_like(kernel)
            side, deferred_join = _wgrad_side(kernel, ctx.weight_is_param, g.device, ctx.needs_input_grad[0], x, g, ws, gw, pairs, plan,
                                               allow=getattr(ctx, 'overlap_ok', True))
            L.call(_entry('u2mkd_conv_wgrad_pairs', x.dtype), L.ptr(x), cin, L.ptr(g), cout,
                   L.ptr(pairs), L.ptr(plan), n, 1, 0, L.ptr(ws), nbytes, L.ptr(gw), side.cuda_stream if side is not None else L.stream())
        if ctx.needs_input_grad[0]:
            gx = _dense_x3(g, kernel, False, kernel_layout=True)
        if side is not None and not deferred_join:
            torch.cuda.current_stream(g.device).wait_stream(side)
        if ctx.has_bias and ctx.needs_input_grad[2]:
            gb = g.sum(0, dtype=torch.float32)
        if gx is not None and gx.dtype != ctx.in_dtype:
            gx = gx.to(ctx.in_dtype)
        return gx, gw, gb


def linear(x, weight, bias=None, bias_feeds_batchnorm=False):
    cout, cin = weight.shape
    pin = (-cin) % 4
    pout = 0 if cout % 4 == 0 else ((-cout) % 32 if cin % 32 == 0 else (-cout) % 4)
    if pin == 0 and pout == 0:
        return LinearFunction.apply(x, weight, bias, bias_feeds_batchnorm)
    if pin:
        x = torch.nn.functional.pad(x, (0, pin))
    weight = torch.nn.functional.pad(weight, (0, pin, 0, pout))
    if bias is not None and pout:
        bias = torch.nn.functional.pad(bias, (0, pout))
    return LinearFunction.apply(x, weight, bias, bias_feeds_batchnorm)[:, :cout]


_OVERLAP_WGRAD = os.environ.get('U2MKD_OVERLAP_WGRAD', '1') != '0'
_DEFER_BIAS_GRAD = os.environ.get('U2MKD_DEFER_BIAS_GRAD', '1') != '0'


def _side_stream(device):
    from ... import deferred
    return deferred.stream(device.index if device.index is not None else torch.cuda.current_device(), 'sparse_wgrad')


def _deferred_overlap_ok():
    from ... import deferred
    return deferred.overlap_ok()


def _wgrad_side(weight, is_param, device, overlap_inline, *used, allow=True):
    from ... import deferred as _d
    if not _OVERLAP_WGRAD or not allow or not _d.overlap_ok():
        return None, False
    from ... import deferred
    if is_param and weight.grad is None and deferred.enabled():
        if deferred.owned(id(weight)):
            deferred.join()
        else:
            side = deferred.side_for('sparse_wgrad', device, owner=id(weight))
            for t in used:
                t.record_stream(side)
            return side, True
    if not overlap_inline:
        return None, False
    side = _side_stream(device)
    side.wait_stream(torch.cuda.current_stream(device))
    return side, False


class ConvolutionFunction(Function):

    @staticmethod
    def forward(ctx, input, weight, kmap, transposed=False):
        L.require_cuda(input, weight)
        param = weight
        weight = weight.contiguous().float()
        ctx.weight_is_param = param.is_leaf and weight.data_ptr() == param.data_ptr() and weight.dtype == param.dtype
        ctx.overlap_ok = _deferred_overlap_ok()
        k, cin, cout = weight.shape
        want16 = row_dtype()
        rows16 = want16 if _conv_rows16_ok(cin, cout) else None
        ctx.in_dtype = input.dtype
        input = _rows(input, rows16)
        if input.shape[1] != cin:
            raise RuntimeError(f'conv3d: input has {input.shape[1]} channels, kernel expects {cin}')
        if cin % 4 != 0:
            raise RuntimeError(f'conv3d: in_channels={cin} must be a multiple of 4 (16-byte row gathers)')
        if not transposed:
            inverse, n_rows = False, kmap.n_out
            expect = kmap.n_in
        else:
            inverse, n_rows = True, kmap.n_in
            expect = kmap.n_out
        if input.shape[0] != expect:
            raise RuntimeError(f'conv3d: {input.shape[0]} input rows, kernel map expects {expect}')
        out = _conv_os(input, weight, True, cout, kmap, inverse, n_rows, 0)
        ctx.save_for_backward(input, weight)
        ctx.kmap = kmap
        ctx.transposed = transposed
        return out.to(want16) if (want16 is not None and rows16 is None) else out

    @staticmethod
    def backward(ctx, grad_output):
        input, weight = ctx.saved_tensors
        kmap, transposed = ctx.kmap, ctx.transposed
        g = _rows(grad_output, input.dtype)
        k, cin, cout = weight.shape
        grad_input = grad_weight = None
        do_w = ctx.needs_input_grad[1]
        do_x = ctx.needs_input_grad[0]
        side, deferred_join = None, False
        if do_w:
            pairs, _, plan = kmap.pairs_plan()
            lib = L.load()
            nbytes = lib.u2mkd_conv_wgrad_pairs_workspace_bytes(kmap.n_out, cin, cout, k)
            ws = torch.empty(max(nbytes, 16), dtype=torch.uint8, device=g.device)
            grad_weight = torch.empty_like(weight)
            side, deferred_join = _wgrad_side(weight, ctx.weight_is_param, g.device, do_x, input, g, ws, grad_weight, pairs, plan,
                                               allow=getattr(ctx, 'overlap_ok', True))
            st = side.cuda_stream if side is not None else L.stream()
            L.call(_entry('u2mkd_conv_wgrad_pairs', input.dtype), L.ptr(input), cin, L.ptr(g), cout,
                   L.ptr(pairs), L.ptr(plan), kmap.n_out, k, 1 if transposed else 0, L.ptr(ws), nbytes, L.ptr(grad_weight), st)
        if do_x:
            if not transposed:
                inverse, kflip = (False, 1) if kmap.symmetric else (True, 0)
            else:
                inverse, kflip = False, 0
            if cout % 4 != 0:
                raise RuntimeError(f'conv3d backward: out_channels={cout} must be a multiple of 4')
            grad_input = _conv_os(g, weight, False, cin, kmap, inverse, input.shape[0], kflip)
        if side is not None and not deferred_join:
            torch.cuda.current_stream(g.device).wait_stream(side)
        if grad_input is not None and grad_input.dtype != ctx.in_dtype:
            grad_input = grad_input.to(ctx.in_dtype)
        return grad_input, grad_weight, None, None


def _conv_any_channels(feats, weight, kmap, transposed):
    cin, cout = weight.shape[1], weight.shape[2]
    pin, pout = (-cin) % 4, (-cout) % 4
    if feats.shape[1] != cin:
        raise RuntimeError(f'conv3d: input has {feats.shape[1]} channels, kernel expects {cin}')
    if pin == 0 and pout == 0:
        return ConvolutionFunction.apply(feats, weight, kmap, transposed)
    feats = torch.nn.functional.pad(feats, (0, pin))
    weight = torch.nn.functional.pad(weight, (0, pout, 0, pin))
    return ConvolutionFunction.apply(feats, weight, kmap, transposed)[:, :cout]


def conv3d(input: SparseTensor, weight: torch.Tensor, kernel_size, bias=None, stride=1, dilation=1,
           transposed: bool = False) -> SparseTensor:
    feats, coords = input.feats, input.coords
    kernel_size = make_ntuple(kernel_size, ndim=3)
    stride = make_ntuple(stride, ndim=3)
    dilation = make_ntuple(dilation, ndim=3)

    if kernel_size == (1, 1, 1) and stride == (1, 1, 1) and dilation == (1, 1, 1):
        w = weight[0] if weight.dim() == 3 else weight
        if (weight.dim() == 2 or weight.shape[0] == 1) and weight.is_contiguous() and weight.dtype == torch.float32 \
                and _dense_x3_ok(w.shape[0], w.shape[1]) and feats.is_cuda and feats.dim() == 2 and feats.shape[1] == w.shape[0]:
            feats = PointwiseConvFunction.apply(feats, weight, bias)
        elif w.shape[0] % 4 == 0 and w.shape[1] % 4 == 0:
            feats = linear(feats, w.t(), bias)
        else:
            feats = feats.matmul(w)
            if bias is not None:
                feats = feats + bias
        output = SparseTensor(coords=coords, feats=feats, stride=input.stride)
    elif not transposed:
        key = (input.stride, kernel_size, stride, dilation)
        kmap = input.kmaps.get(key)
        if kmap is None:
            kmap = build_kmap(coords, input.stride, kernel_size, stride)
            input.kmaps[key] = kmap
        feats = _conv_any_channels(feats, weight, kmap, transposed)
        if bias is not None:
            feats = feats + bias
        output = SparseTensor(coords=kmap.out_coords, feats=feats,
                              stride=tuple(input.stride[k] * stride[k] for k in range(3)))
    else:
        tensor_stride = tuple(input.stride[k] // stride[k] for k in range(3))
        kmap = input.kmaps[(tensor_stride, kernel_size, stride, dilation)]
        feats = _conv_any_channels(feats, weight, kmap, transposed)
        if bias is not None:
            feats = feats + bias
        output = SparseTensor(coords=input.cmaps[tensor_stride], feats=feats, stride=tensor_stride)

    output.cmaps = input.cmaps
    output.cmaps.setdefault(output.stride, output.coords)
    output.kmaps = input.kmaps
    return output


class BatchNormFunction(Function):

    @staticmethod
    def forward(ctx, x, gamma, beta, running_mean, running_var, training, momentum, eps, relu, counter=None, res=None, stats=None):
        L.require_cuda(x)
        rows16 = row_dtype() or _stored16(x.dtype)
        ctx.in_dtype, ctx.res_dtype = x.dtype, (res.dtype if res is not None else None)
        x = _rows(x, rows16)
        n, c = x.shape
        dev = x.device
        if res is not None:
            assert relu and res.shape == x.shape, (relu, res.shape, x.shape)
            res = _rows(res, rows16)
        y = torch.empty_like(x)
        invstd = torch.empty(c, dtype=torch.float32, device=dev)
        if training and stats is not None and rows16 is None:
            mean = torch.empty(c, dtype=torch.float32, device=dev)
            L.call('u2mkd_bn_train_forward_from_partial', L.ptr(x), L.ptr(res), n, c, L.ptr(gamma), L.ptr(beta), float(eps),
                   float(momentum), L.ptr(running_mean), L.ptr(running_var), L.ptr(counter), int(relu), L.ptr(stats.partial),
                   int(stats.slab_rows), L.ptr(mean), L.ptr(invstd), L.ptr(y), L.stream())
        elif training:
            slabs = L.load().u2mkd_bn_num_slabs(n)
            partial = torch.empty(max(slabs, 1) * 2 * c, dtype=torch.float32, device=dev)
            mean = torch.empty(c, dtype=torch.float32, device=dev)
            L.call('u2mkd_bn_train_forward', L.ptr(x), L.ptr(res), _row_code(x.dtype), n, c, L.ptr(gamma), L.ptr(beta), float(eps),
                   float(momentum), L.ptr(running_mean), L.ptr(running_var), L.ptr(counter), int(relu), L.ptr(partial),
                   L.ptr(mean), L.ptr(invstd), L.ptr(y), L.stream())
        else:
            mean = running_mean
            L.call('u2mkd_bn_eval_forward', L.ptr(x), L.ptr(res), _row_code(x.dtype), n, c, L.ptr(gamma), L.ptr(beta), float(eps),
                   L.ptr(running_mean), L.ptr(running_var), int(relu), L.ptr(invstd), L.ptr(y), L.stream())
        ctx.save_for_backward(x, gamma, beta, mean, invstd, res)
        ctx.relu, ctx.training = bool(relu), bool(training)
        return y

    @staticmethod
    def backward(ctx, dy):
        x, gamma, beta, mean, invstd, res = ctx.saved_tensors
        dy = _rows(dy, x.dtype)
        n, c = x.shape
        dev = x.device
        slabs = L.load().u2mkd_bn_num_slabs(n)
        partial = torch.empty(max(slabs, 1) * 2 * c, dtype=torch.float32, device=dev)
        dgamma = torch.empty(c, dtype=torch.float32, device=dev)
        dbeta = torch.empty(c, dtype=torch.float32, device=dev)
        dx = torch.empty_like(x)
        dres = torch.empty_like(x) if res is not None else None
        L.call('u2mkd_bn_backward', L.ptr(dy), L.ptr(x), L.ptr(res), _row_code(x.dtype), n, c, L.ptr(mean), L.ptr(invstd), L.ptr(gamma),
               L.ptr(beta), int(ctx.relu), int(ctx.training), L.ptr(partial), L.ptr(dgamma), L.ptr(dbeta), L.ptr(dx),
               L.ptr(dres), L.stream())
        if dx.dtype != ctx.in_dtype:
# ... 294 lines not shown
```

Before: 1.268 million.

## Fuse gradient fan-in accumulation into backward input-gradient kernel epilogues

```diff
diff --git a/include/u2mkd_hip.h b/include/u2mkd_hip.h
--- a/include/u2mkd_hip.h
+++ b/include/u2mkd_hip.h
@@ -113,6 +113,17 @@
                                float *y, u2mkd_stream_t s);
 int u2mkd_pairs_gather_sum(const float *y, const int32_t *pos , int64_t n_rows, int32_t k, int32_t cout,
                            float *out , u2mkd_stream_t s);
+int u2mkd_pairs_gather_sum_acc(const float *y, const int32_t *pos , int64_t n_rows, int32_t k, int32_t cout,
+                               const float *addend , int64_t addend_ld, float *out ,
+                               u2mkd_stream_t s);
+int u2mkd_conv_forward_tiles_acc(const float *in, int64_t n_in, int32_t cin, const void *wf, int32_t cout,
+                                 const int32_t *nbr_sorted, const int32_t *order, const int32_t *items,
+                                 const int32_t *n_items, int64_t n_out, int32_t k, int32_t kflip, int32_t arith,
+                                 const float *addend , int64_t addend_ld, float *out, u2mkd_stream_t s);
+int u2mkd_linear_forward_f16x2_acc(const float *x, int64_t n, int32_t cin, const void *wf, int32_t cout, const float *bias,
+                                   const float *addend , int64_t addend_ld, float *y, u2mkd_stream_t s);
+int u2mkd_linear_forward_x3_acc(const float *x, int64_t n, int32_t cin, const void *wf, int32_t cout, const float *bias,
+                                const float *addend , int64_t addend_ld, float *y, u2mkd_stream_t s);
 int u2mkd_kmap_rowmask(const int32_t *nbr , int64_t n_out, int32_t k, int32_t *mask ,
                        u2mkd_stream_t s);
 int u2mkd_conv_forward_tiles_bf16(const void *in , int64_t n_in, int32_t cin, const void *wf, int32_t cout,
diff --git a/u2mkd_amd/_lib.py b/u2mkd_amd/_lib.py
--- a/u2mkd_amd/_lib.py
+++ b/u2mkd_amd/_lib.py
@@ -75,6 +75,10 @@
     'u2mkd_pairs_capacity': (_i64, [_i64, _i64, _i32]),
     'u2mkd_pairs_build': (C.c_int, [_p, _i64, _i64, _i32, _p, _p, _p, _p, _p, _p, _p, _p, _p]),
     'u2mkd_pairs_gather_sum': (C.c_int, [_p, _p, _i64, _i32, _i32, _p, _p]),
+    'u2mkd_pairs_gather_sum_acc': (C.c_int, [_p, _p, _i64, _i32, _i32, _p, _i64, _p, _p]),
+    'u2mkd_conv_forward_tiles_acc': (C.c_int, [_p, _i64, _i32, _p, _i32, _p, _p, _p, _p, _i64, _i32, _i32, _i32, _p, _i64, _p, _p]),
+    'u2mkd_linear_forward_f16x2_acc': (C.c_int, [_p, _i64, _i32, _p, _i32, _p, _p, _i64, _p, _p]),
+    'u2mkd_linear_forward_x3_acc': (C.c_int, [_p, _i64, _i32, _p, _i32, _p, _p, _i64, _p, _p]),
     'u2mkd_kmap_rowmask': (C.c_int, [_p, _i64, _i32, _p, _p]),
     'u2mkd_tile_schedule_workspace_bytes': (_sz, [_i64]),
     'u2mkd_tile_schedule': (C.c_int, [_p, _p, _i64, _i32, _i32, _i32, _p, _p, _p, _p, _p]),
diff --git a/u2mkd_amd/csrc/conv.hip b/u2mkd_amd/csrc/conv.hip
--- a/u2mkd_amd/csrc/conv.hip
+++ b/u2mkd_amd/csrc/conv.hip
@@ -760,10 +760,12 @@
     return 0;
 }
 
+template <bool ADD = false>
 __global__ void __launch_bounds__(256)
 pairs_gather_sum_kernel(const float *__restrict__ y, const int32_t *__restrict__ pos, int64_t n_rows, int K, int c4,
                         float *__restrict__ out, const float *__restrict__ ep_scale = nullptr,
-                        const float *__restrict__ ep_shift = nullptr, const float *__restrict__ ep_res = nullptr, int ep_relu = 0) {
+                        const float *__restrict__ ep_shift = nullptr, const float *__restrict__ ep_res = nullptr, int ep_relu = 0,
+                        int64_t addend_ld4 = 0) {
     int64_t t = (int64_t)blockIdx.x * 256 + threadIdx.x;
     if (t >= n_rows * c4) return;
     int64_t r = t / c4;
@@ -781,7 +783,7 @@
 #pragma unroll
         for (int i = 0; i < 8; ++i) { acc.x += v[i].x; acc.y += v[i].y; acc.z += v[i].z; acc.w += v[i].w; }
     }
-    if (ep_scale) {
+    if (!ADD && ep_scale) {
         const float4 sc = reinterpret_cast<const float4 *>(ep_scale)[c], sh = reinterpret_cast<const float4 *>(ep_shift)[c];
         acc.x = fmaf(acc.x, sc.x, sh.x); acc.y = fmaf(acc.y, sc.y, sh.y); acc.z = fmaf(acc.z, sc.z, sh.z); acc.w = fmaf(acc.w, sc.w, sh.w);
         if (ep_res) {
@@ -789,6 +791,10 @@
             acc.x += rs.x; acc.y += rs.y; acc.z += rs.z; acc.w += rs.w;
         }
         if (ep_relu) { acc.x = fmaxf(acc.x, 0.f); acc.y = fmaxf(acc.y, 0.f); acc.z = fmaxf(acc.z, 0.f); acc.w = fmaxf(acc.w, 0.f); }
+    }
+    if (ADD && ep_res) {
+        const float4 ad = reinterpret_cast<const float4 *>(ep_res)[r * addend_ld4 + c];
+        acc.x = __fadd_rn(acc.x, ad.x); acc.y = __fadd_rn(acc.y, ad.y); acc.z = __fadd_rn(acc.z, ad.z); acc.w = __fadd_rn(acc.w, ad.w);
     }
     reinterpret_cast<float4 *>(out)[r * c4 + c] = acc;
 }
@@ -1218,9 +1224,74 @@
     U2_REQUIRE(cout > 0 && cout % 4 == 0 && k > 0, "u2mkd_pairs_gather_sum: cout=%d must be a positive multiple of 4", cout);
     const int c4 = cout / 4;
     const int64_t total = n_rows * c4;
-    hipLaunchKernelGGL(pairs_gather_sum_kernel, dim3((unsigned)ceil_div(total, 256)), dim3(256), 0, as_stream(s), y, pos,
+    hipLaunchKernelGGL(pairs_gather_sum_kernel<false>, dim3((unsigned)ceil_div(total, 256)), dim3(256), 0, as_stream(s), y, pos,
                        n_rows, k, c4, out, (const float *)nullptr, (const float *)nullptr, (const float *)nullptr, 0);
     return check_launch("u2mkd_pairs_gather_sum");
+}
+
+#define U2_REQUIRE_ADDEND(who, addend, addend_ld, cout)                                                                          \
+    U2_REQUIRE(!(addend) || ((addend_ld) >= (cout) && (addend_ld) % 4 == 0 && reinterpret_cast<uintptr_t>(addend) % 16 == 0),     \
+               "%s: the addend's row stride %lld must be a multiple of 4, at least cout=%d, its base 16-byte aligned", who,        \
+               (long long)(addend_ld), (int)(cout))
+
+int u2mkd_pairs_gather_sum_acc(const float *y, const int32_t *pos, int64_t n_rows, int32_t k, int32_t cout, const float *addend,
+                               int64_t addend_ld, float *out, u2mkd_stream_t s) {
+    if (n_rows == 0) return 0;
+    U2_REQUIRE(y && pos && out, "u2mkd_pairs_gather_sum_acc: null pointer");
+    U2_REQUIRE(cout > 0 && cout % 4 == 0 && k > 0, "u2mkd_pairs_gather_sum_acc: cout=%d must be a positive multiple of 4", cout);
+    U2_REQUIRE_ADDEND("u2mkd_pairs_gather_sum_acc", addend, addend_ld, cout);
+    U2_REQUIRE(addend != out, "u2mkd_pairs_gather_sum_acc: the addend must not alias the output");
+    const int c4 = cout / 4;
+    const int64_t total = n_rows * c4;
+    hipLaunchKernelGGL(pairs_gather_sum_kernel<true>, dim3((unsigned)ceil_div(total, 256)), dim3(256), 0, as_stream(s), y, pos,
+                       n_rows, k, c4, out, (const float *)nullptr, (const float *)nullptr, addend, 0,
+                       addend ? addend_ld / 4 : (int64_t)0);
+    return check_launch("u2mkd_pairs_gather_sum_acc");
+}
+
+int u2mkd_conv_forward_tiles_acc(const float *in, int64_t n_in, int32_t cin, const void *wf, int32_t cout,
+                                 const int32_t *nbr_sorted, const int32_t *order, const int32_t *items,
+                                 const int32_t *n_items, int64_t n_out, int32_t k, int32_t kflip, int32_t arith,
+                                 const float *addend, int64_t addend_ld, float *out, u2mkd_stream_t s) {
+    if (n_out <= 0) return 0;
+    U2_REQUIRE(in && wf && nbr_sorted && out, "u2mkd_conv_forward_tiles_acc: null pointer");
+    U2_REQUIRE(kflip == 0 || kflip == 1, "u2mkd_conv_forward_tiles_acc: kflip must be 0 or 1");
+    U2_REQUIRE((arith >= 0 && arith <= 2) || arith == 4, "u2mkd_conv_forward_tiles_acc: arith must be 0 (default), 1 (f32), 2 (bf16x3) or 4 (f16x2)");
+    U2_REQUIRE(n_in > 0 && n_in <= (1 << 25), "u2mkd_conv_forward_tiles_acc: %lld input rows out of range", (long long)n_in);
+    U2_REQUIRE((items == nullptr) == (n_items == nullptr), "u2mkd_conv_forward_tiles_acc: items and n_items go together");
+    U2_REQUIRE_ADDEND("u2mkd_conv_forward_tiles_acc", addend, addend_ld, cout);
+    U2_REQUIRE(addend != out, "u2mkd_conv_forward_tiles_acc: the addend must not alias the output");
+    RowRange rr{n_out, 0, n_out, nullptr};
+    U2_REQUIRE(addend_ld < ((int64_t)1 << 31), "u2mkd_conv_forward_tiles_acc: addend row stride %lld out of range", (long long)addend_ld);
+    rr.ep_res = addend; rr.ep_relu = addend ? (int)addend_ld : 0;
+    int rc = launch_conv_tp("u2mkd_conv_forward_tiles_acc", in, cin, reinterpret_cast<const float *>(wf), cout, nbr_sorted, order,
+                            rr, items, n_items, k, kflip, arith, out, as_stream(s));
+    U2_REQUIRE(rc >= 0, "u2mkd_conv_forward_tiles_acc: no instantiation for %d -> %d channels, kernel volume %d "
+               "(ask u2mkd_conv_tiles_supported first)", cin, cout, k);
+    return rc;
+}
+
+static int linear_forward_acc(const char *who, bool f16x2, const float *x, int64_t n, int32_t cin, const void *wf, int32_t cout,
+                              const float *bias, const float *addend, int64_t addend_ld, float *y, u2mkd_stream_t s) {
+    if (n == 0) return 0;
+    U2_REQUIRE(x && wf && y, "%s: null pointer", who);
+    U2_REQUIRE(n > 0 && n < ((int64_t)1 << 31) - 64, "%s: %lld rows out of range", who, (long long)n);
+    U2_REQUIRE_ADDEND(who, addend, addend_ld, cout);
+    U2_REQUIRE(addend != y, "%s: the addend must not alias the output", who);
+    int rc = launch_linear_px3(who, x, n, cin, reinterpret_cast<const float *>(wf), cout, bias, y, as_stream(s), kRowsF32, f16x2,
+                               addend, addend ? addend_ld : 0);
+    U2_REQUIRE(rc >= 0, "%s: cin=%d and cout=%d must be multiples of 32", who, cin, cout);
+    return rc;
+}
+
+int u2mkd_linear_forward_f16x2_acc(const float *x, int64_t n, int32_t cin, const void *wf, int32_t cout, const float *bias,
+                                   const float *addend, int64_t addend_ld, float *y, u2mkd_stream_t s) {
+    return linear_forward_acc("u2mkd_linear_forward_f16x2_acc", true, x, n, cin, wf, cout, bias, addend, addend_ld, y, s);
+}
+
+int u2mkd_linear_forward_x3_acc(const float *x, int64_t n, int32_t cin, const void *wf, int32_t cout, const float *bias,
+                                const float *addend, int64_t addend_ld, float *y, u2mkd_stream_t s) {
+    return linear_forward_acc("u2mkd_linear_forward_x3_acc", false, x, n, cin, wf, cout, bias, addend, addend_ld, y, s);
 }
 
 int32_t u2mkd_pairs_gather_sum_stats_slab_rows(void) { return kGsSlabRows; }
@@ -1246,7 +1317,7 @@
     U2_REQUIRE(cout > 0 && cout % 4 == 0 && k > 0, "u2mkd_pairs_gather_sum_ep: cout=%d must be a positive multiple of 4", cout);
     const int c4 = cout / 4;
     const int64_t total = n_rows * c4;
-    hipLaunchKernelGGL(pairs_gather_sum_kernel, dim3((unsigned)ceil_div(total, 256)), dim3(256), 0, as_stream(s), y, pos,
+    hipLaunchKernelGGL(pairs_gather_sum_kernel<false>, dim3((unsigned)ceil_div(total, 256)), dim3(256), 0, as_stream(s), y, pos,
                        n_rows, k, c4, out, scale, shift, res, (int)relu);
     return check_launch("u2mkd_pairs_gather_sum_ep");
 }
diff --git a/u2mkd_amd/csrc/conv_internal.h b/u2mkd_amd/csrc/conv_internal.h
--- a/u2mkd_amd/csrc/conv_internal.h
+++ b/u2mkd_amd/csrc/conv_internal.h
@@ -112,7 +112,9 @@
                     int rows16 = kRowsF32 ,
                     int f16x2_k = 0 );
 int launch_linear_px3(const char *who, const float *in, int64_t n_rows, int cin, const float *wf, int cout,
-                      const float *bias, float *y, hipStream_t st, int rows16 = kRowsF32, bool f16x2 = false);
+                      const float *bias, float *y, hipStream_t st, int rows16 = kRowsF32, bool f16x2 = false,
+                      const float *addend = nullptr ,
+                      int64_t addend_ld = 0);
 
 bool conv_wgrad_x3_supported(int ca, int cb, int k);
 int launch_conv_wgrad_x3(const float *a, int ca, const float *b, int cb, const int32_t *pairs, const int32_t *plan,
diff --git a/u2mkd_amd/csrc/conv_px3.hip b/u2mkd_amd/csrc/conv_px3.hip
--- a/u2mkd_amd/csrc/conv_px3.hip
+++ b/u2mkd_amd/csrc/conv_px3.hip
@@ -27,15 +27,16 @@
     return __int_as_float(__builtin_amdgcn_update_dpp(0, __float_as_int(v), CTRL, 0xf, 0xf, true));
 }
 
-template <int NW, int NBW, bool DENSE = false, bool B16 = false, int SC = 32, int TL = 1, bool F2 = false, bool H16 = false>
+template <int NW, int NBW, bool DENSE = false, bool B16 = false, int SC = 32, int TL = 1, bool F2 = false, bool H16 = false, bool ADD = false>
 __global__ void __launch_bounds__(64 * NW)
 conv_px3_kernel(const float *__restrict__ in, int cin, const float *__restrict__ wf, int cout,
                 const int32_t *__restrict__ pair_idx, const int32_t *__restrict__ tile_k,
                 const int32_t *__restrict__ n_tiles, float *__restrict__ y, const float *__restrict__ bias = nullptr,
-                int n_rows = 0, int k_total = 1) {
+                int n_rows = 0, int k_total = 1, const float *__restrict__ addend = nullptr, int64_t addend_ld = 0) {
     static_assert(B16 ? (SC == 32 || SC == 64) : SC == 32, "step width");
     static_assert(!(F2 && B16), "f16x2 is an arithmetic of fp32 rows");
     static_assert(!H16 || B16, "fp16 storage is a form of the 2-byte-row pipeline");
+    static_assert(!ADD || (DENSE && !B16), "the addend is an operand of the dense fp32-row store");
     constexpr int NT = 64 * NW, TN = 16 * NW * NBW;
     constexpr int RS = 192;
     constexpr int CH = B16 ? SC / 8 : 8;
@@ -262,6 +263,11 @@
                     if (cbw + n < ncb && (!DENSE || row < n_rows)) {
                         f32x4 o = acc[rb][n];
                         if (DENSE && bias) o += *reinterpret_cast<const f32x4 *>(bias + col);
+                        if (ADD && addend) {
+                            const f32x4 ad = *reinterpret_cast<const f32x4 *>(addend + (size_t)row * addend_ld + col);
+                            o[0] = __fadd_rn(o[0], ad[0]); o[1] = __fadd_rn(o[1], ad[1]);
+                            o[2] = __fadd_rn(o[2], ad[2]); o[3] = __fadd_rn(o[3], ad[3]);
+                        }
                         if (H16) {
                             *reinterpret_cast<uint2 *>(reinterpret_cast<char *>(y) + ((size_t)row * cout + col) * 2) =
                                 make_uint2(pack_rows16<true>(o[0], o[1]), pack_rows16<true>(o[2], o[3]));
@@ -305,14 +311,14 @@
     return p;
 }
 
-template <bool DENSE, bool B16, int SC, bool F2 = false, bool H16 = false>
+template <bool DENSE, bool B16, int SC, bool F2 = false, bool H16 = false, bool ADD = false>
 static void px3_launch(const Px3Shape &p, dim3 grid, hipStream_t st, const float *in, int cin, const float *wf, int cout,
                        const int32_t *pair_idx, const int32_t *tile_k, const int32_t *n_tiles, float *y, const float *bias,
-                       int n_rows, int k_total = 1) {
+                       int n_rows, int k_total = 1, const float *addend = nullptr, int64_t addend_ld = 0) {
     const size_t lds = (size_t)2 * 64 * p.tl * 192;
 #define U2_PX3(NW_, NBW_, TL_)                                                                                                  \
-    hipLaunchKernelGGL((conv_px3_kernel<NW_, NBW_, DENSE, B16, SC, TL_, F2, H16>), grid, dim3(64 * NW_), lds, st, in, cin, wf, cout, pair_idx, \
-                       tile_k, n_tiles, y, bias, n_rows, k_total)
+    hipLaunchKernelGGL((conv_px3_kernel<NW_, NBW_, DENSE, B16, SC, TL_, F2, H16, ADD>), grid, dim3(64 * NW_), lds, st, in, cin, wf, cout, pair_idx, \
+                       tile_k, n_tiles, y, bias, n_rows, k_total, addend, addend_ld)
     if (p.tl == 2) {
         if (p.w3) U2_PX3(3, 2, 2); else U2_PX3(4, 2, 2);
     } else if (p.nbw == 4) {
@@ -343,15 +349,18 @@
 }
 
 int launch_linear_px3(const char *who, const float *in, int64_t n_rows, int cin, const float *wf, int cout,
-                      const float *bias, float *y, hipStream_t st, int rows16, bool f16x2) {
+                      const float *bias, float *y, hipStream_t st, int rows16, bool f16x2, const float *addend, int64_t addend_ld) {
     if (!conv_px3_supported(cin, cout)) return -1;
+    if (addend && rows16 != kRowsF32) return -1;
     const Px3Shape p = px3_shape(cin, cout);
     const int gy = (int)ceil_div(cout, p.tn);
     const int64_t cap_x = (p.tl == 1 && p.nbw == 2 ? 3 : 2) * 256;
     int64_t gx = std::min<int64_t>(cap_x, ceil_div(ceil_div(n_rows, 64 * p.tl) * gy, 8) * 8);
     if (gx < 8) gx = 8;
     dim3 grid((unsigned)gx);
-    if (f16x2) px3_launch<true, false, 32, true>(p, grid, st, in, cin, wf, cout, nullptr, nullptr, nullptr, y, bias, (int)n_rows, 1);
+    if (addend && f16x2) px3_launch<true, false, 32, true, false, true>(p, grid, st, in, cin, wf, cout, nullptr, nullptr, nullptr, y, bias, (int)n_rows, 1, addend, addend_ld);
+    else if (addend) px3_launch<true, false, 32, false, false, true>(p, grid, st, in, cin, wf, cout, nullptr, nullptr, nullptr, y, bias, (int)n_rows, 1, addend, addend_ld);
+    else if (f16x2) px3_launch<true, false, 32, true>(p, grid, st, in, cin, wf, cout, nullptr, nullptr, nullptr, y, bias, (int)n_rows, 1);
     else if (rows16 == kRowsF32) px3_launch<true, false, 32>(p, grid, st, in, cin, wf, cout, nullptr, nullptr, nullptr, y, bias, (int)n_rows);
     else if (rows16 == kRowsF16 && cin % 64 == 0) px3_launch<true, true, 64, false, true>(p, grid, st, in, cin, wf, cout, nullptr, nullptr, nullptr, y, bias, (int)n_rows);
     else if (rows16 == kRowsF16) px3_launch<true, true, 32, false, true>(p, grid, st, in, cin, wf, cout, nullptr, nullptr, nullptr, y, bias, (int)n_rows);
diff --git a/u2mkd_amd/csrc/conv_tp.hip b/u2mkd_amd/csrc/conv_tp.hip
--- a/u2mkd_amd/csrc/conv_tp.hip
+++ b/u2mkd_amd/csrc/conv_tp.hip
@@ -609,6 +609,9 @@
                     v.x += r.x; v.y += r.y; v.z += r.z; v.w += r.w;
                 }
                 if (rr_.ep_relu) { v.x = fmaxf(v.x, 0.f); v.y = fmaxf(v.y, 0.f); v.z = fmaxf(v.z, 0.f); v.w = fmaxf(v.w, 0.f); }
+            } else if (!B16 && rr_.ep_res) {
+                const float4 ad = *reinterpret_cast<const float4 *>(rr_.ep_res + (size_t)rid * rr_.ep_relu + col);
+                v.x = __fadd_rn(v.x, ad.x); v.y = __fadd_rn(v.y, ad.y); v.z = __fadd_rn(v.z, ad.z); v.w = __fadd_rn(v.w, ad.w);
             }
             if (H16) {
                 *reinterpret_cast<uint2 *>(reinterpret_cast<char *>(out) + ((size_t)rid * cout + col) * 2) =
diff --git a/u2mkd_amd/fusion.py b/u2mkd_amd/fusion.py
--- a/u2mkd_amd/fusion.py
+++ b/u2mkd_amd/fusion.py
@@ -37,13 +37,21 @@
         self.fc2 = nn.Linear(self.pc, rc)
         self.fc3 = nn.Linear(rc, 1)
 
-    def forward(self, img_feats, point_feats):
+    def forward(self, img_feats, point_feats, own_point_feats=False):
+        from .torchsparse.nn.functional import FanIn
         img_feats = img_feats.contiguous()
+        with FanIn() as own:
+            img_lin = _rows_linear(img_feats, self.conv1[0].weight, self.conv1[0].bias, before=self.conv1[1])
+        if own.thru is not None:
+            img_feats = own.thru
         ri = _rows_linear(_rows_bn(self.fc1[0], img_feats, relu=True), self.fc1[2].weight, self.fc1[2].bias)
-        rp = _rows_linear(point_feats.contiguous(), self.fc2.weight, self.fc2.bias)
+        with FanIn() as own:
+            rp = _rows_linear(point_feats.contiguous(), self.fc2.weight, self.fc2.bias)
+        if own.thru is not None:
+            point_feats = own.thru
         att = torch.sigmoid(_rows_linear(torch.tanh(ri + rp), self.fc3.weight, self.fc3.bias))
-        img = _rows_bn(self.conv1[1], _rows_linear(img_feats, self.conv1[0].weight, self.conv1[0].bias, before=self.conv1[1]), relu=True)
-        return img * att
+        img = _rows_bn(self.conv1[1], img_lin, relu=True)
+        return (img * att, point_feats) if own_point_feats else img * att
 
 
 class Atten_Fusion_Conv(nn.Module):
@@ -54,7 +62,7 @@
         self.bn1 = nn.BatchNorm1d(outplanes)
 
     def forward(self, point_features, img_features):
-        img = self.ai_layer(img_features, point_features)
+        img, point_features = self.ai_layer(img_features, point_features, own_point_feats=True)
         fused = torch.cat([point_features, img], dim=1)
         return _rows_bn(self.bn1, _rows_linear(fused, self.conv1.weight, self.conv1.bias, before=self.bn1), relu=True)
 
diff --git a/u2mkd_amd/kd.py b/u2mkd_amd/kd.py
--- a/u2mkd_amd/kd.py
+++ b/u2mkd_amd/kd.py
@@ -194,7 +194,10 @@
         for idx in range(n_stage):
             if idx > 0:
                 cam = on_side(lambda: cam_stage(x_im, idx), x_im, after=x_im_ready if _CAMERA_FORK_EARLY else None)
-            vox_out = self.vox_downs[idx](vox_feats[idx])
+            with spf.FanIn() as own:
+                vox_out = self.vox_downs[idx](vox_feats[idx])
+            if own.thru is not None and idx > 0:
+                vox_feats[idx].F = own.thru
             if ahead is not None:
                 coord_xyz, batch = ahead['tokens'][idx]
             else:
@@ -215,10 +218,11 @@
             img_feats.append(skip)
 
             img_feat_tensor = c2l_gather(skip.view(ib, ncam, ifc, ifh, ifw), pixel_coordinates, masks)
-            pseudo = self.learner[idx](pts_feat.F)
+            with spf.FanIn() as own:
+                pseudo = self.learner[idx](pts_feat.F)
             img_feat_tensor, mse = _select_and_mse(img_feat_tensor, pseudo, fov_mask)
             mse_loss.append(mse)
-            pts_feat.F = self.c2l_fusion_blocks[idx](pts_feat.F, img_feat_tensor)
+            pts_feat.F = self.c2l_fusion_blocks[idx](pts_feat.F if own.thru is None else own.thru, img_feat_tensor)
             vox_feats.append(point_to_voxel(vox_out, pts_feat))
 
         fused = fork.mark()
diff --git a/u2mkd_amd/lidar/blocks.py b/u2mkd_amd/lidar/blocks.py
--- a/u2mkd_amd/lidar/blocks.py
+++ b/u2mkd_amd/lidar/blocks.py
@@ -46,6 +46,17 @@
     def forward(self, x, residual=None):
         mods = list(self)
         i = 0
+        if isinstance(residual, nn.Module):
+            shortcut, residual = residual, None
+            if (spf.fanin_store_enabled() and torch.is_grad_enabled() and isinstance(x, SparseTensor) and mods
+                    and isinstance(mods[0], spnn.Conv3d) and x.F.requires_grad and not spf.conv_bn_stats_enabled()):
+                with spf.FanIn() as owner:
+                    y = mods[0](x)
+                xs = x if owner.thru is None else fapply(x, lambda f: owner.thru)
+                x, i = y, 1
+                residual = shortcut(xs)
+            else:
+                residual = shortcut(x)
         fold = _FOLD_EVAL_BN and isinstance(x, SparseTensor) and not torch.is_grad_enabled()
         stats = None
         while i < len(mods):
@@ -140,4 +151,4 @@
         self.relu = spnn.ReLU(True)
 
     def forward(self, x):
-        return self.net(x, residual=self.downsample(x))
+        return self.net(x, residual=self.downsample)
diff --git a/u2mkd_amd/torchsparse/nn/functional.py b/u2mkd_amd/torchsparse/nn/functional.py
--- a/u2mkd_amd/torchsparse/nn/functional.py
+++ b/u2mkd_amd/torchsparse/nn/functional.py
@@ -576,7 +576,7 @@
     def tiles(self):
         return self.nbr_s, self.order
 
-    def run(self, feats, weight, transpose, cout, kflip, out, epilogue=None):
+    def run(self, feats, weight, transpose, cout, kflip, out, epilogue=None, addend=None):
         n_in, cin = feats.shape
         ar = 4 if feats.dtype == torch.float32 and _tiles_arith(cin, cout, self.k) == 4 else 0
         if epilogue is not None:
@@ -591,6 +591,11 @@
             L.call(_entry('u2mkd_conv_forward_tiles', feats.dtype), L.ptr(feats), n_in, cin, L.ptr(wf), cout, L.ptr(self.nbr_s),
                    L.ptr(self.order), L.ptr(self.items), L.ptr(self.n_items), self.n, self.k, int(kflip), L.ptr(out),
                    L.stream())
+        elif addend is not None:
+            wf = _weight_layout(weight, transpose, True, arith=ar)
+            L.call('u2mkd_conv_forward_tiles_acc', L.ptr(feats), n_in, cin, L.ptr(wf), cout, L.ptr(self.nbr_s),
+                   L.ptr(self.order), L.ptr(self.items), L.ptr(self.n_items), self.n, self.k, int(kflip), ar, L.ptr(addend),
+                   addend.stride(0), L.ptr(out), L.stream())
         elif L.load().u2mkd_conv_tiles_supported(cin, cout, self.k):
             wf = _weight_layout(weight, transpose, True, arith=ar)
             L.call('u2mkd_conv_forward_tiles', L.ptr(feats), n_in, cin, L.ptr(wf), cout, L.ptr(self.nbr_s),
@@ -654,7 +659,7 @@
                    L.ptr(self.tile_k), L.ptr(self.meta), st)
         self.nbsizes = nbsizes
 
-    def run(self, feats, wt, cout, swap, out, variant=0, fragments=False, epilogue=None):
+    def run(self, feats, wt, cout, swap, out, variant=0, fragments=False, epilogue=None, addend=None):
         n, cin = feats.shape
         st = L.stream()
         idx, pos, n_rows = (self.pair_out, self.pos_in, self.n_in) if swap else (self.pair_in, self.pos_out, self.n_out)
@@ -676,6 +681,9 @@
             sc, sh, res, relu = epilogue
             L.call('u2mkd_pairs_gather_sum_ep', L.ptr(y), L.ptr(pos), n_rows, self.k, cout, L.ptr(sc), L.ptr(sh), L.ptr(res), int(relu),
                    L.ptr(out), st)
+            return out
+        if addend is not None:
+            L.call('u2mkd_pairs_gather_sum_acc', L.ptr(y), L.ptr(pos), n_rows, self.k, cout, L.ptr(addend), addend.stride(0), L.ptr(out), st)
             return out
         sink = BN_STATS_SINK[0]
         if sink is not None and sink.partial is None and out.dtype == torch.float32 and _stats_in_store(n_rows, cout):
@@ -828,9 +836,50 @@
             x.cmaps.setdefault(ts, coords)
 
 
-def _conv_os(feats, weight, transpose, cout, kmap, inverse, n_rows, kflip, epilogue=None):
+_FANIN_STORE = os.environ.get('U2MKD_FANIN_STORE', '1') != '0'
+FANIN_SINK = [None]
+
+
+class FanIn:
+    __slots__ = ('thru',)
+
+    def __init__(self):
+        self.thru = None
+
+    def __enter__(self):
+        FANIN_SINK[0] = self
+        return self
+
+    def __exit__(self, *exc):
+        FANIN_SINK[0] = None
+        return False
+
+
+def fanin_store_enabled():
+    return _FANIN_STORE
+
+
+def _fanin_wanted(x):
+    sink = FANIN_SINK[0]
+    if sink is None:
+        return None
+    FANIN_SINK[0] = None
+    if not (_FANIN_STORE and torch.is_grad_enabled() and x.requires_grad and x.is_cuda and x.dtype == torch.float32
+            and x.dim() == 2 and row_dtype() is None):
+        return None
+    return sink
+
+
+def _addend_ok(a, n_rows, cout):
+    return (a is not None and a.is_cuda and a.dtype == torch.float32 and a.dim() == 2 and tuple(a.shape) == (n_rows, cout)
+            and a.stride(1) == 1 and a.stride(0) >= cout and a.stride(0) % 4 == 0 and a.data_ptr() % 16 == 0)
+
+
+def _conv_os(feats, weight, transpose, cout, kmap, inverse, n_rows, kflip, epilogue=None, addend=None):
     out = torch.empty(n_rows, cout, dtype=feats.dtype, device=feats.device)
     rows16 = feats.dtype != torch.float32
+    if addend is not None and (rows16 or epilogue is not None or not _addend_ok(addend, n_rows, cout)):
+        return _conv_os(feats, weight, transpose, cout, kmap, inverse, n_rows, kflip, epilogue) + addend.to(feats.dtype)
     if rows16 and not L.load().u2mkd_conv_tiles_supported(feats.shape[1], cout, kmap.k):
         wt = _weight_layout(weight, transpose, True, arith=_arith16(feats.dtype))
         return kmap.pair_schedule().run(feats, wt, cout, bool(inverse) or bool(kflip), out)
@@ -838,12 +887,15 @@
         x3 = _PAIRS_X3 and bool(L.load().u2mkd_conv_pairs_x3_supported(feats.shape[1], cout))
         f2 = x3 and _pairs_f16x2(feats.shape[1], cout)
         wt = _weight_layout(weight, transpose, x3, arith=4 if f2 else 0)
-        return kmap.pair_schedule().run(feats, wt, cout, bool(inverse) or bool(kflip), out, fragments=2 if f2 else x3, epilogue=epilogue)
+        return kmap.pair_schedule().run(feats, wt, cout, bool(inverse) or bool(kflip), out, fragments=2 if f2 else x3, epilogue=epilogue,
+                                        addend=addend)
     if inverse and kmap.nbr_inv is None:
         inverse, kflip = False, 1 - int(kflip)
     sch = kmap.schedule(inverse)
     assert sch.n == n_rows
-    return sch.run(feats, weight, transpose, cout, kflip, out, epilogue=epilogue)
+    if addend is not None and not L.load().u2mkd_conv_tiles_supported(feats.shape[1], cout, kmap.k):
+        return sch.run(feats, weight, transpose, cout, kflip, out) + addend
+    return sch.run(feats, weight, transpose, cout, kflip, out, epilogue=epilogue, addend=addend)
 
 
 def conv_epilogue_supported(feats, cin, cout, k, n_rows):
@@ -1058,7 +1110,7 @@
     return _PAIRS_X3 and _LINEAR_X3 and bool(L.load().u2mkd_conv_pairs_x3_supported(cin, cout))
 
 
-def _dense_x3(x, weight, forward, bias=None, kernel_layout=False):
+def _dense_x3(x, weight, forward, bias=None, kernel_layout=False, addend=None):
     n = x.shape[0]
     if kernel_layout:
         cout = weight.shape[-1] if forward else weight.shape[-2]
@@ -1068,9 +1120,13 @@
     f2 = not rows16 and _pairs_f16x2(x.shape[1], cout)
     wf = _weight_layout(weight, forward if kernel_layout else not forward, True, arith=_arith16(x.dtype) if rows16 else (4 if f2 else 0))
     y = torch.empty(n, cout, dtype=x.dtype, device=x.device)
+    if addend is not None and not rows16 and _addend_ok(addend, n, cout):
+        L.call('u2mkd_linear_forward_f16x2_acc' if f2 else 'u2mkd_linear_forward_x3_acc', L.ptr(x), n, x.shape[1], L.ptr(wf), cout,
+               L.ptr(bias), L.ptr(addend), addend.stride(0), L.ptr(y), L.stream())
+        return y
     L.call(_entry('u2mkd_linear_forward', x.dtype) if rows16 else ('u2mkd_linear_forward_f16x2' if f2 else 'u2mkd_linear_forward_x3'), L.ptr(x), n,
            x.shape[1], L.ptr(wf), cout, L.ptr(bias), L.ptr(y), L.stream())
-    return y
+    return y if addend is None else y + addend.to(y.dtype)
 
 
 def _dense(x, w_oc_ic, bias=None):
@@ -1101,8 +1157,9 @@
 class LinearFunction(Function):
 
     @staticmethod
-    def forward(ctx, x, weight, bias, bias_grad_is_zero=False):
+    def forward(ctx, x, weight, bias, bias_grad_is_zero=False, thru=False):
         L.require_cuda(x, weight)
+        x_in = x
         param = weight
         weight = weight.contiguous().float()
         owner = param if param.is_leaf else _leaf_behind_view(param)
@@ -1121,22 +1178,28 @@
         ctx.save_for_backward(x, weight)
         ctx.has_bias = bias is not None
         ctx.bias_grad_is_zero = bool(bias_grad_is_zero)
+        if thru:
+            ctx.set_materialize_grads(False)
         if x.shape[0] == 0:
-            return x.new_zeros(0, weight.shape[0])
+            y = x.new_zeros(0, weight.shape[0])
+            return (y, x_in) if thru else y
         b = bias.contiguous().float() if bias is not None else None
         ctx.x3 = rows16 is not None or _dense_x3_ok(weight.shape[1], weight.shape[0])
         y = _dense_x3(x, weight, True, b) if ctx.x3 else _dense(x, weight, b)
-        return y.to(want16) if (want16 is not None and rows16 is None) else y
+        y = y.to(want16) if (want16 is not None and rows16 is None) else y
+        return (y, x_in) if thru else y
 
     @staticmethod
-    def backward(ctx, g):
+    def backward(ctx, g, g_thru=None):
         x, weight = ctx.saved_tensors
+        if g is None:
+            return g_thru, None, None, None, None
         g = _rows(g, x.dtype)
         n = x.shape[0]
         cout, cin = weight.shape
         gx = gw = gb = None
         if n == 0:
-            return x.new_zeros(x.shape), torch.zeros_like(weight), (weight.new_zeros(cout) if ctx.has_bias else None), None
+            return x.new_zeros(x.shape), torch.zeros_like(weight), (weight.new_zeros(cout) if ctx.has_bias else None), None, None
         side, deferred_join = None, False
         if ctx.needs_input_grad[1]:
             pairs, plan = _identity_pairs(n, g.device)
@@ -1149,11 +1212,13 @@
             L.call(_entry('u2mkd_conv_wgrad_pairs', x.dtype), L.ptr(g), cout, L.ptr(x), cin,
                    L.ptr(pairs), L.ptr(plan), n, 1, 0, L.ptr(ws), nbytes, L.ptr(gw), side.cuda_stream if side is not None else L.stream())
         if ctx.needs_input_grad[0] and ctx.x3:
-            gx = _dense_x3(g, weight, False)
+            gx = _dense_x3(g, weight, False, addend=g_thru)
         elif ctx.needs_input_grad[0]:
             w_t = torch.empty(1, cin, cout, dtype=torch.float32, device=g.device)
             L.call('u2mkd_transpose_weights', L.ptr(weight), 1, cout, cin, L.ptr(w_t), L.stream())
             gx = _dense(g, w_t[0])
+            if g_thru is not None:
+                gx = gx + g_thru
         if side is not None and not deferred_join:
             torch.cuda.current_stream(g.device).wait_stream(side)
         if ctx.has_bias and ctx.needs_input_grad[2]:
@@ -1169,14 +1234,15 @@
                 gb = weight.new_zeros(cout) if ctx.bias_grad_is_zero else g.sum(0, dtype=torch.float32)
         if gx is not None and gx.dtype != ctx.in_dtype:
             gx = gx.to(ctx.in_dtype)
-        return gx, gw, gb, None
+        return gx, gw, gb, None, None
 
 
 class PointwiseConvFunction(Function):
 
     @staticmethod
-    def forward(ctx, x, kernel, bias):
+    def forward(ctx, x, kernel, bias, thru=False):
         L.require_cuda(x, kernel)
+        x_in = x
         ctx.weight_is_param = kernel.is_leaf
         ctx.overlap_ok = _deferred_overlap_ok()
         cin, cout = kernel.shape[-2], kernel.shape[-1]
@@ -1188,21 +1254,27 @@
             raise RuntimeError(f'conv3d (1x1x1): input {tuple(x.shape)} does not match kernel {tuple(kernel.shape)}')
         ctx.save_for_backward(x, kernel)
         ctx.has_bias = bias is not None
+        if thru:
+            ctx.set_materialize_grads(False)
         if x.shape[0] == 0:
-            return x.new_zeros(0, cout)
+            y = x.new_zeros(0, cout)
+            return (y, x_in) if thru else y
         b = bias.contiguous().float() if bias is not None else None
         y = _dense_x3(x, kernel, True, b, kernel_layout=True)
-        return y.to(want16) if (want16 is not None and rows16 is None) else y
+        y = y.to(want16) if (want16 is not None and rows16 is None) else y
+        return (y, x_in) if thru else y
 
     @staticmethod
-    def backward(ctx, g):
+    def backward(ctx, g, g_thru=None):
         x, kernel = ctx.saved_tensors
+        if g is None:
+            return g_thru, None, None, None
         g = _rows(g, x.dtype)
         n = x.shape[0]
         cin, cout = kernel.shape[-2], kernel.shape[-1]
         gx = gw = gb = None
         if n == 0:
-            return x.new_zeros(x.shape), torch.zeros_like(kernel), (kernel.new_zeros(cout) if ctx.has_bias else None)
+            return x.new_zeros(x.shape), torch.zeros_like(kernel), (kernel.new_zeros(cout) if ctx.has_bias else None), None
         side, deferred_join = None, False
         if ctx.needs_input_grad[1]:
             pairs, plan = _identity_pairs(n, g.device)
@@ -1214,21 +1286,25 @@
             L.call(_entry('u2mkd_conv_wgrad_pairs', x.dtype), L.ptr(x), cin, L.ptr(g), cout,
                    L.ptr(pairs), L.ptr(plan), n, 1, 0, L.ptr(ws), nbytes, L.ptr(gw), side.cuda_stream if side is not None else L.stream())
         if ctx.needs_input_grad[0]:
-            gx = _dense_x3(g, kernel, False, kernel_layout=True)
+            gx = _dense_x3(g, kernel, False, kernel_layout=True, addend=g_thru)
         if side is not None and not deferred_join:
             torch.cuda.current_stream(g.device).wait_stream(side)
         if ctx.has_bias and ctx.needs_input_grad[2]:
             gb = g.sum(0, dtype=torch.float32)
         if gx is not None and gx.dtype != ctx.in_dtype:
             gx = gx.to(ctx.in_dtype)
-        return gx, gw, gb
+        return gx, gw, gb, None
 
 
 def linear(x, weight, bias=None, bias_feeds_batchnorm=False):
     cout, cin = weight.shape
     pin = (-cin) % 4
     pout = 0 if cout % 4 == 0 else ((-cout) % 32 if cin % 32 == 0 else (-cout) % 4)
+    sink = _fanin_wanted(x) if FANIN_SINK[0] is not None else None
     if pin == 0 and pout == 0:
+        if sink is not None and x.dim() == 2 and _dense_x3_ok(cin, cout):
+            y, sink.thru = LinearFunction.apply(x, weight, bias, bias_feeds_batchnorm, True)
+            return y
         return LinearFunction.apply(x, weight, bias, bias_feeds_batchnorm)
     if pin:
         x = torch.nn.functional.pad(x, (0, pin))
@@ -1275,8 +1351,9 @@
 class ConvolutionFunction(Function):
 
     @staticmethod
-    def forward(ctx, input, weight, kmap, transposed=False):
+    def forward(ctx, input, weight, kmap, transposed=False, thru=False):
         L.require_cuda(input, weight)
+        x_in = input
         param = weight
         weight = weight.contiguous().float()
         ctx.weight_is_param = param.is_leaf and weight.data_ptr() == param.data_ptr() and weight.dtype == param.dtype
@@ -1302,12 +1379,18 @@
         ctx.save_for_backward(input, weight)
         ctx.kmap = kmap
         ctx.transposed = transposed
-        return out.to(want16) if (want16 is not None and rows16 is None) else out
+        out = out.to(want16) if (want16 is not None and rows16 is None) else out
+        if thru:
+            ctx.set_materialize_grads(False)
+            return out, x_in
+        return out
 
     @staticmethod
-    def backward(ctx, grad_output):
+    def backward(ctx, grad_output, g_thru=None):
         input, weight = ctx.saved_tensors
         kmap, transposed = ctx.kmap, ctx.transposed
+        if grad_output is None:
+            return g_thru, None, None, None, None
         g = _rows(grad_output, input.dtype)
         k, cin, cout = weight.shape
         grad_input = grad_weight = None
@@ -1332,12 +1415,12 @@
                 inverse, kflip = False, 0
             if cout % 4 != 0:
                 raise RuntimeError(f'conv3d backward: out_channels={cout} must be a multiple of 4')
-            grad_input = _conv_os(g, weight, False, cin, kmap, inverse, input.shape[0], kflip)
+            grad_input = _conv_os(g, weight, False, cin, kmap, inverse, input.shape[0], kflip, addend=g_thru)
         if side is not None and not deferred_join:
             torch.cuda.current_stream(g.device).wait_stream(side)
         if grad_input is not None and grad_input.dtype != ctx.in_dtype:
             grad_input = grad_input.to(ctx.in_dtype)
-        return grad_input, grad_weight, None, None
+        return grad_input, grad_weight, None, None, None
 
 
 def _conv_any_channels(feats, weight, kmap, transposed):
@@ -1345,7 +1428,11 @@
     pin, pout = (-cin) % 4, (-cout) % 4
     if feats.shape[1] != cin:
         raise RuntimeError(f'conv3d: input has {feats.shape[1]} channels, kernel expects {cin}')
+    sink = _fanin_wanted(feats) if FANIN_SINK[0] is not None else None
     if pin == 0 and pout == 0:
+        if sink is not None:
+            out, sink.thru = ConvolutionFunction.apply(feats, weight, kmap, transposed, True)
+            return out
         return ConvolutionFunction.apply(feats, weight, kmap, transposed)
     feats = torch.nn.functional.pad(feats, (0, pin))
     weight = torch.nn.functional.pad(weight, (0, pout, 0, pin))
@@ -1363,7 +1450,11 @@
         w = weight[0] if weight.dim() == 3 else weight
         if (weight.dim() == 2 or weight.shape[0] == 1) and weight.is_contiguous() and weight.dtype == torch.float32 \
                 and _dense_x3_ok(w.shape[0], w.shape[1]) and feats.is_cuda and feats.dim() == 2 and feats.shape[1] == w.shape[0]:
-            feats = PointwiseConvFunction.apply(feats, weight, bias)
+            sink = _fanin_wanted(feats) if FANIN_SINK[0] is not None else None
+            if sink is not None:
+                feats, sink.thru = PointwiseConvFunction.apply(feats, weight, bias, True)
+            else:
+                feats = PointwiseConvFunction.apply(feats, weight, bias)
         elif w.shape[0] % 4 == 0 and w.shape[1] % 4 == 0:
             feats = linear(feats, w.t(), bias)
         else:
```

Result: slower. 1.244 million (-1.9%).
